# COx2/docker-nvidia-glx-desktop

Measured on AMD Instinct MI355X. Metric: encoded FPS + p50 end-to-end latency at 1080p60 H.264; concurrent sessions/node, higher is better.
Workload: dtype uint8 video (8-bit 4:2:0), H.264 Constrained Baseline

## Files before the change

### csrc/bindings/module.cpp

```cpp
#include <pybind11/numpy.h>
#include <pybind11/pybind11.h>
#include <pybind11/stl.h>

#include <cstring>

#include "../codec/h264_core.h"
#include "../codec/h264_encoder.h"
#include "../codec/vp8_encoder.h"
#include "../codec/hevc_encoder.h"
#include "../common/hip_check.h"
#include "../common/trace.h"
#include "../kernels/pixel.h"
#include "../runtime/session.h"

namespace py = pybind11;
using namespace mx;

void register_net(py::module& m);
void register_audio(py::module& m);
void register_rfb(py::module& m);

namespace {

template <class T>
// ... 6 lines not shown
    return py::bytes(reinterpret_cast<const char*>(v.data()), v.size());
}

struct PyBits {
    std::vector<uint32_t> words;
    h264::BitWriter w;
    PyBits() : words(4096) { w.init(words.data()); }
    py::tuple finish() {
        const uint32_t bits = w.bits;
        w.flush();
        std::vector<uint8_t> out;
        for (uint32_t i = 0; i < (bits + 7) / 8; ++i) out.push_back((uint8_t)(words[i / 4] >> (24 - 8 * (i % 4))));
        return py::make_tuple(to_bytes(out), bits);
    }
};

py::tuple cavlc_block_py(const std::vector<int>& coef, int nc) {
    PyBits b;
    int16_t c[16] = {0};
    const int n = (int)coef.size();
    if (n != 4 && n != 15 && n != 16) throw std::invalid_argument("block must have 4, 15 or 16 coefficients");
    for (int i = 0; i < n; ++i) c[i] = (int16_t)coef[i];
    h264::cavlc_block(b.w, c, n, nc);
    return b.finish();
}

py::array_t<int> fdct_py(py::array_t<int, py::array::c_style | py::array::forcecast> x) {
    if (x.size() != 16) throw std::invalid_argument("need 16 values");
    py::array_t<int> y(16);
    h264::fdct4x4(x.data(), y.mutable_data());
    return y;
}
py::array_t<int> idct_py(py::array_t<int, py::array::c_style | py::array::forcecast> x) {
    if (x.size() != 16) throw std::invalid_argument("need 16 values");
    py::array_t<int> y(16);
    h264::idct4x4(x.data(), y.mutable_data());
    return y;
}

py::array_t<uint8_t> copy_plane(const uint8_t* dev, int pitch, int w, int h) {
    py::array_t<uint8_t> out({h, w});
    HIP_CHECK(hipDeviceSynchronize());
    HIP_CHECK(hipMemcpy2D(out.mutable_data(), w, dev, pitch, w, h, hipMemcpyDeviceToHost));
    return out;
}

}

PYBIND11_MODULE(_native, m) {
    m.doc() = "mxdesk native runtime: HIP kernels (gfx950), H.264 encoder, session pipeline";

    m.def("device_count", []() {
        int n = 0;
        if (hipGetDeviceCount(&n) != hipSuccess) return 0;
        return n;
    });
    m.def("set_device", [](int d) { HIP_CHECK(hipSetDevice(d)); });
    m.def("device_name", [](int d) {
        hipDeviceProp_t p;
        HIP_CHECK(hipGetDeviceProperties(&p, d));
        return std::string(p.gcnArchName) + " / " + p.name;
    });
    m.def("synchronize", []() { HIP_CHECK(hipDeviceSynchronize()); });
    register_net(m);
    register_audio(m);
    register_rfb(m);
    m.def("now_us", &Session::now_us, "CLOCK_MONOTONIC microseconds (same clock as time.monotonic())");

    py::module h = m.def_submodule("h264", "H.264 building blocks (for tests)");
    h.def("hpel_planes", [](py::array_t<uint8_t, py::array::c_style> ref, int coded_w) {
        if (ref.ndim() != 2 || coded_w % 16 || ref.shape(0) % 16 || ref.shape(1) < coded_w)
            throw std::invalid_argument("ref must be (coded_h, pitch) with 16-aligned coded size");
        int hp = 0;
        auto planes = h264::hpel_planes_for_test(ref.data(), coded_w, (int)ref.shape(0), (int)ref.shape(1), &hp);
        const int rows = (int)ref.shape(0) + 2 * h264::kHpelPad;
        py::list out;
        for (auto& p : planes) {
            py::array_t<uint8_t> a({rows, hp});
            std::memcpy(a.mutable_data(), p.data(), p.size());
            out.append(a);
        }
        return out;
    });
    h.def("cavlc_block", &cavlc_block_py, py::arg("coef"), py::arg("nc"));
    h.def("fdct4x4", &fdct_py);
    h.def("idct4x4", &idct_py);
    h.def("ue", [](uint32_t k) {
        PyBits b;
        h264::put_ue(b.w, k);
        return b.finish();
    });
    h.def("se", [](int v) {
        PyBits b;
        h264::put_se(b.w, v);
        return b.finish();
    });
    h.def("luma_qpel", [](py::array_t<uint8_t, py::array::c_style> plane, int x4, int y4) {
        if (plane.ndim() != 2) throw std::invalid_argument("2-D plane");
        const int H = (int)plane.shape(0), W = (int)plane.shape(1);
        return h264::luma_qpel(plane.data(), W, W, H, x4, y4);
    });
    h.def("level_for", &h264::pick_level);

    py::class_<h264::EncoderConfig>(m, "EncoderConfig")
        .def(py::init<>())
        .def_readwrite("width", &h264::EncoderConfig::width)
        .def_readwrite("height", &h264::EncoderConfig::height)
        .def_readwrite("fps", &h264::EncoderConfig::fps)
        .def_readwrite("bitrate_kbps", &h264::EncoderConfig::bitrate_kbps)
        .def_readwrite("qp", &h264::EncoderConfig::qp)
        .def_readwrite("qp_min", &h264::EncoderConfig::qp_min)
        .def_readwrite("qp_max", &h264::EncoderConfig::qp_max)
        .def_readwrite("keyint", &h264::EncoderConfig::keyint)
        .def_readwrite("search_range", &h264::EncoderConfig::search_range)
        .def_readwrite("me_coarse", &h264::EncoderConfig::me_coarse)
        .def_readwrite("intra4x4", &h264::EncoderConfig::intra4x4)
        .def_readwrite("subpel", &h264::EncoderConfig::subpel)
        .def_readwrite("chroma_qp_offset", &h264::EncoderConfig::chroma_qp_offset)
        .def_readwrite("pipeline_depth", &h264::EncoderConfig::pipeline_depth)
        .def_readwrite("aq", &h264::EncoderConfig::aq)
        .def_readwrite("intra_in_p", &h264::EncoderConfig::intra_in_p)
        .def_readwrite("vp8_bpred", &h264::EncoderConfig::vp8_bpred)
        .def_readwrite("vp8_intra", &h264::EncoderConfig::vp8_intra)
        .def_readwrite("mask_x0", &h264::EncoderConfig::mask_x0)
        .def_readwrite("mask_y0", &h264::EncoderConfig::mask_y0)
        .def_readwrite("mask_x1", &h264::EncoderConfig::mask_x1)
        .def_readwrite("mask_y1", &h264::EncoderConfig::mask_y1)
        .def_readwrite("deblock", &h264::EncoderConfig::deblock)
        .def_readwrite("partitions", &h264::EncoderConfig::partitions)
        .def_readwrite("tu_split", &h264::EncoderConfig::tu_split)
        .def_readwrite("hevc_slice_cost", &h264::EncoderConfig::hevc_slice_cost)
        .def_readwrite("hevc_wpp", &h264::EncoderConfig::hevc_wpp)
        .def_readwrite("hevc_wpp_rows", &h264::EncoderConfig::hevc_wpp_rows)
        .def_readwrite("sao", &h264::EncoderConfig::sao)
        .def_readwrite("hevc_chroma_keep", &h264::EncoderConfig::hevc_chroma_keep)
        .def_readwrite("hevc_intra_split", &h264::EncoderConfig::hevc_intra_split);

    py::class_<h264::FrameStats>(m, "FrameStats")
        .def_readonly("frame_index", &h264::FrameStats::frame_index)
        .def_readonly("idr", &h264::FrameStats::idr)
        .def_readonly("qp", &h264::FrameStats::qp)
        .def_readonly("bytes", &h264::FrameStats::bytes)
        .def_readonly("skipped_mbs", &h264::FrameStats::skipped_mbs)
        .def_readonly("encode_ms", &h264::FrameStats::encode_ms)
        .def_property_readonly("sse", [](const h264::FrameStats& s) { return py::make_tuple(s.sse[0], s.sse[1], s.sse[2]); })
        .def_readonly("sse_masked", &h264::FrameStats::sse_masked)
        .def_readonly("masked_pixels", &h264::FrameStats::masked_pixels)
        .def_readonly("deblocked", &h264::FrameStats::deblocked)
        .def_readonly("db_coherent", &h264::FrameStats::db_coherent)
        .def_readonly("db_changed", &h264::FrameStats::db_changed)
        .def_readonly("db_moving", &h264::FrameStats::db_moving);

    py::class_<h264::CpuH264Encoder>(m, "CpuH264Encoder")
        .def(py::init<const h264::EncoderConfig&>())
        .def(
            "encode",
            [](h264::CpuH264Encoder& e, py::array_t<uint8_t, py::array::c_style> y,
               py::array_t<uint8_t, py::array::c_style> uv, bool force_idr) {
                if (y.ndim() != 2 || uv.ndim() != 2 || y.shape(1) != uv.shape(1))
                    throw std::invalid_argument("y (H,P) and uv (H/2,P) planes with equal pitch");
                const int pitch = (int)y.shape(1);
                const int cw = e.coded_pitch();
                const auto& cfg = e.common().config();
                const int ch = e.common().mb_h() * 16;
                if (y.shape(0) < cfg.height || pitch < cfg.width || uv.shape(0) < cfg.height / 2)
                    throw std::invalid_argument("planes smaller than the encoder's configured picture");
// ... 598 lines not shown
```

### csrc/codec/h264_encoder.cpp

```cpp
#include "h264_encoder.h"

#include <hip/hip_ext.h>

#include <algorithm>
#include <cmath>
#include <cstring>
#include <stdexcept>
#include <string>

#include "../common/hip_check.h"
#include "h264_mb.h"

namespace mx {
namespace h264 {

EncoderCommon::EncoderCommon(const EncoderConfig& c) : cfg_(c) {
    if (c.width <= 0 || c.height <= 0 || (c.width & 1) || (c.height & 1))
        throw std::invalid_argument("encoder size must be positive and even");
    mb_w_ = (c.width + 15) / 16;
    mb_h_ = (c.height + 15) / 16;
    cur_qp_ = std::clamp(c.qp, 0, 51);
}

double EncoderCommon::frame_budget_bits() const {
// ... 106 lines not shown
        const uint8_t b = rbsp[i];
        if (zeros >= 2 && b <= 3) {
            out.push_back(3);
            zeros = 0;
        }
        out.push_back(b);
        zeros = (b == 0) ? zeros + 1 : 0;
    }
}

void EncoderCommon::write_parameter_sets(std::vector<uint8_t>& out) const {
    uint32_t words[64];
    SeqParams sp;
    sp.width = cfg_.width;
    sp.height = cfg_.height;
    sp.mb_w = mb_w_;
    sp.mb_h = mb_h_;
    sp.level_idc = pick_level(mb_w_ * mb_h_, cfg_.fps);
    sp.log2_max_frame_num = log2_max_frame_num();
    sp.fps_num = cfg_.fps;
    sp.fps_den = 1;
    BitWriter w;
    w.init(words);
    write_sps(w, sp);
    std::vector<uint8_t> rbsp;
    words_to_bytes(words, w.bits + (w.bits % 8 ? 8 - w.bits % 8 : 0), rbsp);
    static const uint8_t sc[4] = {0, 0, 0, 1};
    out.insert(out.end(), sc, sc + 4);
    out.push_back(0x67);
    emulation_prevent(out, rbsp.data(), rbsp.size());
    w.init(words);
    write_pps(w, pic_init_qp(), cfg_.chroma_qp_offset);
    rbsp.clear();
    words_to_bytes(words, w.bits + (w.bits % 8 ? 8 - w.bits % 8 : 0), rbsp);
    out.insert(out.end(), sc, sc + 4);
    out.push_back(0x68);
    emulation_prevent(out, rbsp.data(), rbsp.size());
}

void EncoderCommon::write_slice_nal(std::vector<uint8_t>& out, const uint8_t* rbsp, size_t n, bool idr) const {
    static const uint8_t sc[4] = {0, 0, 0, 1};
    out.insert(out.end(), sc, sc + 4);
    out.push_back(idr ? 0x65 : 0x41);
    emulation_prevent(out, rbsp, n);
}

std::vector<std::vector<uint8_t>> hpel_planes_for_test(const uint8_t* ref, int coded_w, int coded_h, int pitch,
                                                       int* hp_pitch_out) {
    Geometry g{};
    g.width = coded_w;
    g.height = coded_h;
    g.mb_w = coded_w / 16;
    g.mb_h = coded_h / 16;
    g.coded_w = coded_w;
    g.coded_h = coded_h;
    g.pitch = pitch;
    const int hp_pitch = (coded_w + 2 * kHpelPad + 255) & ~255;
    const size_t hp_bytes = (size_t)hp_pitch * (coded_h + 2 * kHpelPad);
    uint8_t* dref = nullptr;
    uint8_t* planes[4];
    FrameState fs{};
    DeviceBuffers b{};
    HIP_CHECK(hipMalloc(&dref, (size_t)pitch * coded_h));
    HIP_CHECK(hipMemcpy(dref, ref, (size_t)pitch * coded_h, hipMemcpyHostToDevice));
    for (auto& p : planes) {
        HIP_CHECK(hipMalloc(&p, hp_bytes));
        HIP_CHECK(hipMemset(p, 0, hp_bytes));
    }
    fs.ref_y = dref;
    HIP_CHECK(hipMalloc(&b.fs, sizeof(FrameState)));
    HIP_CHECK(hipMemcpy(b.fs, &fs, sizeof(FrameState), hipMemcpyHostToDevice));
    launch_hpel(g, b, planes, hp_pitch, nullptr);
    HIP_CHECK(hipGetLastError());
    HIP_CHECK(hipDeviceSynchronize());
    std::vector<std::vector<uint8_t>> out(4, std::vector<uint8_t>(hp_bytes));
    for (int i = 0; i < 4; ++i) {
        HIP_CHECK(hipMemcpy(out[i].data(), planes[i], hp_bytes, hipMemcpyDeviceToHost));
        (void)hipFree(planes[i]);
    }
    (void)hipFree(dref);
    (void)hipFree(b.fs);
    *hp_pitch_out = hp_pitch;
    return out;
}

constexpr unsigned kDeviceEvent = hipEventDisableTiming | hipEventReleaseToDevice;

void GpuH264Encoder::alloc_slot(FrameSlot& sl) {
    const int nmb = geom_.mb_w * geom_.mb_h;
    DeviceBuffers& b = sl.buf;
    HIP_CHECK(hipMalloc(&b.fs, sizeof(FrameState)));
    HIP_CHECK(hipMalloc(&b.mb, sizeof(MbInfo) * nmb));
    HIP_CHECK(hipMemsetAsync(b.mb, 0, sizeof(MbInfo) * nmb, stream_));
    HIP_CHECK(hipMalloc(&b.coef, sizeof(int16_t) * kCoefStride * nmb));
    HIP_CHECK(hipMalloc(&b.slot, sizeof(uint32_t) * kSlotWords * (size_t)nmb));
    HIP_CHECK(hipMalloc(&b.slot_bits, sizeof(uint32_t) * nmb));
    HIP_CHECK(hipMalloc(&b.row_agg, sizeof(uint4) * (size_t)geom_.mb_h));
    HIP_CHECK(hipMalloc(&b.row_sse, sizeof(unsigned long long) * 4 * 512));
    HIP_CHECK(hipMalloc(&b.coded_info, sizeof(uint4) * nmb));
    HIP_CHECK(hipMalloc(&b.slice_info, sizeof(uint32_t) * kSliceInfo * kMaxSlices));
    HIP_CHECK(hipMemsetAsync(b.slice_info, 0, sizeof(uint32_t) * kSliceInfo * kMaxSlices, stream_));
    b.out_bytes = (size_t)nmb * 768;
    HIP_CHECK(hipMalloc(&b.quad_unit, sizeof(uint32_t) * (b.out_bytes / 16 + 1)));
    HIP_CHECK(hipMalloc(&b.out_hdr, sizeof(OutHeader)));
    HIP_CHECK(hipMalloc(&b.sse_part, 4 * sizeof(unsigned long long) * kSsePartStride));
    HIP_CHECK(hipMalloc(&b.wave_prog, sizeof(int) * 4));
    HIP_CHECK(hipMalloc(&b.mb_sse, sizeof(uint32_t) * 3 * (size_t)nmb));
    HIP_CHECK(hipMalloc(&b.intra_gain, sizeof(int32_t) * (size_t)nmb));
    HIP_CHECK(hipMalloc(&b.intra_cand, sizeof(int) * (size_t)nmb));
    HIP_CHECK(hipMalloc(&b.db_rec, sizeof(uint4) * (size_t)nmb));
    HIP_CHECK(hipMalloc(&b.db_rowq, sizeof(int) * (size_t)geom_.mb_h));
    HIP_CHECK(hipMalloc(&b.db_glb, sizeof(uint64_t) * 2 * 24 * (size_t)nmb));
    HIP_CHECK(hipMemsetAsync(b.db_glb, 0, sizeof(uint64_t) * 2 * 24 * (size_t)nmb, stream_));
    HIP_CHECK(hipMalloc(&b.pack_done, sizeof(uint32_t)));
    HIP_CHECK(hipMemsetAsync(b.pack_done, 0, sizeof(uint32_t), stream_));
    HIP_CHECK(hipMalloc(&b.db_cnt, sizeof(uint32_t) * 4));
    HIP_CHECK(hipMemsetAsync(b.db_cnt, 0, sizeof(uint32_t) * 4, stream_));
    HIP_CHECK(hipHostMalloc(&b.db_err, sizeof(int), hipHostMallocMapped));
    *b.db_err = 0;
    HIP_CHECK(hipHostMalloc(&sl.fs_host, sizeof(FrameState), hipHostMallocDefault));
    HIP_CHECK(hipHostMalloc(&sl.host_out, kOutPayloadOffset + b.out_bytes + 16, hipHostMallocMapped));
    std::memset(sl.host_out, 0, kOutPayloadOffset);
    HIP_CHECK(hipEventCreateWithFlags(&sl.start, hipEventDisableTiming));
    HIP_CHECK(hipEventCreateWithFlags(&sl.analysis_done, kDeviceEvent));
    HIP_CHECK(hipEventCreateWithFlags(&sl.deblock_done, kDeviceEvent));
    HIP_CHECK(hipEventCreateWithFlags(&sl.hpel_done, kDeviceEvent));
    HIP_CHECK(hipEventCreateWithFlags(&sl.me_done, kDeviceEvent));
    HIP_CHECK(hipEventCreateWithFlags(&sl.done, hipEventDisableTiming));
}

void GpuH264Encoder::free_slot(FrameSlot& sl) {
    DeviceBuffers& b = sl.buf;
    for (void* p : {(void*)b.fs, (void*)b.mb, (void*)b.coef, (void*)b.slot, (void*)b.slot_bits, (void*)b.row_agg,
                    (void*)b.row_sse, (void*)b.coded_info, (void*)b.slice_info,
                    (void*)b.out_hdr, (void*)b.sse_part, (void*)b.wave_prog, (void*)b.mb_sse, (void*)b.intra_gain, (void*)b.intra_cand, (void*)b.quad_unit,
                    (void*)b.db_rec, (void*)b.db_rowq, (void*)b.db_glb, (void*)b.pack_done, (void*)b.db_cnt})
        if (p) (void)hipFree(p);
    if (b.db_err) (void)hipHostFree(b.db_err);
    if (sl.fs_host) (void)hipHostFree(sl.fs_host);
    if (sl.host_out) (void)hipHostFree(sl.host_out);
    for (hipEvent_t e : {sl.start, sl.analysis_done, sl.deblock_done, sl.done, sl.hpel_done, sl.me_done})
        if (e) (void)hipEventDestroy(e);
}

GpuH264Encoder::GpuH264Encoder(const EncoderConfig& cfg, hipStream_t stream)
    : cfg_(cfg.with_aq_default(4)), common_(cfg), stream_(stream) {
    if (cfg.pipeline_depth < 1 || cfg.pipeline_depth > kMaxInFlight)
        throw std::invalid_argument("pipeline_depth must be 1 to 4");
    depth_ = cfg.pipeline_depth;
    db_lag_.reset(cfg_.h264_deblock_mode());
    geom_.width = cfg.width;
    geom_.height = cfg.height;
    geom_.mb_w = common_.mb_w();
    geom_.mb_h = common_.mb_h();
    geom_.coded_w = geom_.mb_w * 16;
    geom_.coded_h = geom_.mb_h * 16;
    geom_.pitch = (geom_.coded_w + 255) & ~255;
    if (geom_.mb_h > kMaxSlices) throw std::invalid_argument("picture too tall");
    if (geom_.mb_w > 512) throw std::invalid_argument("picture too wide (k_intra_wave stages <= 512 MBs per row)");
    const int nmb = geom_.mb_w * geom_.mb_h;
    if ((nmb + 3) / 4 + geom_.mb_h > kSsePartStride)
        throw std::invalid_argument("frame too large for the distortion partials");
    const size_t ysz = (size_t)geom_.pitch * geom_.coded_h, uvsz = ysz / 2;
    for (int i = 0; i < 2; ++i) {
        HIP_CHECK(hipMalloc(&rec_y_[i], ysz));
        HIP_CHECK(hipMalloc(&rec_uv_[i], uvsz));
        HIP_CHECK(hipMemsetAsync(rec_y_[i], 16, ysz, stream_));
        HIP_CHECK(hipMemsetAsync(rec_uv_[i], 128, uvsz, stream_));
        HIP_CHECK(hipMalloc(&src_keep_[i], ysz));
        HIP_CHECK(hipMemsetAsync(src_keep_[i], 16, ysz, stream_));
    }
    if (cfg.mask_x1 > cfg.mask_x0 && cfg.mask_y1 > cfg.mask_y0) {
        mask_mb_[0] = std::max(0, cfg.mask_x0) / 16;
        mask_mb_[1] = std::max(0, cfg.mask_y0) / 16;
        mask_mb_[2] = std::min(geom_.mb_w, (cfg.mask_x1 + 15) / 16);
        mask_mb_[3] = std::min(geom_.mb_h, (cfg.mask_y1 + 15) / 16);
    }
    masked_pixels_ = (int64_t)cfg.width * cfg.height;
    for (int my = mask_mb_[1]; my < mask_mb_[3]; ++my)
        for (int mx = mask_mb_[0]; mx < mask_mb_[2]; ++mx)
            masked_pixels_ -= (int64_t)std::max(0, std::min(16, cfg.width - 16 * mx)) *
                              std::max(0, std::min(16, cfg.height - 16 * my));
    hp_pitch_ = (geom_.coded_w + 2 * kHpelPad + 255) & ~255;
    const size_t hp_bytes = (size_t)hp_pitch_ * (geom_.coded_h + 2 * kHpelPad);
    for (int i = 0; i < 4; ++i) HIP_CHECK(hipMalloc(&hp_[i], hp_bytes));
    if (cfg_.h264_deblock())
        for (int i = 0; i < 4; ++i) HIP_CHECK(hipMalloc(&hpu_[i], hp_bytes));
    for (int i = 0; i < depth_; ++i) alloc_slot(slots_[i]);
    clock_khz_ = device_clock_khz();
    if (depth_ > 1) {
        HIP_CHECK(hipStreamCreateWithFlags(&stream_e_, hipStreamNonBlocking));
        HIP_CHECK(hipStreamCreateWithFlags(&stream_a_, hipStreamNonBlocking));
        HIP_CHECK(hipEventCreateWithFlags(&ref_ready_, kDeviceEvent));
        HIP_CHECK(hipEventRecord(ref_ready_, stream_));
        if (cfg_.h264_deblock()) {
            const char* rv = std::getenv("MXDESK_ME_CU_RESERVE");
            const int reserve = rv ? std::atoi(rv) : 0;
            int ncu = 0;
            HIP_CHECK(hipDeviceGetAttribute(&ncu, hipDeviceAttributeMultiprocessorCount, 0));
            if (reserve > 0 && reserve < ncu) {
                std::vector<uint32_t> mask((size_t)(ncu + 31) / 32, 0u);
                for (int c = 0; c < ncu - reserve; ++c) mask[(size_t)c / 32] |= 1u << (c % 32);
                HIP_CHECK(hipExtStreamCreateWithCUMask(&stream_m_, (uint32_t)mask.size(), mask.data()));
            } else {
                HIP_CHECK(hipStreamCreateWithFlags(&stream_m_, hipStreamNonBlocking));
            }
            HIP_CHECK(hipEventCreateWithFlags(&ev_hpu_, kDeviceEvent));
            HIP_CHECK(hipEventRecord(ev_hpu_, stream_));
        }
    }
    HIP_CHECK(hipStreamSynchronize(stream_));
    const char* et = std::getenv("MXDESK_ENTROPY_THREAD");
    if (stream_e_ && !(et && et[0] == '0')) {
        HIP_CHECK(hipGetDevice(&device_));
        launcher_ = std::thread([this]() { launcher_loop(); });
    }
}

void GpuH264Encoder::set_hpel_side_stream(bool on) {
    hpel_side_ = on;
    if (!on && stream_a_) {
        HIP_CHECK(hipStreamSynchronize(stream_a_));
        HIP_CHECK(hipStreamDestroy(stream_a_));
        stream_a_ = nullptr;
    }
}

void GpuH264Encoder::launcher_loop() {
    (void)hipSetDevice(device_);
    for (;;) {
        EntropyJob j;
        {
            std::unique_lock<std::mutex> lk(lmu_);
            lcv_.wait(lk, [&] { return lstop_ || !ljobs_.empty(); });
            if (ljobs_.empty()) return;
            j = ljobs_.front();
            ljobs_.pop_front();
        }
        try {
            FrameSlot& sl = slots_[j.slot];
            HIP_CHECK(hipStreamWaitEvent(stream_e_, sl.analysis_done, 0));
            launch_entropy(geom_, sl.buf, sl.host_out, stream_e_, j.sse_ready);
            HIP_CHECK(hipGetLastError());
            HIP_CHECK(hipEventRecord(sl.done, stream_e_));
        } catch (...) {
            std::lock_guard<std::mutex> lk(lmu_);
            lerr_ = std::current_exception();
        }
        {
            std::lock_guard<std::mutex> lk(lmu_);
            ++l_done_;
        }
        lcv_.notify_all();
    }
}

void GpuH264Encoder::drain_launcher() const {
    if (!launcher_.joinable()) return;
    std::unique_lock<std::mutex> lk(lmu_);
    lcv_.wait(lk, [&] { return l_done_ >= l_pushed_ || lerr_; });
    if (lerr_) std::rethrow_exception(lerr_);
}

void GpuH264Encoder::wait_launched(int slot) const {
    std::unique_lock<std::mutex> lk(lmu_);
    lcv_.wait(lk, [&] { return l_done_ >= slot_job_[slot] || lerr_; });
    if (lerr_) std::rethrow_exception(lerr_);
}

GpuH264Encoder::~GpuH264Encoder() {
    if (launcher_.joinable()) {
        {
            std::lock_guard<std::mutex> lk(lmu_);
            lstop_ = true;
        }
        lcv_.notify_all();
        launcher_.join();
    }
    (void)hipStreamSynchronize(stream_);
    if (stream_e_) {
        (void)hipStreamSynchronize(stream_e_);
        (void)hipStreamDestroy(stream_e_);
    }
    if (stream_a_) {
        (void)hipStreamSynchronize(stream_a_);
        (void)hipStreamDestroy(stream_a_);
    }
    if (ref_ready_) (void)hipEventDestroy(ref_ready_);
    if (stream_m_) {
        (void)hipStreamSynchronize(stream_m_);
        (void)hipStreamDestroy(stream_m_);
    }
    if (ev_hpu_) (void)hipEventDestroy(ev_hpu_);
    for (int i = 0; i < 4; ++i)
        if (hpu_[i]) (void)hipFree(hpu_[i]);
    for (int i = 0; i < 2; ++i) {
        (void)hipFree(rec_y_[i]);
        (void)hipFree(rec_uv_[i]);
        (void)hipFree(src_keep_[i]);
    }
    for (int i = 0; i < 4; ++i) (void)hipFree(hp_[i]);
    for (int i = 0; i < depth_; ++i) free_slot(slots_[i]);
}

void GpuH264Encoder::enqueue_analysis_kernels(bool idr, const uint8_t* src_y, const uint8_t* src_uv, bool publish) {
    FrameSlot& sl = slots_[prep_slot_];
    const FrameState* pub = publish ? sl.fs_host : nullptr;
    auto wait_input = [&]() {
        if (!in_ev_) return;
        HIP_CHECK(hipStreamWaitEvent(stream_, in_ev_, 0));
        in_ev_ = nullptr;
    };
    if (idr) {
        wait_input();
        launch_intra(geom_, sl.buf, src_y, src_uv, stream_, pub);
        if (cfg_.aq >= 3)
            launch_save_src(geom_, sl.buf, src_y, stream_);
    } else {
        static const bool early = [] {
            const char* e = std::getenv("MXDESK_INPUT_WAIT");
            return e && std::string(e) == "early";
        }();
        if (early) wait_input();
        const bool side_me = stream_m_ && pub && sl.me_unf;
        if (side_me) {
            HIP_CHECK(hipStreamWaitEvent(stream_m_, ev_hpu_, 0));
            if (in_ev_) {
                HIP_CHECK(hipStreamWaitEvent(stream_m_, in_ev_, 0));
                in_ev_ = nullptr;
            }
            launch_me(geom_, sl.buf, src_y, stream_m_, pub);
            HIP_CHECK(hipEventRecord(sl.me_done, stream_m_));
        }
        if (stream_a_ && hpel_side_ && pub && ref_seq_ + 1 == seq_) {
            HIP_CHECK(hipStreamWaitEvent(stream_a_, ref_ready_, 0));
            launch_hpel(geom_, sl.buf, hp_, hp_pitch_, stream_a_, pub);
            HIP_CHECK(hipEventRecord(sl.hpel_done, stream_a_));
            HIP_CHECK(hipStreamWaitEvent(stream_, sl.hpel_done, 0));
        } else {
            launch_hpel(geom_, sl.buf, hp_, hp_pitch_, stream_, pub);
        }
        wait_input();
        if (side_me)
            HIP_CHECK(hipStreamWaitEvent(stream_, sl.me_done, 0));
        else
            launch_me(geom_, sl.buf, src_y, stream_);
        launch_inter(geom_, sl.buf, src_y, src_uv, stream_);
        if (cfg_.intra_in_p) launch_intra_in_p(geom_, sl.buf, src_y, src_uv, stream_);
    }
}

void GpuH264Encoder::link_entropy() {
    if (!stream_e_) return;
    drain_launcher();
    FrameSlot& sl = slots_[prep_slot_];
    HIP_CHECK(hipEventRecord(sl.analysis_done, stream_));
    HIP_CHECK(hipStreamWaitEvent(stream_e_, sl.analysis_done, 0));
}

void GpuH264Encoder::enqueue_entropy() {
    drain_launcher();
    FrameSlot& sl = slots_[prep_slot_];
    launch_entropy(geom_, sl.buf, sl.host_out, stream_e_ ? stream_e_ : stream_, nullptr);
}

void GpuH264Encoder::unfiltered_planes(FrameSlot& sl) {
    launch_hpel_of(geom_, sl.fs_host->rec_y, hpu_, hp_pitch_, stream_);
    if (stream_m_) HIP_CHECK(hipEventRecord(ev_hpu_, stream_));
}

void GpuH264Encoder::enqueue_kernels(bool idr, const uint8_t* src_y, const uint8_t* src_uv, bool publish) {
    FrameSlot& sl = slots_[prep_slot_];
    enqueue_analysis_kernels(idr, src_y, src_uv, publish);
    async_frame_ = launcher_.joinable() && publish && !sync_launch_;
    if (async_frame_) {
        HIP_CHECK(hipEventRecord(sl.analysis_done, stream_));
        hipEvent_t sse_ready = nullptr;
        if (sl.deblock) {
            unfiltered_planes(sl);
            launch_deblock(geom_, sl.buf, src_y, src_uv, stream_);
            HIP_CHECK(hipEventRecord(sl.deblock_done, stream_));
            sse_ready = sl.deblock_done;
        }
        if (stream_a_ && hpel_side_ && publish) {
            HIP_CHECK(hipEventRecord(ref_ready_, stream_));
            ref_seq_ = seq_;
        }
        HIP_CHECK(hipGetLastError());
        {
            std::lock_guard<std::mutex> lk(lmu_);
            if (lerr_) std::rethrow_exception(lerr_);
            ljobs_.push_back(EntropyJob{prep_slot_, sse_ready});
            slot_job_[prep_slot_] = ++l_pushed_;
        }
        lcv_.notify_all();
        return;
    }
    link_entropy();
    hipStream_t es = stream_e_ ? stream_e_ : stream_;
    hipEvent_t sse_ready = nullptr;
    if (sl.deblock) {
        unfiltered_planes(sl);
        launch_deblock(geom_, sl.buf, src_y, src_uv, stream_);
        if (stream_e_) {
            HIP_CHECK(hipEventRecord(sl.deblock_done, stream_));
            sse_ready = sl.deblock_done;
        }
    }
    if (stream_a_ && hpel_side_ && publish) {
        HIP_CHECK(hipEventRecord(ref_ready_, stream_));
        ref_seq_ = seq_;
    }
    launch_entropy(geom_, sl.buf, sl.host_out, es, sse_ready);
    HIP_CHECK(hipGetLastError());
}

void GpuH264Encoder::fill_state(FrameSlot& sl, bool idr, int qp, int ref, int cur) {
    FrameState& f = *sl.fs_host;
    f.ref_y = rec_y_[ref];
    f.ref_uv = rec_uv_[ref];
    f.rec_y = rec_y_[cur];
    f.rec_uv = rec_uv_[cur];
    f.idr = idr ? 1 : 0;
    f.frame_num = common_.cur_frame_num();
    f.idr_pic_id = common_.cur_idr_pic_id();
    f.qp = qp;
    f.slice_rows = idr ? idr_slice_rows(geom_.mb_h) : geom_.mb_h;
    f.num_slices = (geom_.mb_h + f.slice_rows - 1) / f.slice_rows;
    f.search_range = me_range(cfg_.search_range);
    f.me_coarse = cfg_.me_coarse;
    f.intra4x4 = cfg_.intra4x4;
    f.subpel = cfg_.subpel;
    f.deblock_off = sl.deblock ? 0 : 1;
    if (++db_epoch_ == 0) db_epoch_ = 1;
    f.db_epoch = (int32_t)db_epoch_;
    f.pic_init_qp = common_.pic_init_qp();
    f.chroma_qp_offset = cfg_.chroma_qp_offset;
    f.log2_max_frame_num = common_.log2_max_frame_num();
    const size_t org = (size_t)kHpelPad * hp_pitch_ + kHpelPad;
    f.hp_pitch = hp_pitch_;
    f.aq = cfg_.aq;
    f.intra_in_p = cfg_.intra_in_p;
    f.partitions = cfg_.partitions ? 1 : 0;
    f.mask_mx0 = mask_mb_[0];
    f.mask_my0 = mask_mb_[1];
    f.mask_mx1 = mask_mb_[2];
    f.mask_my1 = mask_mb_[3];
    f.hp_f = hp_[0] + org;
    f.hp_h = hp_[1] + org;
    f.hp_v = hp_[2] + org;
    f.hp_j = hp_[3] + org;
    f.me_f = sl.me_unf ? hpu_[0] + org : nullptr;
    f.me_h = sl.me_unf ? hpu_[1] + org : nullptr;
    f.me_v = sl.me_unf ? hpu_[2] + org : nullptr;
    f.me_j = sl.me_unf ? hpu_[3] + org : nullptr;
    f.sse_part = sl.buf.sse_part;
    f.prev_src = src_keep_[ref];
    f.save_src = src_keep_[cur];
}

int GpuH264Encoder::probe_bytes(const uint8_t* src_y, const uint8_t* src_uv, int qp) {
    if (!inflight_.empty()) throw std::logic_error("GpuH264Encoder: probe with frames in flight");
    prep_slot_ = 0;
    FrameSlot& sl = slots_[0];
    sl.deblock = cfg_.deblock == 1;
    sl.me_unf = false;
    fill_state(sl, true, qp, cur_ ^ 1, cur_);
    sl.fs_host->frame_num = 0;
    sl.fs_host->idr_pic_id = 0;
    sync_launch_ = true;
    enqueue_kernels(true, src_y, src_uv, true);
    sync_launch_ = false;
    HIP_CHECK(hipStreamSynchronize(stream_));
    if (stream_e_) HIP_CHECK(hipStreamSynchronize(stream_e_));
    const OutHeader hdr = *reinterpret_cast<const OutHeader*>(sl.host_out);
    return hdr.overflow ? (int)sl.buf.out_bytes : (int)(hdr.total_bytes + hdr.num_slices * 6 + 32);
}

bool GpuH264Encoder::prepare(bool force_idr) {
    if ((int)inflight_.size() >= depth_)
        throw std::logic_error("GpuH264Encoder: collect() a frame first (pipeline full)");
    const int s = (depth_ == 1) ? 0 : next_slot_;
    next_slot_ = (next_slot_ + 1) % depth_;
    prep_slot_ = s;
    ++seq_;
    FrameSlot& sl = slots_[s];
    common_.begin_frame(force_idr || !have_ref_);
    have_ref_ = true;
    const bool idr = common_.cur_idr();
    sl.idr = idr;
    sl.qp = common_.cur_qp();
    const int ref = cur_;
    cur_ ^= 1;
    sl.fidx = seq_;
    sl.me_unf = !idr && last_deblock_;
    sl.deblock = db_lag_.decide((long long)seq_, idr);
    last_deblock_ = sl.deblock;
    fill_state(sl, idr, sl.qp, ref, cur_);
    return idr;
}

void GpuH264Encoder::enqueue_body(bool idr, const uint8_t* src_y, const uint8_t* src_uv) {
    drain_launcher();
    FrameSlot& sl = slots_[prep_slot_];
    HIP_CHECK(hipMemcpyAsync(sl.buf.fs, sl.fs_host, sizeof(FrameState), hipMemcpyHostToDevice, stream_));
    enqueue_kernels(idr, src_y, src_uv, false);
}

void GpuH264Encoder::enqueue_analysis(bool idr, const uint8_t* src_y, const uint8_t* src_uv) {
    drain_launcher();
    FrameSlot& sl = slots_[prep_slot_];
    HIP_CHECK(hipMemcpyAsync(sl.buf.fs, sl.fs_host, sizeof(FrameState), hipMemcpyHostToDevice, stream_));
    enqueue_analysis_kernels(idr, src_y, src_uv, false);
}

void GpuH264Encoder::record_start() {}

void GpuH264Encoder::record_done() {
    FrameSlot& sl = slots_[prep_slot_];
    if (async_frame_) {
        async_frame_ = false;
    } else {
        slot_job_[prep_slot_] = 0;
        HIP_CHECK(hipEventRecord(sl.done, stream_e_ ? stream_e_ : stream_));
    }
    inflight_.push_back(prep_slot_);
}

void GpuH264Encoder::submit(const uint8_t* src_y, const uint8_t* src_uv, bool force_idr) {
    while (common_.wants_probe()) {
        const int q = common_.probe_qp();
        common_.add_probe(q, probe_bytes(src_y, src_uv, q));
    }
    const bool idr = prepare(force_idr);
    record_start();
    enqueue_kernels(idr, src_y, src_uv, true);
    record_done();
}
// ... 51 lines not shown
```

### csrc/codec/h264_encoder.h

```cpp
#pragma once
#include <hip/hip_runtime.h>
#include <stdint.h>

#include <cmath>
#include <condition_variable>
#include <cstdlib>
#include <deque>
#include <exception>
#include <mutex>
#include <string>
#include <thread>
#include <vector>

#include "h264_core.h"
#include "h264_deblock.h"
#include "h264_gpu.h"
#include "video_encoder.h"

namespace mx {
namespace h264 {

struct EncoderConfig {
    int width = 1920;
    int height = 1080;
// ... 37 lines not shown
};

struct FrameStats {
    int64_t frame_index = 0;
    int idr = 0;
    int qp = 0;
    int bytes = 0;
    int skipped_mbs = 0;
    double encode_ms = 0;
    uint64_t sse[3] = {0, 0, 0};
    uint64_t sse_masked = 0;
    int64_t masked_pixels = 0;
    int deblocked = 0;
    int db_coherent = 0, db_changed = 0, db_moving = 0;
};

class EncoderCommon {
   public:
    explicit EncoderCommon(const EncoderConfig& c);
    const EncoderConfig& config() const { return cfg_; }
    int mb_w() const { return mb_w_; }
    int mb_h() const { return mb_h_; }
    void begin_frame(bool force_idr);
    bool cur_idr() const { return cur_idr_; }
    int cur_qp() const { return cur_qp_; }
    int cur_frame_num() const { return frame_num_; }
    int cur_idr_pic_id() const { return idr_pic_id_; }
    int log2_max_frame_num() const { return 8; }
    int pic_init_qp() const { return 26; }
    void write_parameter_sets(std::vector<uint8_t>& out) const;
    void write_slice_nal(std::vector<uint8_t>& out, const uint8_t* rbsp, size_t n, bool idr) const;
    void end_frame(int bytes, bool idr);
    void request_idr() { idr_requested_ = true; }
    void set_bitrate(int kbps) { cfg_.bitrate_kbps = kbps; }
    int64_t frames() const { return frame_index_; }

    static double qstep(double qp) { return 0.625 * std::exp2(qp / 6.0); }
    double frame_budget_bits() const;
    bool wants_probe() const { return cfg_.bitrate_kbps > 0 && begun_ == 0 && probes_ < kMaxProbes && !probe_done_; }
    int probe_qp() const;
    void add_probe(int qp, int bytes);
    double vbv_excess_bits() const { return vbv_; }
    static constexpr int kDrainFrames = 4;
    static constexpr double kPPrior = 0.3;
    static constexpr double kIdrBudget = 5.0;
    static constexpr int kMaxProbes = 2;
    static constexpr int kMaxStep = 4;
    static constexpr int kMaxDown = 3;

   private:
    int qp_for(double x, double bits, double alpha) const;
    EncoderConfig cfg_;
    int mb_w_, mb_h_;
    bool cur_idr_ = true;
    bool idr_requested_ = true;
    int cur_qp_;
    int frame_num_ = 0;
    int idr_pic_id_ = -1;
    int64_t frame_index_ = 0;
    int64_t begun_ = 0;
    int64_t since_idr_ = 0;
    double x_i_ = 0, x_p_ = 0;
    double alpha_p_ = 1.0;
    double prev_p_bits_ = 0;
    int prev_p_qp_ = -1;
    int last_i_qp_ = -1, last_p_qp_ = -1;
    bool last_was_idr_ = false;
    double vbv_ = 0;
    struct Pending {
        double budget;
        int qp;
        bool idr;
        int64_t since_idr;
    };
    std::deque<Pending> pending_;
    int probes_ = 0;
    bool probe_done_ = false;
    int probe_q_[kMaxProbes] = {0, 0};
};

void emulation_prevent(std::vector<uint8_t>& out, const uint8_t* rbsp, size_t n);
std::vector<std::vector<uint8_t>> hpel_planes_for_test(const uint8_t* ref, int coded_w, int coded_h, int pitch,
                                                       int* hp_pitch);

class GpuH264Encoder final : public VideoEncoder {
   public:
    const char* codec() const override { return "h264"; }
    EncoderCommon& rc() override { return common_; }
    static constexpr int kMaxInFlight = 4;
    GpuH264Encoder(const EncoderConfig& cfg, hipStream_t stream);
    ~GpuH264Encoder();
    GpuH264Encoder(const GpuH264Encoder&) = delete;
    GpuH264Encoder& operator=(const GpuH264Encoder&) = delete;

    const Geometry& geometry() const override { return geom_; }
    int pitch() const override { return geom_.pitch; }
    hipStream_t stream() const { return stream_; }
    int depth() const override { return depth_; }
    int in_flight() const { return (int)inflight_.size(); }

    void submit(const uint8_t* src_y, const uint8_t* src_uv, bool force_idr = false) override;
    const std::vector<uint8_t>& collect() override;
    const FrameStats& last_stats() const override { return stats_; }
    EncoderCommon& common() { return common_; }
    const uint8_t* recon_y() const override { return rec_y_[cur_]; }
    const uint8_t* recon_uv() const override { return rec_uv_[cur_]; }
    bool prepare(bool force_idr) override;
    void enqueue_body(bool idr, const uint8_t* src_y, const uint8_t* src_uv) override;
    void record_start() override;
    void record_done() override;
    bool supports_split() const override { return !cfg_.h264_deblock(); }
    bool masked_sse_in_encoder() const override { return true; }
    int prep_slot() const override { return prep_slot_; }
    hipStream_t entropy_stream() const override { return stream_e_; }
    void enqueue_analysis(bool idr, const uint8_t* src_y, const uint8_t* src_uv) override;
    void enqueue_entropy() override;
    void link_entropy() override;
    void set_hpel_side_stream(bool on) override;
    void quiesce() override { drain_launcher(); }
    bool set_input_event(hipEvent_t ev) override {
        in_ev_ = ev;
        return true;
    }
    hipEvent_t done_event() const override { return last_done_; }
    bool device_clock() const override { return true; }
    uint64_t last_t_end() const override { return last_t_end_; }
    hipEvent_t pending_done_event() const override {
        if (inflight_.empty()) return last_done_;
        wait_launched(inflight_.front());
        return slots_[inflight_.front()].done;
    }
    void enqueue_kernels(bool idr, const uint8_t* src_y, const uint8_t* src_uv, bool publish);
    void enqueue_analysis_kernels(bool idr, const uint8_t* src_y, const uint8_t* src_uv, bool publish);

   private:
    struct FrameSlot {
        DeviceBuffers buf{};
        FrameState* fs_host = nullptr;
        uint8_t* host_out = nullptr;
        hipEvent_t start = nullptr, analysis_done = nullptr, deblock_done = nullptr, done = nullptr;
        hipEvent_t hpel_done = nullptr;
        bool idr = false;
        bool deblock = false;
        bool me_unf = false;
        int qp = 0;
        uint64_t fidx = 0;
        hipEvent_t me_done = nullptr;
    };
    void alloc_slot(FrameSlot& sl);
    void free_slot(FrameSlot& sl);
    void fill_state(FrameSlot& sl, bool idr, int qp, int ref, int cur);
    void unfiltered_planes(FrameSlot& sl);
    int probe_bytes(const uint8_t* src_y, const uint8_t* src_uv, int qp);
    struct EntropyJob {
        int slot;
        hipEvent_t sse_ready;
    };
    void launcher_loop();
    void wait_launched(int slot) const;
    void drain_launcher() const;
    std::thread launcher_;
    mutable std::mutex lmu_;
    mutable std::condition_variable lcv_;
    std::deque<EntropyJob> ljobs_;
    uint64_t l_pushed_ = 0, l_done_ = 0;
    uint64_t slot_job_[kMaxInFlight] = {};
    bool lstop_ = false;
    std::exception_ptr lerr_;
    bool sync_launch_ = false;
    bool async_frame_ = false;
    int device_ = 0;

    EncoderConfig cfg_;
    EncoderCommon common_;
    hipStream_t stream_;
    hipStream_t stream_e_ = nullptr;
    hipStream_t stream_a_ = nullptr;
    bool hpel_side_ = true;
    hipEvent_t in_ev_ = nullptr;
    hipEvent_t ref_ready_ = nullptr;
    uint64_t seq_ = 0, ref_seq_ = ~0ull;
    int depth_ = 1;
    Geometry geom_;
    FrameSlot slots_[kMaxInFlight];
    int next_slot_ = 0, prep_slot_ = 0;
    std::deque<int> inflight_;
    hipEvent_t last_done_ = nullptr;
    uint64_t last_t_end_ = 0;
    double clock_khz_ = 100000;
    uint8_t* hp_[4] = {nullptr, nullptr, nullptr, nullptr};
    uint8_t* hpu_[4] = {nullptr, nullptr, nullptr, nullptr};
    hipStream_t stream_m_ = nullptr;
    hipEvent_t ev_hpu_ = nullptr;
    bool last_deblock_ = false;
    int hp_pitch_ = 0;
    uint8_t* rec_y_[2] = {nullptr, nullptr};
    uint8_t* rec_uv_[2] = {nullptr, nullptr};
    uint8_t* src_keep_[2] = {nullptr, nullptr};
    int cur_ = 0;
    bool have_ref_ = false;
    uint32_t db_epoch_ = 0;
    DbLagDecision db_lag_;
    int mask_mb_[4] = {0, 0, 0, 0};
    int64_t masked_pixels_ = 0;
    std::vector<uint8_t> au_;
    FrameStats stats_;
};

class CpuH264Encoder {
   public:
    explicit CpuH264Encoder(const EncoderConfig& cfg);
    const std::vector<uint8_t>& encode(const uint8_t* y, const uint8_t* uv, int pitch, bool force_idr = false);
    const FrameStats& last_stats() const { return stats_; }
    EncoderCommon& common() { return common_; }
    const std::vector<uint8_t>& recon_y() const { return rec_y_[cur_]; }
    const std::vector<uint8_t>& recon_uv() const { return rec_uv_[cur_]; }
    int coded_pitch() const { return cw_; }
    const std::vector<uint32_t>& mb_bits() const { return mb_bits_; }
    const std::vector<MbInfo>& mb_info() const { return mb_; }

   private:
    void encode_intra(const uint8_t* y, const uint8_t* uv, int pitch);
    void encode_inter(const uint8_t* y, const uint8_t* uv, int pitch);
    void entropy(std::vector<uint8_t>& payload, std::vector<uint32_t>& slice_off, std::vector<uint32_t>& slice_len);
    int frame_qp_() const { return qp_override_ >= 0 ? qp_override_ : common_.cur_qp(); }
    void decide_deblock();
    void update_deblock_decision();
    bool deblock_now_ = false;
    bool ref_deblocked_ = false;
    std::vector<uint8_t> rec_unf_y_;
    DbLagDecision db_lag_;
    uint64_t enc_seq_ = 0;
    DbAutoCounts db_counts_;
    int qp_override_ = -1;

    EncoderConfig cfg_;
    EncoderCommon common_;
    int cw_, ch_;
    std::vector<uint8_t> rec_y_[2], rec_uv_[2];
    int cur_ = 0;
    bool have_ref_ = false;
    std::vector<MbInfo> mb_;
    std::vector<int16_t> coef_;
    std::vector<uint32_t> mb_bits_;
    std::vector<uint8_t> prev_src_;
    std::vector<uint8_t> au_;
    FrameStats stats_;
};

void me_search_cpu(const uint8_t* sy, int pitch, const uint8_t* ref_y, int cw, int ch, int x0, int y0, int qp,
                   int search_range, int subpel, int* mvx, int* mvy, int coarse);
void me_search_parts_cpu(const uint8_t* sy, int pitch, const uint8_t* ref_y, int cw, int ch, int x0, int y0, int qp,
                         int search_range, int subpel, int coarse, MbInfo& m);

void pad_nv12(const uint8_t* y, const uint8_t* uv, int w, int h, int pitch, int coded_w, int coded_h,
              std::vector<uint8_t>& oy, std::vector<uint8_t>& ouv);

}
}
```

### csrc/codec/h264_gpu.h

```cpp
#pragma once
#include <vector>
#include <hip/hip_runtime.h>
#include <stdint.h>

#define MXHD_GPU __host__ __device__ __forceinline__

namespace mx {
namespace h264 {

constexpr int kSlotWords = 640;
constexpr int kCoefStride = 416;
constexpr int kCoefLuma = 0;
constexpr int kCoefLumaDc = 256;
constexpr int kCoefChromaDc = 272;
constexpr int kCoefChromaAc = 280;

enum MbType : uint8_t { kMbP16x16 = 0, kMbI16x16 = 1, kMbI4x4 = 2 };

struct MbInfo {
    int16_t mvx, mvy;
    uint8_t type;
    uint8_t cbp;
    uint8_t i16_mode;
    uint8_t chroma_mode;
    uint8_t nz_luma[16];
    uint8_t nz_cb[4];
    uint8_t nz_cr[4];
    uint8_t skip;
    uint8_t qp;
    uint8_t cbp_c;
    uint8_t itype;
    uint8_t i4[8];
    uint32_t cost;
    int16_t pmv[4];
    uint8_t part;
    uint8_t pad_[7];
};
static_assert(sizeof(MbInfo) == 64, "MbInfo layout");
enum MbPart : uint8_t { kPart16x16 = 0, kPart16x8 = 1, kPart8x16 = 2 };

MXHD_GPU bool is_intra(const MbInfo& m) { return m.type != kMbP16x16; }
template <class FS>
MXHD_GPU bool mb_unmasked(const FS* fs, int mbx, int mby) {
    return !(mbx >= fs->mask_mx0 && mbx < fs->mask_mx1 && mby >= fs->mask_my0 && mby < fs->mask_my1);
}
MXHD_GPU bool carries_dqp(const MbInfo& m) { return m.type == kMbI16x16 || m.cbp != 0; }

struct FrameState {
    const uint8_t* ref_y;
    const uint8_t* ref_uv;
    uint8_t* rec_y;
    uint8_t* rec_uv;
    int32_t idr;
    int32_t frame_num;
    int32_t idr_pic_id;
    int32_t qp;
    int32_t slice_rows;
    int32_t num_slices;
    int32_t search_range;
    int32_t subpel;
    int32_t me_coarse;
    int32_t intra4x4;
    int32_t deblock_off;
    int32_t db_epoch;
    int32_t pic_init_qp;
    int32_t chroma_qp_offset;
    int32_t log2_max_frame_num;
    int32_t hp_pitch;
    int32_t aq;
    int32_t intra_in_p;
    int32_t partitions;
    int32_t mask_mx0, mask_my0, mask_mx1, mask_my1;
    const uint8_t* prev_src;
    uint8_t* save_src;
    const uint8_t* hp_f;
    const uint8_t* hp_h;
    const uint8_t* hp_v;
    const uint8_t* hp_j;
    const uint8_t* me_f;
    const uint8_t* me_h;
    const uint8_t* me_v;
    const uint8_t* me_j;
    unsigned long long* sse_part;
};
constexpr int kHpelPad = 48;
constexpr int kSsePartStride = 65536;

struct OutHeader {
    uint32_t total_bytes;
    uint32_t num_slices;
    uint32_t overflow;
    uint32_t deblocked;
    uint64_t sse[3];
    uint64_t sse_masked;
    uint64_t t_start;
    uint64_t t_end;
    uint32_t db_coherent, db_changed, db_moving;
    uint32_t pad;
};
static_assert(sizeof(OutHeader) % 16 == 0, "payload must stay 16-byte aligned");
constexpr int kMaxSlices = 1024;
constexpr int kSliceInfo = 8;
constexpr size_t kOutPayloadOffset = sizeof(OutHeader) + 2 * kMaxSlices * sizeof(uint32_t);

struct Geometry {
    int width, height;
    int mb_w, mb_h;
    int pitch;
    int coded_w, coded_h;
};

struct DeviceBuffers {
    FrameState* fs;
    MbInfo* mb;
    int16_t* coef;
    uint32_t* slot;
    uint32_t* slot_bits;
    uint4* row_agg;
    unsigned long long* row_sse;
    uint4* coded_info;
    uint32_t* quad_unit;
    uint32_t* slice_info;
    size_t out_bytes;
    OutHeader* out_hdr;
    unsigned long long* sse_part;
    int* wave_prog;
    int32_t* intra_gain;
    int* intra_cand;
    uint32_t* mb_sse;
    uint4* db_rec;
    int* db_rowq;
    uint64_t* db_glb;
    int* db_err;
    uint32_t* db_cnt;
    uint32_t* pack_done;
};

void launch_me(const Geometry& g, const DeviceBuffers& b, const uint8_t* src_y, hipStream_t stream,
               const FrameState* state = nullptr);
void launch_hpel_of(const Geometry& g, const uint8_t* luma, uint8_t* const planes[4], int hp_pitch, hipStream_t stream);
void launch_inter(const Geometry& g, const DeviceBuffers& b, const uint8_t* src_y, const uint8_t* src_uv,
                  hipStream_t stream);
void launch_intra(const Geometry& g, const DeviceBuffers& b, const uint8_t* src_y, const uint8_t* src_uv,
                  hipStream_t stream, const FrameState* publish = nullptr);
void launch_hpel(const Geometry& g, const DeviceBuffers& b, uint8_t* const planes[4], int hp_pitch,
                 hipStream_t stream, const FrameState* publish = nullptr);
std::vector<unsigned long long> deblock_row_stamps(int mb_h);
void launch_deblock(const Geometry& g, const DeviceBuffers& b, const uint8_t* src_y, const uint8_t* src_uv,
                    hipStream_t stream);
void launch_save_src(const Geometry& g, const DeviceBuffers& b, const uint8_t* src_y, hipStream_t stream);
void launch_entropy(const Geometry& g, const DeviceBuffers& b, uint8_t* host_out, hipStream_t stream,
                    hipEvent_t wait_for_sse = nullptr);
void launch_intra_in_p(const Geometry& g, const DeviceBuffers& b, const uint8_t* src_y, const uint8_t* src_uv,
                       hipStream_t stream);

}
}
```

### csrc/codec/h264_kernels.hip

```cpp
#include <hip/hip_runtime.h>

#include <cstddef>

#include "../common/hip_check.h"
#include "h264_core.h"
#include "h264_deblock.h"
#include "h264_gpu.h"
#include "h264_mb.h"

namespace mx {
namespace h264 {

namespace {

__device__ __forceinline__ uint32_t bswap32(uint32_t v) { return __builtin_bswap32(v); }

template <bool kSwap>
struct OrWriter {
    uint32_t* dst;
    uint32_t pos;
    uint64_t acc;
    int nacc;
    uint32_t bits;

    __device__ __forceinline__ void init(uint32_t* d, uint32_t bitpos) {
        dst = d;
        pos = bitpos;
        acc = 0;
        nacc = 0;
        bits = 0;
    }
    __device__ __forceinline__ void emit(uint32_t w, int n) {
        const uint32_t wi = pos >> 5, sh = pos & 31;
        uint32_t a = w >> sh;
        if (a) atomicOr(dst + wi, kSwap ? bswap32(a) : a);
        if (sh && n > (int)(32 - sh)) {
            uint32_t b2 = w << (32 - sh);
            if (b2) atomicOr(dst + wi + 1, kSwap ? bswap32(b2) : b2);
        }
        pos += n;
    }
    __device__ __forceinline__ void put(uint32_t v, int n) {
        if (n <= 0) return;
        uint64_t m = (n == 32) ? 0xffffffffull : ((1ull << n) - 1);
        acc = (acc << n) | (v & m);
        nacc += n;
        bits += n;
        if (nacc >= 32) {
            emit((uint32_t)(acc >> (nacc - 32)), 32);
            nacc -= 32;
        }
    }
    __device__ __forceinline__ void flush() {
        if (nacc > 0) {
            emit((uint32_t)(acc << (32 - nacc)), nacc);
            nacc = 0;
            acc = 0;
        }
    }
};

__device__ __forceinline__ uint32_t rows_sum(uint32_t v) {
    const auto r16 = __builtin_amdgcn_permlane16_swap(v, v, false, false);
    v = r16[0] + r16[1];
    const auto r32 = __builtin_amdgcn_permlane32_swap(v, v, false, false);
    return r32[0] + r32[1];
}
__device__ __forceinline__ int wave_sum(int v) {
    v += __builtin_amdgcn_mov_dpp(v, 0xB1, 0xF, 0xF, false);
    v += __builtin_amdgcn_mov_dpp(v, 0x4E, 0xF, 0xF, false);
    v += __builtin_amdgcn_mov_dpp(v, 0x124, 0xF, 0xF, false);
    v += __builtin_amdgcn_mov_dpp(v, 0x128, 0xF, 0xF, false);
    return (int)rows_sum((uint32_t)v);
}

struct Planes {
    const uint8_t *f, *h, *v, *j;
    int pitch;
};
__device__ __forceinline__ Planes planes_of(const FrameState* fs) {
    return Planes{fs->hp_f, fs->hp_h, fs->hp_v, fs->hp_j, fs->hp_pitch};
}
__device__ __forceinline__ Planes me_planes_of(const FrameState* fs) {
    return fs->me_f ? Planes{fs->me_f, fs->me_h, fs->me_v, fs->me_j, fs->hp_pitch} : planes_of(fs);
}
__device__ __forceinline__ int qpel_planes(const Planes& P, int x4, int y4) {
    const int xi = x4 >> 2, yi = y4 >> 2, xf = x4 & 3, yf = y4 & 3;
    const int o = yi * P.pitch + xi;
    const int G = P.f[o];
    if ((xf | yf) == 0) return G;
    if (yf == 0) {
        const int b = P.h[o];
        if (xf == 2) return b;
        return ((xf == 1 ? G : (int)P.f[o + 1]) + b + 1) >> 1;
    }
    if (xf == 0) {
        const int hh = P.v[o];
        if (yf == 2) return hh;
        return ((yf == 1 ? G : (int)P.f[o + P.pitch]) + hh + 1) >> 1;
    }
    if (xf == 2 && yf == 2) return P.j[o];
    if (xf == 2) return ((yf == 1 ? (int)P.h[o] : (int)P.h[o + P.pitch]) + P.j[o] + 1) >> 1;
    if (yf == 2) return ((xf == 1 ? (int)P.v[o] : (int)P.v[o + 1]) + P.j[o] + 1) >> 1;
    const int bb = (yf == 1) ? P.h[o] : P.h[o + P.pitch];
    const int hh = (xf == 1) ? P.v[o] : P.v[o + 1];
    return (bb + hh + 1) >> 1;
}

constexpr int kHpTW = 128, kHpTH = 16;
constexpr int kHpSW = kHpTW + 8;
__device__ __forceinline__ int byte_of(uint32_t w, int k) { return (int)((w >> (8 * k)) & 0xff); }
__device__ __forceinline__ uint32_t pack4(int a, int b, int c, int d) {
    const uint32_t lo = __builtin_amdgcn_perm((uint32_t)b, (uint32_t)a, 0x0c0c0400u);
    const uint32_t hi = __builtin_amdgcn_perm((uint32_t)d, (uint32_t)c, 0x0c0c0400u);
    return __builtin_amdgcn_perm(hi, lo, 0x05040100u);
}
struct StateArg {
    FrameState v;
    FrameState* dst;
    int publish;
    uint64_t* t_start;
};
__device__ __forceinline__ void publish_state(const StateArg& a) {
    static_assert(sizeof(FrameState) % 4 == 0, "FrameState is copied as dwords");
    if (a.t_start && blockIdx.x == 0 && blockIdx.y == 0 && threadIdx.x == 0) *a.t_start = wall_clock64();
    if (a.publish && blockIdx.x == 0 && blockIdx.y == 0 && threadIdx.x < sizeof(FrameState) / 4)
        reinterpret_cast<uint32_t*>(a.dst)[threadIdx.x] = reinterpret_cast<const uint32_t*>(&a.v)[threadIdx.x];
}
__device__ __forceinline__ const FrameState& state_of(const StateArg& a) { return a.publish ? a.v : *a.dst; }

__global__ __launch_bounds__(256) void k_hpel(Geometry g, StateArg sa, uint8_t* __restrict__ pf,
                                              uint8_t* __restrict__ ph, uint8_t* __restrict__ pv,
                                              uint8_t* __restrict__ pj, int hp_pitch,
                                              const uint8_t* __restrict__ src) {
    __shared__ uint32_t smp[kHpTH + 5][kHpSW / 4];
    __shared__ int4 b1[kHpTH + 5][kHpTW / 4];
    publish_state(sa);
    const uint8_t* __restrict__ ref = src ? src : state_of(sa).ref_y;
    const int px0 = blockIdx.x * kHpTW, py0 = blockIdx.y * kHpTH;
    const int W = g.coded_w + 2 * kHpelPad, H = g.coded_h + 2 * kHpelPad;
    const int tid = threadIdx.x;
    const int xs = px0 - 4 - kHpelPad, ys = py0 - 2 - kHpelPad;
    const bool interior = xs >= 0 && xs + kHpSW <= g.coded_w && ys >= 0 && ys + kHpTH + 5 <= g.coded_h &&
                          (g.pitch & 3) == 0 && (reinterpret_cast<uintptr_t>(ref) & 3) == 0;
    for (int i = tid; i < (kHpTH + 5) * (kHpSW / 4); i += 256) {
        const int r = i / (kHpSW / 4), k4 = i - r * (kHpSW / 4);
        uint32_t w;
        if (interior) {
            w = *reinterpret_cast<const uint32_t*>(ref + (size_t)(ys + r) * g.pitch + xs + 4 * k4);
        } else {
            w = 0;
            for (int k = 0; k < 4; ++k)
                w |= (uint32_t)ref_px(ref, g.pitch, g.coded_w, g.coded_h, xs + 4 * k4 + k, ys + r) << (8 * k);
        }
        smp[r][k4] = w;
    }
    __syncthreads();
    for (int i = tid; i < (kHpTH + 5) * (kHpTW / 4); i += 256) {
        const int r = i / (kHpTW / 4), q = i - r * (kHpTW / 4);
        const uint32_t w0 = smp[r][q], w1 = smp[r][q + 1], w2 = smp[r][q + 2];
        int s[12];
#pragma unroll
        for (int k = 0; k < 4; ++k) {
            s[k] = byte_of(w0, k);
            s[4 + k] = byte_of(w1, k);
            s[8 + k] = byte_of(w2, k);
        }
        int t[4];
#pragma unroll
        for (int j = 0; j < 4; ++j) t[j] = tap6(s[j + 2], s[j + 3], s[j + 4], s[j + 5], s[j + 6], s[j + 7]);
        b1[r][q] = make_int4(t[0], t[1], t[2], t[3]);
    }
    __syncthreads();
    const int q = tid & (kHpTW / 4 - 1), r0 = (tid / (kHpTW / 4)) * 2;
    const int x = px0 + 4 * q;
    if (x >= W) return;
    int sv[7][4], bv[7][4];
#pragma unroll
    for (int k = 0; k < 7; ++k) {
        const uint32_t w = smp[r0 + k][q + 1];
        const int4 bb = b1[r0 + k][q];
#pragma unroll
        for (int j = 0; j < 4; ++j) sv[k][j] = byte_of(w, j);
        bv[k][0] = bb.x;
        bv[k][1] = bb.y;
        bv[k][2] = bb.z;
        bv[k][3] = bb.w;
    }
#pragma unroll
    for (int rr = 0; rr < 2; ++rr) {
        const int y = py0 + r0 + rr;
        if (y >= H) break;
        int Hs[4], Vs[4], Js[4];
#pragma unroll
        for (int j = 0; j < 4; ++j) {
            Hs[j] = clip255((bv[rr + 2][j] + 16) >> 5);
            const int v1 = tap6(sv[rr][j], sv[rr + 1][j], sv[rr + 2][j], sv[rr + 3][j], sv[rr + 4][j], sv[rr + 5][j]);
            Vs[j] = clip255((v1 + 16) >> 5);
            const int j1 = tap6(bv[rr][j], bv[rr + 1][j], bv[rr + 2][j], bv[rr + 3][j], bv[rr + 4][j], bv[rr + 5][j]);
            Js[j] = clip255((j1 + 512) >> 10);
        }
        const size_t o = (size_t)y * hp_pitch + x;
        *reinterpret_cast<uint32_t*>(pf + o) = smp[r0 + rr + 2][q + 1];
        *reinterpret_cast<uint32_t*>(ph + o) = pack4(Hs[0], Hs[1], Hs[2], Hs[3]);
        *reinterpret_cast<uint32_t*>(pv + o) = pack4(Vs[0], Vs[1], Vs[2], Vs[3]);
        *reinterpret_cast<uint32_t*>(pj + o) = pack4(Js[0], Js[1], Js[2], Js[3]);
    }
}

constexpr int kSpW = 20;
__device__ __forceinline__ int qpel_lds(const uint8_t (*sp)[18][kSpW], int x4, int y4) {
    const int xi = x4 >> 2, yi = y4 >> 2, xf = x4 & 3, yf = y4 & 3;
    const int G = sp[0][yi][xi];
    if ((xf | yf) == 0) return G;
    if (yf == 0) {
        const int b = sp[1][yi][xi];
        if (xf == 2) return b;
        return ((xf == 1 ? G : (int)sp[0][yi][xi + 1]) + b + 1) >> 1;
    }
    if (xf == 0) {
        const int hh = sp[2][yi][xi];
        if (yf == 2) return hh;
        return ((yf == 1 ? G : (int)sp[0][yi + 1][xi]) + hh + 1) >> 1;
    }
    if (xf == 2 && yf == 2) return sp[3][yi][xi];
    if (xf == 2) return ((yf == 1 ? (int)sp[1][yi][xi] : (int)sp[1][yi + 1][xi]) + sp[3][yi][xi] + 1) >> 1;
    if (yf == 2) return ((xf == 1 ? (int)sp[2][yi][xi] : (int)sp[2][yi][xi + 1]) + sp[3][yi][xi] + 1) >> 1;
    const int bb = (yf == 1) ? sp[1][yi][xi] : sp[1][yi + 1][xi];
    const int hh = (xf == 1) ? sp[2][yi][xi] : sp[2][yi][xi + 1];
    return (bb + hh + 1) >> 1;
}

constexpr int kMaxRange = 32;
static_assert(kMaxRange + 2 <= kHpelPad, "search window must stay inside the padded planes");
constexpr int kWinStride = 16 + 2 * kMaxRange + 8;

constexpr int kMeThreads = 256, kMeWaves = kMeThreads / 64;
__device__ __forceinline__ void me_full_body(const Geometry& g, const FrameState* __restrict__ fs,
                                             const uint8_t* __restrict__ src_y, MbInfo* __restrict__ mbs) {
    __shared__ uint32_t win32[(16 + 2 * kMaxRange) * kWinStride / 4];
    __shared__ uint32_t srcw[64];
    __shared__ unsigned long long red[kMeWaves];
    __shared__ uint32_t cand_cost[8];
    __shared__ uint32_t s_sad0[4];

    const int mbi = blockIdx.x;
    const int mbx = mbi % g.mb_w, mby = mbi / g.mb_w;
    const int x0 = mbx * 16, y0 = mby * 16;
    const int tid = threadIdx.x, lane = tid & 63;
    const int R = me_range(fs->search_range);
    const int W = 16 + 2 * R;
    const Planes P = me_planes_of(fs);
    const int lambda = lambda_sad(fs->qp);

    constexpr int kWs4 = kWinStride / 4;
    {
        if (tid < 64) {
            const int r = tid >> 2, c4 = (tid & 3) * 4;
            const uint32_t sw = *reinterpret_cast<const uint32_t*>(src_y + (y0 + r) * g.pitch + x0 + c4);
            const uint32_t rw = *reinterpret_cast<const uint32_t*>(P.f + (y0 + r) * P.pitch + x0 + c4);
            const int d = wave_sum((int)__builtin_amdgcn_sad_u8(sw, rw, 0u));
            if (tid == 0) s_sad0[0] = (uint32_t)d;
        }
        __syncthreads();
        const uint32_t sad0 = s_sad0[0];
        if (sad0 <= static_sad(fs->qp)) {
            if (tid == 0) {
                MbInfo& m = mbs[mbi];
                m.mvx = 0;
                m.mvy = 0;
                m.part = kPart16x16;
                m.pmv[0] = m.pmv[1] = m.pmv[2] = m.pmv[3] = 0;
            }
            return;
        }
    }
    const bool t256 = tid < 256;
    for (int i = tid; i < W * kWs4; i += kMeThreads) {
        const int wy = i / kWs4, wx4 = (i - wy * kWs4) * 4;
        win32[i] = (wx4 < W) ? *reinterpret_cast<const uint32_t*>(P.f + (y0 - R + wy) * P.pitch + (x0 - R + wx4)) : 0u;
    }
    if (tid < 64) {
        const int r = tid >> 2, c = (tid & 3) * 4;
        srcw[tid] = *reinterpret_cast<const uint32_t*>(src_y + (y0 + r) * g.pitch + x0 + c);
    }
    __syncthreads();

    const int side = 2 * R + 1, gw = (side + 3) >> 2, ngroups = side * gw;
    unsigned long long best = ~0ull;
    const bool coarse = fs->me_coarse != 0;
    const bool parts = fs->partitions != 0;
    const int ntask = (coarse && !parts) ? (R + 1) * gw : 0;
    auto mkey = [&](uint32_t sad, int dxr, int dyr) {
        const int dx = dxr - R, dy = dyr - R;
        const uint32_t cost = me_cost(sad, lambda, 4 * dx, 4 * dy);
        const uint32_t dist = (uint32_t)(abs(dx) + abs(dy));
        return ((unsigned long long)cost << 32) | (dist << 16) | (uint32_t)(dyr * side + dxr);
    };
    unsigned long long pb[4] = {~0ull, ~0ull, ~0ull, ~0ull};
    auto kmin = [](unsigned long long a, unsigned long long c) { return c < a ? c : a; };
    auto visit_quads = [&](const uint32_t* qd, int dxr, int dyr) {
        best = kmin(best, mkey(qd[0] + qd[1] + qd[2] + qd[3], dxr, dyr));
        pb[0] = kmin(pb[0], mkey(qd[0] + qd[1], dxr, dyr));
        pb[1] = kmin(pb[1], mkey(qd[2] + qd[3], dxr, dyr));
        pb[2] = kmin(pb[2], mkey(qd[0] + qd[2], dxr, dyr));
        pb[3] = kmin(pb[3], mkey(qd[1] + qd[3], dxr, dyr));
    };
    if (parts) {
        const int nsh = coarse ? 2 : 4, ntp = coarse ? (R + 1) * gw : ngroups;
        for (int q = tid; q < ntp; q += kMeThreads) {
            const int dyr = coarse ? 2 * (q / gw) : q / gw, g = q % gw;
            uint32_t acc[4][4];
#pragma unroll
            for (int i = 0; i < 4; ++i) acc[i][0] = acc[i][1] = acc[i][2] = acc[i][3] = 0;
#pragma unroll 2
            for (int r = 0; r < 16; ++r) {
                const int a = (dyr + r) * kWs4 + g, hq = r < 8 ? 0 : 2;
                const uint32_t w0 = win32[a], w1 = win32[a + 1], w2 = win32[a + 2], w3 = win32[a + 3], w4 = win32[a + 4];
                const uint32_t s0 = srcw[r * 4 + 0], s1 = srcw[r * 4 + 1], s2 = srcw[r * 4 + 2], s3 = srcw[r * 4 + 3];
#pragma unroll
                for (int si = 0; si < 4; ++si) {
                    if (si >= nsh) break;
                    const int sh = coarse ? 2 * si : si;
                    const uint32_t a0 = sh ? __builtin_amdgcn_alignbyte(w1, w0, sh) : w0;
                    const uint32_t a1 = sh ? __builtin_amdgcn_alignbyte(w2, w1, sh) : w1;
                    const uint32_t a2 = sh ? __builtin_amdgcn_alignbyte(w3, w2, sh) : w2;
                    const uint32_t a3 = sh ? __builtin_amdgcn_alignbyte(w4, w3, sh) : w3;
                    uint32_t lft = hq ? acc[si][2] : acc[si][0], rgt = hq ? acc[si][3] : acc[si][1];
                    lft = __builtin_amdgcn_sad_u8(a1, s1, __builtin_amdgcn_sad_u8(a0, s0, lft));
                    rgt = __builtin_amdgcn_sad_u8(a3, s3, __builtin_amdgcn_sad_u8(a2, s2, rgt));
                    if (hq) {
                        acc[si][2] = lft;
                        acc[si][3] = rgt;
                    } else {
                        acc[si][0] = lft;
                        acc[si][1] = rgt;
                    }
                }
            }
#pragma unroll
            for (int si = 0; si < 4; ++si) {
                if (si >= nsh) break;
                const int dxr = 4 * g + (coarse ? 2 * si : si);
                if (dxr >= side) break;
                visit_quads(acc[si], dxr, dyr);
            }
        }
    }
    for (int q = tid; q < ntask; q += kMeThreads) {
        const int dyr = 2 * (q / gw), g = q % gw;
        uint32_t s0a = 0, s2a = 0;
#pragma unroll 4
        for (int r = 0; r < 16; ++r) {
            const int a = (dyr + r) * kWs4 + g;
            const uint32_t w0 = win32[a], w1 = win32[a + 1], w2 = win32[a + 2], w3 = win32[a + 3], w4 = win32[a + 4];
            const uint32_t s0 = srcw[r * 4 + 0], s1 = srcw[r * 4 + 1], s2 = srcw[r * 4 + 2], s3 = srcw[r * 4 + 3];
            s0a = __builtin_amdgcn_sad_u8(w0, s0, s0a);
            s0a = __builtin_amdgcn_sad_u8(w1, s1, s0a);
            s0a = __builtin_amdgcn_sad_u8(w2, s2, s0a);
            s0a = __builtin_amdgcn_sad_u8(w3, s3, s0a);
            s2a = __builtin_amdgcn_sad_u8(__builtin_amdgcn_alignbyte(w1, w0, 2), s0, s2a);
            s2a = __builtin_amdgcn_sad_u8(__builtin_amdgcn_alignbyte(w2, w1, 2), s1, s2a);
            s2a = __builtin_amdgcn_sad_u8(__builtin_amdgcn_alignbyte(w3, w2, 2), s2, s2a);
            s2a = __builtin_amdgcn_sad_u8(__builtin_amdgcn_alignbyte(w4, w3, 2), s3, s2a);
        }
#pragma unroll
        for (int h2 = 0; h2 < 2; ++h2) {
            const int dxr = 4 * g + 2 * h2;
            if (dxr >= side) break;
            const int dx = dxr - R, dy = dyr - R, c = dyr * side + dxr;
            const uint32_t cost = me_cost(h2 ? s2a : s0a, lambda, 4 * dx, 4 * dy);
            const uint32_t dist = (uint32_t)(abs(dx) + abs(dy));
            const unsigned long long key = ((unsigned long long)cost << 32) | (dist << 16) | (uint32_t)c;
            best = key < best ? key : best;
// ... 45 lines not shown
            for (int o = 32; o > 0; o >>= 1) {
                const unsigned long long other = __shfl_xor(v, o, 64);
                v = other < v ? other : v;
            }
            if (lane == 0) pred4[sh][tid >> 6] = v;
        }
    }
    __syncthreads();
    unsigned long long b = red[0];
    for (int i = 1; i < kMeWaves; ++i) b = red[i] < b ? red[i] : b;
    unsigned long long pbest[4] = {~0ull, ~0ull, ~0ull, ~0ull};
    if (parts)
        for (int sh = 0; sh < 4; ++sh)
            for (int i = 0; i < kMeWaves; ++i) pbest[sh] = pred4[sh][i] < pbest[sh] ? pred4[sh][i] : pbest[sh];
    if (parts && coarse) {
        __shared__ unsigned long long pnkey[4][8];
        const int ev = (tid & 255) >> 3, sub = tid & 7, sh = ev >> 3, k = ev & 7;
        const int cb0 = (int)(pbest[sh] & 0xffff), bxr = cb0 % side, byr = cb0 / side;
        int ddx, ddy;
        subpel_offset(k, &ddx, &ddy);
        const int nxr = bxr + ddx, nyr = byr + ddy;
        const bool inside = t256 && nxr >= 0 && nxr < side && nyr >= 0 && nyr < side;
        int d = 0;
        if (inside) {
            const uint8_t* wb = reinterpret_cast<const uint8_t*>(win32);
            const uint8_t* sb = reinterpret_cast<const uint8_t*>(srcw);
            for (int part_row = 0; part_row < 2; ++part_row) {
                const int rr = sh < 2 ? (sh == 0 ? sub : 8 + sub) : 2 * sub + part_row;
                const int c0 = sh < 2 ? 8 * part_row : (sh == 2 ? 0 : 8);
#pragma unroll
                for (int j = 0; j < 8; ++j)
                    d += abs((int)sb[rr * 16 + c0 + j] - (int)wb[(nyr + rr) * kWinStride + nxr + c0 + j]);
            }
        }
        for (int o = 4; o > 0; o >>= 1) d += __shfl_xor(d, o, 64);
        if (t256 && sub == 0) pnkey[sh][k] = inside ? mkey((uint32_t)d, nxr, nyr) : ~0ull;
        __syncthreads();
        for (int s2 = 0; s2 < 4; ++s2)
            for (int i = 0; i < 8; ++i) pbest[s2] = pnkey[s2][i] < pbest[s2] ? pnkey[s2][i] : pbest[s2];
    }
    if (coarse) {
        __shared__ unsigned long long nkey[8];
        const int cb0 = (int)(b & 0xffff), bxr = cb0 % side, byr = cb0 / side;
        const int k = (tid & 255) >> 5, sub = tid & 31, py = sub >> 1, px0 = (sub & 1) * 8;
        int ddx, ddy;
        subpel_offset(k, &ddx, &ddy);
        const int nxr = bxr + ddx, nyr = byr + ddy;
        const bool inside = t256 && nxr >= 0 && nxr < side && nyr >= 0 && nyr < side;
        int d = 0;
        if (inside) {
            const uint8_t* wrow = reinterpret_cast<const uint8_t*>(win32) + (nyr + py) * kWinStride + nxr + px0;
            const uint32_t s0 = srcw[py * 4 + (px0 >> 2)], s1 = srcw[py * 4 + (px0 >> 2) + 1];
#pragma unroll
            for (int j = 0; j < 8; ++j) d += abs((int)(((j < 4 ? s0 : s1) >> (8 * (j & 3))) & 0xff) - (int)wrow[j]);
        }
        for (int o = 16; o > 0; o >>= 1) d += __shfl_xor(d, o, 64);
        if (t256 && sub == 0) {
            const int dx = nxr - R, dy = nyr - R;
            const uint32_t cost = me_cost((uint32_t)d, lambda, 4 * dx, 4 * dy);
            const uint32_t dist = (uint32_t)(abs(dx) + abs(dy));
            nkey[k] = inside ? (((unsigned long long)cost << 32) | (dist << 16) | (uint32_t)(nyr * side + nxr)) : ~0ull;
        }
        __syncthreads();
        for (int i = 0; i < 8; ++i) b = nkey[i] < b ? nkey[i] : b;
    }
    const int cbest = (int)(b & 0xffff);
    int mvx = 4 * ((cbest % side) - R), mvy = 4 * ((cbest / side) - R);

    if (parts) {
        const uint32_t c16 = (uint32_t)(b >> 32);
        const uint32_t chz = (uint32_t)(pbest[0] >> 32) + (uint32_t)(pbest[1] >> 32) + 2u * (uint32_t)lambda;
        const uint32_t cvt = (uint32_t)(pbest[2] >> 32) + (uint32_t)(pbest[3] >> 32) + 2u * (uint32_t)lambda;
        const int part = (c16 <= chz && c16 <= cvt) ? kPart16x16 : (chz <= cvt ? kPart16x8 : kPart8x16);
        if (part != kPart16x16) {
            const int s0 = part == kPart16x8 ? 0 : 2;
            int pvx[2], pvy[2];
            uint32_t pcost[2];
            for (int i = 0; i < 2; ++i) {
                const int cb = (int)(pbest[s0 + i] & 0xffff);
                pvx[i] = 4 * ((cb % side) - R);
                pvy[i] = 4 * ((cb / side) - R);
                pcost[i] = (uint32_t)(pbest[s0 + i] >> 32);
            }
            if (fs->subpel) {
                __shared__ uint8_t psp[2][4][18][kSpW];
                __shared__ uint32_t pcand[2][8];
                for (int i = tid; i < 2 * 4 * 18 * 18; i += kMeThreads) {
                    const int pi = i / (4 * 324), rem0 = i - pi * 4 * 324;
                    const int pl = rem0 / 324, rem = rem0 - pl * 324, r = rem / 18, c = rem - r * 18;
                    const uint8_t* base = pl == 0 ? P.f : pl == 1 ? P.h : pl == 2 ? P.v : P.j;
                    const int ix = x0 + (pvx[pi] >> 2) - 1, iy = y0 + (pvy[pi] >> 2) - 1;
                    psp[pi][pl][r][c] = base[(iy + r) * P.pitch + ix + c];
                }
                __syncthreads();
                const int pi = (tid & 255) >> 7, k = (tid >> 4) & 7, sub = tid & 15;
                const int rx = part == kPart8x16 ? 8 * pi : 0, ry = part == kPart16x8 ? 8 * pi : 0;
                const int prow = part == kPart16x8 ? (sub >> 1) : sub, pcol = part == kPart16x8 ? (sub & 1) * 8 : 0;
                const int yy = ry + prow, xx = rx + pcol;
                const uint32_t s0w = srcw[yy * 4 + (xx >> 2)], s1w = srcw[yy * 4 + (xx >> 2) + 1];
                const int ivx = pvx[pi], ivy = pvy[pi];
                const int base_x4 = xx * 4 + 4 - ivx, base_y4 = yy * 4 + 4 - ivy;
                for (int step = 2; step >= 1; step >>= 1) {
                    int ddx, ddy;
                    subpel_offset(k, &ddx, &ddy);
                    const int cx = pvx[pi] + ddx * step, cy = pvy[pi] + ddy * step;
                    int d = 0;
#pragma unroll
                    for (int j = 0; j < 8; ++j) {
                        const int sv = (int)(((j < 4 ? s0w : s1w) >> (8 * (j & 3))) & 0xff);
                        d += abs(sv - qpel_lds(psp[pi], base_x4 + 4 * j + cx, base_y4 + cy));
                    }
                    for (int o = 8; o > 0; o >>= 1) d += __shfl_xor(d, o, 64);
                    __syncthreads();
                    if (t256 && sub == 0) pcand[pi][k] = me_cost((uint32_t)d, lambda, cx, cy);
                    __syncthreads();
                    for (int q = 0; q < 2; ++q) {
                        int bdx = 0, bdy = 0;
                        uint32_t bcost = pcost[q];
                        for (int kk = 0; kk < 8; ++kk) {
                            const uint32_t cc = pcand[q][kk];
                            if (cc < bcost) {
                                int ex, ey;
                                subpel_offset(kk, &ex, &ey);
                                bcost = cc;
                                bdx = ex * step;
                                bdy = ey * step;
                            }
                        }
                        pvx[q] += bdx;
                        pvy[q] += bdy;
                        pcost[q] = bcost;
                    }
                }
            }
            if (tid == 0) {
                MbInfo& m = mbs[mbi];
                m.mvx = (int16_t)mvx;
                m.mvy = (int16_t)mvy;
                m.part = (uint8_t)part;
                m.pmv[0] = (int16_t)pvx[0];
                m.pmv[1] = (int16_t)pvy[0];
                m.pmv[2] = (int16_t)pvx[1];
                m.pmv[3] = (int16_t)pvy[1];
            }
            return;
        }
    }

    if (fs->subpel) {
        __shared__ uint8_t sp[4][18][kSpW];
        const int ix = x0 + (mvx >> 2) - 1, iy = y0 + (mvy >> 2) - 1;
        for (int i = tid; i < 4 * 18 * 18; i += kMeThreads) {
            const int pl = i / 324, rem = i - pl * 324, r = rem / 18, c = rem - r * 18;
            const uint8_t* base = pl == 0 ? P.f : pl == 1 ? P.h : pl == 2 ? P.v : P.j;
            sp[pl][r][c] = base[(iy + r) * P.pitch + ix + c];
        }
        __syncthreads();
        uint32_t cur_cost = (uint32_t)(b >> 32);
        const int k = (tid & 255) >> 5, sub = tid & 31;
        const int py = sub >> 1, px0 = (sub & 1) * 8;
        const uint32_t s0 = srcw[py * 4 + (px0 >> 2)], s1 = srcw[py * 4 + (px0 >> 2) + 1];
        const int base_x4 = px0 * 4 + 4 - mvx, base_y4 = py * 4 + 4 - mvy;
        for (int step = 2; step >= 1; step >>= 1) {
            int ddx, ddy;
            subpel_offset(k, &ddx, &ddy);
            const int cx = mvx + ddx * step, cy = mvy + ddy * step;
            int d = 0;
#pragma unroll
            for (int j = 0; j < 8; ++j) {
                const int sv = (int)(((j < 4 ? s0 : s1) >> (8 * (j & 3))) & 0xff);
                d += abs(sv - qpel_lds(sp, base_x4 + 4 * j + cx, base_y4 + cy));
            }
            for (int o = 16; o > 0; o >>= 1) d += __shfl_xor(d, o, 64);
            __syncthreads();
            if (t256 && sub == 0) cand_cost[k] = me_cost((uint32_t)d, lambda, cx, cy);
            __syncthreads();
            int bdx = 0, bdy = 0;
            uint32_t bcost = cur_cost;
            for (int kk = 0; kk < 8; ++kk) {
                const uint32_t cc = cand_cost[kk];
                if (cc < bcost) {
                    int ex, ey;
                    subpel_offset(kk, &ex, &ey);
                    bcost = cc;
                    bdx = ex * step;
                    bdy = ey * step;
                }
            }
            mvx += bdx;
            mvy += bdy;
            cur_cost = bcost;
        }
    }
    if (tid == 0) {
        MbInfo& m = mbs[mbi];
        m.mvx = (int16_t)mvx;
        m.mvy = (int16_t)mvy;
        m.part = kPart16x16;
        m.pmv[0] = m.pmv[1] = m.pmv[2] = m.pmv[3] = 0;
    }
}

__global__ __launch_bounds__(kMeThreads) void k_me_full(Geometry g, const FrameState* __restrict__ fs,
                                                  const uint8_t* __restrict__ src_y, MbInfo* __restrict__ mbs) {
    me_full_body(g, fs, src_y, mbs);
}
__global__ __launch_bounds__(kMeThreads) void k_me_full_val(Geometry g, FrameState fs,
                                                      const uint8_t* __restrict__ src_y, MbInfo* __restrict__ mbs) {
    me_full_body(g, &fs, src_y, mbs);
}

template <int K>
__device__ __forceinline__ int qbc(int v) {
    return __builtin_amdgcn_mov_dpp(v, K * 0x55, 0xF, 0xF, false);
}
__device__ __forceinline__ int quad_sum(int v) { return qbc<0>(v) + qbc<1>(v) + qbc<2>(v) + qbc<3>(v); }

__device__ __forceinline__ void fdct_row(const int* x, int r, int* y) {
    const int s03 = x[0] + x[3], d03 = x[0] - x[3], s12 = x[1] + x[2], d12 = x[1] - x[2];
    const int t[4] = {s03 + s12, 2 * d03 + d12, s03 - s12, d03 - 2 * d12};
#pragma unroll
    for (int c = 0; c < 4; ++c) {
        const int a0 = qbc<0>(t[c]), a1 = qbc<1>(t[c]), a2 = qbc<2>(t[c]), a3 = qbc<3>(t[c]);
        const int u03 = a0 + a3, e03 = a0 - a3, u12 = a1 + a2, e12 = a1 - a2;
        y[c] = r == 0 ? u03 + u12 : r == 1 ? 2 * e03 + e12 : r == 2 ? u03 - u12 : e03 - 2 * e12;
    }
}
__device__ __forceinline__ void idct_row(const int* d, int r, int* out) {
    const int e0 = d[0] + d[2], e1 = d[0] - d[2], e2 = (d[1] >> 1) - d[3], e3 = d[1] + (d[3] >> 1);
    const int f[4] = {e0 + e3, e1 + e2, e1 - e2, e0 - e3};
#pragma unroll
    for (int c = 0; c < 4; ++c) {
        const int b0 = qbc<0>(f[c]), b1 = qbc<1>(f[c]), b2 = qbc<2>(f[c]), b3 = qbc<3>(f[c]);
        const int g0 = b0 + b2, g1 = b0 - b2, g2 = (b1 >> 1) - b3, g3 = b1 + (b3 >> 1);
        const int v = r == 0 ? g0 + g3 : r == 1 ? g1 + g2 : r == 2 ? g1 - g2 : g0 - g3;
        out[c] = (v + 32) >> 6;
    }
}
__device__ __forceinline__ int had_row_abs(const int* x, int r) {
    const int t[4] = {x[0] + x[1] + x[2] + x[3], x[0] + x[1] - x[2] - x[3], x[0] - x[1] - x[2] + x[3],
                      x[0] - x[1] + x[2] - x[3]};
    int s = 0;
#pragma unroll
    for (int c = 0; c < 4; ++c) {
        const int a = qbc<0>(t[c]), b = qbc<1>(t[c]), cc = qbc<2>(t[c]), d = qbc<3>(t[c]);
        const int v = r == 0 ? a + b + cc + d : r == 1 ? a + b - cc - d : r == 2 ? a - b - cc + d : a - b + cc - d;
        s += v < 0 ? -v : v;
    }
    return s;
}
__device__ __forceinline__ int quant_row(const int* y, int r, int qp, bool intra, int start, int* z) {
    const int qm = qp % 6, qbits = 15 + qp / 6;
    const int f = intra ? ((1 << qbits) / 3) : ((1 << qbits) / 6);
    int nz = 0;
#pragma unroll
    for (int c = 0; c < 4; ++c) {
        const int i = r * 4 + c;
        if (i < start) {
            z[c] = 0;
            continue;
        }
        const int a = y[c] < 0 ? -y[c] : y[c];
        int q = (int)(((int64_t)a * kQuantMF[qm][kPosClass[i]] + f) >> qbits);
        q = q > kMaxLevel ? kMaxLevel : q;
        z[c] = y[c] < 0 ? -q : q;
        nz += (q != 0);
    }
    return nz;
}
__device__ __forceinline__ void dequant_row(const int* z, int r, int qp, int* d) {
    const int qm = qp % 6, qs = qp / 6;
#pragma unroll
    for (int c = 0; c < 4; ++c) d[c] = z[c] * kDequantV[qm][kPosClass[r * 4 + c]] * (1 << qs);
}

__global__ __launch_bounds__(256) void k_inter_encode(Geometry g, const FrameState* __restrict__ fs,
                                                       const uint8_t* __restrict__ src_y,
                                                       const uint8_t* __restrict__ src_uv, MbInfo* __restrict__ mbs,
                                                       int16_t* __restrict__ coef, uint32_t* __restrict__ mb_sse,
                                                       int* __restrict__ wave_prog) {
    __shared__ uint8_t pred[4][384];
    __shared__ int16_t res[4][384];
    __shared__ int cdc[4][8];
    __shared__ int cdc_nz[4][2];

    const int wave = threadIdx.x >> 6, lane = threadIdx.x & 63;
    const int nmb = g.mb_w * g.mb_h;
    const int bid = blockIdx.x;
    const int mbi = bid * 4 + wave;
    if (bid == 0 && threadIdx.x == 0) wave_prog[1] = 0;
    const bool valid = mbi < nmb;
    const int mbx = valid ? mbi % g.mb_w : 0, mby = valid ? mbi / g.mb_w : 0;
    const int x0 = mbx * 16, y0 = mby * 16;
    const Planes P = planes_of(fs);
    const uint8_t* ref_uv = fs->ref_uv;
    const int cw = g.coded_w / 2, ch = g.coded_h / 2;
    int mvx = 0, mvy = 0;
    int lsad = 0;
    int tsad = 0;
    MbInfo mi;
    mi.part = kPart16x16;
    if (valid) {
        mi = mbs[mbi];
        const int r = lane >> 2, c0 = (lane & 3) * 4;
        const Mv lv = px_mv(mi, c0, r);
        mvx = lv.x;
        mvy = lv.y;
        const uint32_t sw = *reinterpret_cast<const uint32_t*>(src_y + (y0 + r) * g.pitch + x0 + c0);
        if (fs->aq >= 3) {
            const int ix = mvx >> 2, iy = mvy >> 2;
            const int px = x0 + c0 + ix, py = y0 + r + iy;
            if (px >= 0 && px + 4 <= g.coded_w && py >= 0 && py < g.coded_h &&
                ((px & 3) == 0 || (px & ~3) + 8 <= g.pitch)) {
                const uint32_t* qa = reinterpret_cast<const uint32_t*>(fs->prev_src + (size_t)py * g.pitch + (px & ~3));
                const uint32_t sh = (uint32_t)(px & 3);
                const uint32_t pw = sh ? __builtin_amdgcn_alignbyte(qa[1], qa[0], sh) : qa[0];
                tsad = (int)__builtin_amdgcn_sad_u8(sw, pw, 0u);
            } else {
                for (int k = 0; k < 4; ++k)
                    tsad += abs((int)((sw >> (8 * k)) & 0xff) -
                                ref_px(fs->prev_src, g.pitch, g.coded_w, g.coded_h, x0 + c0 + k + ix, y0 + r + iy));
            }
            *reinterpret_cast<uint32_t*>(fs->save_src + (y0 + r) * g.pitch + x0 + c0) = sw;
        }
        if (((mvx | mvy) & 3) == 0) {
            const uint8_t* q = P.f + (size_t)((y0 + r) + (mvy >> 2)) * P.pitch + (x0 + c0 + (mvx >> 2));
            const uint32_t* qa = reinterpret_cast<const uint32_t*>(reinterpret_cast<uintptr_t>(q) & ~(uintptr_t)3);
            const uint32_t sh = (uint32_t)(reinterpret_cast<uintptr_t>(q) & 3);
            const uint32_t pw = sh ? __builtin_amdgcn_alignbyte(qa[1], qa[0], sh) : qa[0];
            for (int k = 0; k < 4; ++k) {
                const int p = (int)((pw >> (8 * k)) & 0xff);
                const int d = (int)((sw >> (8 * k)) & 0xff) - p;
                pred[wave][r * 16 + c0 + k] = (uint8_t)p;
                res[wave][r * 16 + c0 + k] = (int16_t)d;
                lsad += d < 0 ? -d : d;
            }
        } else {
            for (int k = 0; k < 4; ++k) {
                const int p = qpel_planes(P, (x0 + c0 + k) * 4 + mvx, (y0 + r) * 4 + mvy);
                const int d = (int)((sw >> (8 * k)) & 0xff) - p;
                pred[wave][r * 16 + c0 + k] = (uint8_t)p;
                res[wave][r * 16 + c0 + k] = (int16_t)d;
                lsad += d < 0 ? -d : d;
            }
        }
        const int cr_ = lane >> 3, cc = lane & 7;
        const int xc = x0 / 2 + cc, yc = y0 / 2 + cr_;
        const Mv cv = px_mv(mi, 2 * cc, 2 * cr_);
        for (int comp = 0; comp < 2; ++comp) {
            const int p = chroma_pred8(ref_uv, g.pitch, cw, ch, comp, xc * 8 + cv.x, yc * 8 + cv.y);
            const int sv = src_uv[yc * g.pitch + 2 * xc + comp];
            pred[wave][256 + comp * 64 + cr_ * 8 + cc] = (uint8_t)p;
            res[wave][256 + comp * 64 + cr_ * 8 + cc] = (int16_t)(sv - p);
        }
    }
    __syncthreads();
    const uint32_t lsad_mb = (uint32_t)wave_sum(lsad);
    const int tcls = temporal_class((uint32_t)wave_sum(tsad), __ballot((mvx | mvy) != 0) == 0ull);
    const int qp = mb_qp_for(fs->qp, lsad_mb, tcls, fs->aq);
    const int qpc = chroma_qp(qp, fs->chroma_qp_offset);
    int16_t* mc = coef + (size_t)(valid ? mbi : 0) * kCoefStride;

    const int lb = lane >> 2, rr = lane & 3, lbx = kBlkX[lb], lby = kBlkY[lb];
    int x[4], y[4], z[4], rres[4];
    const int ro = (lby * 4 + rr) * 16 + lbx * 4;
#pragma unroll
    for (int c = 0; c < 4; ++c) x[c] = res[wave][ro + c];
    const int hs = quad_sum(had_row_abs(x, rr));
    fdct_row(x, rr, y);
    const int nzb = quad_sum(quant_row(y, rr, qp, false, 0, z));
    {
        int d[4];
        dequant_row(z, rr, qp, d);
        idct_row(d, rr, rres);
    }
    int d_pred = 0, d_coded = 0;
#pragma unroll
    for (int c = 0; c < 4; ++c) {
        const int pv = pred[wave][ro + c];
        const int e = pv + x[c] - clip255(pv + rres[c]);
        d_pred += x[c] * x[c];
        d_coded += e * e;
    }
    const uint32_t bits = rr == 0 ? block_bits_est(nzb) : 0u;
    const bool drop = valid && drop_luma_for(fs->aq, lsad_mb, tcls, qp, wave_sum(d_pred), wave_sum(d_coded),
                                             (uint32_t)wave_sum((int)bits));
    const bool drop_c = drop_chroma_for(fs->aq, tcls, drop);
    const int nz_l = drop ? 0 : nzb;
    int sse_y = 0;
    if (valid) {
        uint32_t packed = 0;
        const bool vis = x0 + lbx * 4 < g.width && (y0 + lby * 4 + rr) < g.height;
#pragma unroll
        for (int c = 0; c < 4; ++c) {
            if (drop) z[c] = rres[c] = 0;
            mc[kCoefLuma + lb * 16 + kZigzagInv4x4[rr * 4 + c]] = (int16_t)z[c];
            const int pv = pred[wave][ro + c];
            const int v = clip255(pv + rres[c]);
            const int e = pv + x[c] - v;
            sse_y += vis ? e * e : 0;
            packed |= (uint32_t)v << (8 * c);
        }
        *reinterpret_cast<uint32_t*>(fs->rec_y + (y0 + lby * 4 + rr) * g.pitch + x0 + lbx * 4) = packed;
        if (rr == 0) mbs[mbi].nz_luma[lby * 4 + lbx] = (uint8_t)nz_l;
    }
    const uint32_t satd_mb = (uint32_t)wave_sum(rr == 0 ? (hs + 1) >> 1 : 0);

    const int cbk = lane >> 2, ccomp = (cbk >> 2) & 1, cblk = cbk & 3, cbx = cblk & 1, cby = cblk >> 1;
    const int co = 256 + ccomp * 64 + (cby * 4 + rr) * 8 + cbx * 4;
    const bool clane = lane < 32;
    int cz[4], nzc = 0;
    if (clane) {
        int cx[4], cy[4];
#pragma unroll
        for (int c = 0; c < 4; ++c) cx[c] = drop_c ? 0 : res[wave][co + c];
        fdct_row(cx, rr, cy);
        if (rr == 0) cdc[wave][ccomp * 4 + cblk] = cy[0];
        nzc = quant_row(cy, rr, qpc, false, 1, cz);
    }
    nzc = quad_sum(nzc);
    if (valid && clane) {
#pragma unroll
        for (int c = 0; c < 4; ++c) {
            const int i = rr * 4 + c;
            if (i > 0) mc[kCoefChromaAc + (ccomp * 4 + cblk) * 16 + kZigzagInv4x4[i]] = (int16_t)cz[c];
        }
        if (rr == 0) (ccomp ? mbs[mbi].nz_cr : mbs[mbi].nz_cb)[cblk] = (uint8_t)nzc;
    }
    __syncthreads();
    if (valid && (lane == 0 || lane == 16)) {
        const int comp = lane >> 4;
        int in[4], zd[4], dq[4];
        for (int i = 0; i < 4; ++i) in[i] = cdc[wave][comp * 4 + i];
        const int n = quant_dc_chroma(in, zd, qpc, false);
        for (int i = 0; i < 4; ++i) mc[kCoefChromaDc + comp * 4 + i] = (int16_t)zd[i];
        dequant_dc_chroma(zd, dq, qpc);
        for (int i = 0; i < 4; ++i) cdc[wave][comp * 4 + i] = dq[i];
        cdc_nz[wave][comp] = n;
    }
    __syncthreads();
    int sse_c = 0;
    if (clane) {
        int d[4], cr[4];
        dequant_row(cz, rr, qpc, d);
        if (rr == 0) d[0] = cdc[wave][ccomp * 4 + cblk];
        idct_row(d, rr, cr);
        if (valid) {
            const int xc = x0 / 2 + cbx * 4, yc = y0 / 2 + cby * 4 + rr;
#pragma unroll
            for (int c = 0; c < 4; ++c) {
                const int v = clip255(pred[wave][co + c] + cr[c]);
                const int e = pred[wave][co + c] + res[wave][co + c] - v;
                sse_c += (2 * (xc + c) < g.width && 2 * yc < g.height) ? e * e : 0;
                fs->rec_uv[yc * g.pitch + 2 * (xc + c) + ccomp] = (uint8_t)v;
            }
        }
    }
    {
        const int sy = wave_sum(sse_y);
        const int su = wave_sum(lane < 16 ? sse_c : 0);
        const int sv = wave_sum((lane >= 16 && lane < 32) ? sse_c : 0);
        if (valid && fs->intra_in_p && lane < 3)
            mb_sse[lane * nmb + mbi] = (uint32_t)(lane == 0 ? sy : (lane == 1 ? su : sv));
        __shared__ uint32_t part[4][4];
        if (lane == 0) {
            part[0][wave] = valid ? (uint32_t)sy : 0u;
            part[1][wave] = valid ? (uint32_t)su : 0u;
            part[2][wave] = valid ? (uint32_t)sv : 0u;
            part[3][wave] = (valid && mb_unmasked(fs, mbx, mby)) ? (uint32_t)sy : 0u;
        }
        __syncthreads();
        if (threadIdx.x < 4) {
            const int c = threadIdx.x;
            fs->sse_part[c * kSsePartStride + bid] =
                (unsigned long long)part[c][0] + part[c][1] + part[c][2] + part[c][3];
        }
    }
    const unsigned long long luma_mask = __ballot(valid && rr == 0 && nz_l > 0);
    const unsigned long long chroma_mask = __ballot(valid && clane && rr == 0 && nzc > 0);
    if (valid && lane == 0) {
        int cbp = 0;
        for (int b8 = 0; b8 < 4; ++b8)
            if ((luma_mask >> (16 * b8)) & 0x1111ull) cbp |= 1 << b8;
        const int cc = (chroma_mask != 0) ? 2 : ((cdc_nz[wave][0] | cdc_nz[wave][1]) ? 1 : 0);
        cbp |= cc << 4;
        MbInfo& m = mbs[mbi];
        m.type = kMbP16x16;
        m.cbp = (uint8_t)cbp;
        m.qp = (uint8_t)qp;
        m.i16_mode = 0;
        m.chroma_mode = 0;
        m.cost = inter_cost_mb(satd_mb, fs->qp, mi);
    }
}

__constant__ uint8_t kRasterToBlk[16] = {0, 1, 4, 5, 2, 3, 6, 7, 8, 9, 12, 13, 10, 11, 14, 15};
__device__ __forceinline__ void wave_sync_lds() {
    __builtin_amdgcn_fence(__ATOMIC_RELEASE, "wavefront");
    __builtin_amdgcn_wave_barrier();
    __builtin_amdgcn_fence(__ATOMIC_ACQUIRE, "wavefront");
}

constexpr int kLT = 24;
constexpr int kCT = 10;
constexpr int kCTI = 20;

__global__ __launch_bounds__(256) void k_intra_analyze(Geometry g, StateArg sa, const uint8_t* __restrict__ src_y,
                                                       const uint8_t* __restrict__ src_uv, MbInfo* __restrict__ mbs,
                                                       int* __restrict__ wave_prog, int32_t* __restrict__ gain,
                                                       int* __restrict__ cand) {
    __shared__ IntraCosts costs[4];
    __shared__ uint8_t ltile[4][17][kLT];
    __shared__ uint8_t ctile[4][9][kCTI];
    publish_state(sa);
    const FrameState* fs = &state_of(sa);
    if (blockIdx.x == 0) {
        if (!fs->idr)
            for (int i = threadIdx.x; i < 4 * g.mb_h; i += 256)
                fs->sse_part[(i / g.mb_h) * kSsePartStride + (g.mb_w * g.mb_h + 3) / 4 + i % g.mb_h] = 0;
    }
    const int wave = threadIdx.x >> 6, lane = threadIdx.x & 63;
    const int mbi = blockIdx.x * 4 + wave;
    if (mbi >= g.mb_w * g.mb_h) return;
    if (!fs->idr && !intra_candidate(mbs[mbi].cost)) {
        if (lane == 0) gain[mbi] = 0;
        return;
    }
    const int mbx = mbi % g.mb_w, mby = mbi / g.mb_w;
    const int x0 = mbx * 16, y0 = mby * 16;
    const Avail av = mb_avail(g, mbx, mby, fs->slice_rows);
    for (int i = lane; i < 17 * 21; i += 64) {
        const int r = i / 21, cx = i - r * 21, x = x0 - 1 + cx, y = y0 - 1 + r;
        ltile[wave][r][cx] = (x >= 0 && y >= 0 && x < g.coded_w) ? src_y[y * g.pitch + x] : 0;
    }
    for (int i = lane; i < 9 * 18; i += 64) {
        const int r = i / 18, bx = i - r * 18, x = x0 - 2 + bx, y = y0 / 2 - 1 + r;
        ctile[wave][r][bx] = (x >= 0 && y >= 0) ? src_uv[y * g.pitch + x] : 0;
    }
    wave_sync_lds();
    const uint8_t* sy = &ltile[wave][1][1];
    const uint8_t* suv = &ctile[wave][1][2];
    IntraCosts& c = costs[wave];
    const int rb = lane >> 2, r = lane & 3, bx = rb & 3, by = rb >> 2;
    auto satd_quad = [&](int d0, int d1, int d2, int d3) -> uint32_t {
        int t[4] = {d0 + d1 + d2 + d3, d0 + d1 - d2 - d3, d0 - d1 - d2 + d3, d0 - d1 + d2 - d3};
        uint32_t sum = 0;
#pragma unroll
        for (int j = 0; j < 4; ++j) {
            int v = t[j];
            int o = __builtin_amdgcn_mov_dpp(v, 0xB1, 0xF, 0xF, false);
            v = (r & 1) ? o - v : v + o;
            o = __builtin_amdgcn_mov_dpp(v, 0x4E, 0xF, 0xF, false);
            v = (r & 2) ? o - v : v + o;
            sum += (uint32_t)(v < 0 ? -v : v);
        }
        sum += (uint32_t)__builtin_amdgcn_mov_dpp((int)sum, 0xB1, 0xF, 0xF, false);
        sum += (uint32_t)__builtin_amdgcn_mov_dpp((int)sum, 0x4E, 0xF, 0xF, false);
        return (sum + 1) >> 1;
    };
    {
        const Nb4 n = nb4_from_plane(sy, kLT, 0, 0, bx, by, av.left, av.top, av.topright, av.topleft);
        int sv[4];
#pragma unroll
        for (int j = 0; j < 4; ++j) sv[j] = sy[(4 * by + r) * kLT + 4 * bx + j];
        for (int m = 0; m < 9; ++m) {
            const bool ok = i4_mode_ok(m, n);
            int d[4];
#pragma unroll
            for (int j = 0; j < 4; ++j) d[j] = ok ? sv[j] - pred4x4_px(m, n, j, r) : 0;
            const uint32_t t = satd_quad(d[0], d[1], d[2], d[3]);
            if (r == 0) c.c4[kRasterToBlk[rb]][m] = ok ? t : kCostInf;
        }
    }
    {
        const NbMb n = nbmb_from_plane(sy, kLT, 0, 0, 16, 1, 0, av.left, av.top, av.topleft);
        for (int m = 0; m < 4; ++m) {
            const bool ok = i16_mode_ok(m, n);
            uint32_t t = 0;
            if (ok) {
                const PredMb p = prep_i16(m, n);
                int d[4];
#pragma unroll
                for (int j = 0; j < 4; ++j)
                    d[j] = (int)sy[(4 * by + r) * kLT + 4 * bx + j] - pred16_px(p, n, 4 * bx + j, 4 * by + r);
// ... 1250 lines not shown
    const bool idr = fs->idr != 0;
    const int ns = (int)h.num_slices;
    const uint32_t nquads = (h.total_bytes + 15) / 16;
    uint4* out = reinterpret_cast<uint4*>(host + kOutPayloadOffset);
    const int sub = threadIdx.x & 3;
    for (size_t qbase = gid >> 2; qbase < ((nquads + 63) / 64) * 64; qbase += stride >> 2) {
        const bool active = qbase < nquads;
        uint32_t acc = 0;
        if (active) {
            const uint32_t W0 = (uint32_t)qbase * 128 + 32 * sub;
            const int qa = (int)quad_unit[qbase];
            int lo = 0, hi = ns - 1;
            while (lo < hi) {
                const int mid = (lo + hi + 1) >> 1;
                if (slice_info[kSliceInfo * mid + 1] * 8 <= W0) lo = mid; else hi = mid - 1;
            }
            for (int s = lo; s < ns; ++s) {
                const uint32_t sbit = slice_info[kSliceInfo * s + 1] * 8;
                if (sbit >= W0 + 32) break;
                const uint32_t hbits = slice_info[kSliceInfo * s + 0];
                const uint32_t dend = slice_info[kSliceInfo * s + 4];
                if (sbit + slice_info[kSliceInfo * s + 2] * 8 <= W0) continue;
                const uint32_t trail = idr ? 0u : slice_info[kSliceInfo * s + 3];
                if (sbit + hbits > W0) {
                    uint32_t hw[4] = {0, 0, 0, 0};
                    BitWriter bw;
                    bw.init(hw);
                    write_slice_header(bw, slice_params(fs, s, g.mb_w));
                    bw.flush();
                    overlap(acc, W0, sbit, hbits, [&](uint32_t x, int n) { return slot_get(hw, x, n); });
                }
                if (dend > W0 && sbit + hbits < W0 + 32) {
                    int a = max((int)slice_info[kSliceInfo * s + 6], qa);
                    const int rend = (int)slice_info[kSliceInfo * s + 7];
                    const int b = rend - 1;
                    while (a < b && coded_info[a + 1].x <= W0) ++a;
                    for (int r = a; r < rend; ++r) {
                        const uint4 ci = coded_info[r];
                        const uint32_t off = ci.x;
                        if (off >= W0 + 32) break;
                        if (off + ci.z <= W0) continue;
                        const int run = (int)ci.w;
                        const int plen = idr ? 0 : ue_len((uint32_t)run);
                        const uint32_t pv = (uint32_t)run + 1;
                        const uint32_t* sp = slot + (size_t)ci.y * kSlotWords;
                        overlap(acc, W0, off, ci.z, [&](uint32_t x, int n) {
                            uint32_t r2 = 0;
                            int rem = n;
                            if ((int)x < plen) {
                                const int kk = min(rem, plen - (int)x);
                                r2 = (pv >> (plen - (int)x - kk)) & mask_bits(kk);
                                rem -= kk;
                                x += kk;
                            }
                            if (rem > 0) r2 = (rem == 32 ? 0u : (r2 << rem)) | slot_get(sp, x - plen, rem);
                            return r2;
                        });
                    }
                }
                const int tl = trail ? ue_len(trail) : 0;
                const uint32_t tv = trail ? (((trail + 1) << 1) | 1u) : 1u;
                overlap(acc, W0, dend, tl + 1, [&](uint32_t x, int n) { return tv >> (tl + 1 - (int)x - n); });
            }
        }
        const uint32_t w = bswap32(acc);
        const int lane = threadIdx.x & 63, q0 = lane & ~3;
        const uint32_t w0 = __shfl(w, q0), w1 = __shfl(w, q0 + 1), w2 = __shfl(w, q0 + 2), w3 = __shfl(w, q0 + 3);
        if (active && sub == 0) out[qbase] = make_uint4(w0, w1, w2, w3);
    }
}

}

void launch_hpel(const Geometry& g, const DeviceBuffers& b, uint8_t* const planes[4], int hp_pitch,
                 hipStream_t stream, const FrameState* publish) {
    const int W = g.coded_w + 2 * kHpelPad, H = g.coded_h + 2 * kHpelPad;
    dim3 grid((W + kHpTW - 1) / kHpTW, (H + kHpTH - 1) / kHpTH);
    StateArg sa{};
    if (publish) sa.v = *publish;
    sa.dst = b.fs;
    sa.publish = publish ? 1 : 0;
    sa.t_start = b.out_hdr ? &b.out_hdr->t_start : nullptr;
    hipLaunchKernelGGL(k_hpel, grid, dim3(256), 0, stream, g, sa, planes[0], planes[1], planes[2], planes[3],
                       hp_pitch, (const uint8_t*)nullptr);
}

void launch_hpel_of(const Geometry& g, const uint8_t* luma, uint8_t* const planes[4], int hp_pitch, hipStream_t stream) {
    const int W = g.coded_w + 2 * kHpelPad, H = g.coded_h + 2 * kHpelPad;
    dim3 grid((W + kHpTW - 1) / kHpTW, (H + kHpTH - 1) / kHpTH);
    StateArg sa{};
    hipLaunchKernelGGL(k_hpel, grid, dim3(256), 0, stream, g, sa, planes[0], planes[1], planes[2], planes[3], hp_pitch,
                       luma);
}

void launch_me(const Geometry& g, const DeviceBuffers& b, const uint8_t* src_y, hipStream_t stream,
               const FrameState* state) {
    const int nmb = g.mb_w * g.mb_h;
    if (state)
        hipLaunchKernelGGL(k_me_full_val, dim3(nmb), dim3(kMeThreads), 0, stream, g, *state, src_y, b.mb);
    else
        hipLaunchKernelGGL(k_me_full, dim3(nmb), dim3(kMeThreads), 0, stream, g, b.fs, src_y, b.mb);
}

void launch_inter(const Geometry& g, const DeviceBuffers& b, const uint8_t* src_y, const uint8_t* src_uv,
                  hipStream_t stream) {
    const int nmb = g.mb_w * g.mb_h;
    hipLaunchKernelGGL(k_inter_encode, dim3((nmb + 3) / 4), dim3(256), 0, stream, g, b.fs, src_y, src_uv, b.mb,
                       b.coef, b.mb_sse, b.wave_prog);
}

static void launch_analyze(const Geometry& g, const DeviceBuffers& b, const uint8_t* src_y, const uint8_t* src_uv,
                           hipStream_t stream, const FrameState* publish, bool first) {
    const int nmb = g.mb_w * g.mb_h;
    StateArg sa{};
    if (publish) sa.v = *publish;
    sa.dst = b.fs;
    sa.publish = publish ? 1 : 0;
    sa.t_start = (b.out_hdr && first) ? &b.out_hdr->t_start : nullptr;
    hipLaunchKernelGGL(k_intra_analyze, dim3((nmb + 3) / 4), dim3(256), 0, stream, g, sa, src_y, src_uv, b.mb,
                       b.wave_prog, b.intra_gain, b.intra_cand);
}

void launch_intra_in_p(const Geometry& g, const DeviceBuffers& b, const uint8_t* src_y, const uint8_t* src_uv,
                       hipStream_t stream) {
    launch_analyze(g, b, src_y, src_uv, stream, nullptr, false);
    hipLaunchKernelGGL(k_intra_p, dim3(256), dim3(128), 0, stream, g, b.fs, src_y, src_uv, b.mb, b.coef,
                       b.intra_gain, b.mb_sse, b.wave_prog, b.intra_cand);
}

void launch_intra(const Geometry& g, const DeviceBuffers& b, const uint8_t* src_y, const uint8_t* src_uv,
                  hipStream_t stream, const FrameState* publish) {
    launch_analyze(g, b, src_y, src_uv, stream, publish, true);
    const int rows = idr_slice_rows(g.mb_h), slices = (g.mb_h + rows - 1) / rows;
    const size_t lds = (size_t)rows * g.coded_w;
    ensure_func_attr(reinterpret_cast<const void*>(&k_intra_wave), hipFuncAttributeMaxDynamicSharedMemorySize,
                     160 * 1024 - (int)(sizeof(IntraWaveTiles) + sizeof(LumaPipeTiles)) * 8 - 32);
    hipLaunchKernelGGL(k_intra_wave, dim3(slices, 2), dim3(64 * rows), lds, stream, g, b.fs, src_y, src_uv, b.mb,
                       b.coef);
    hipLaunchKernelGGL(k_intra_cbp, dim3((g.mb_w * g.mb_h + 255) / 256), dim3(256), 0, stream, g, b.mb);
}

__global__ __launch_bounds__(256) void k_save_src(Geometry g, const FrameState* __restrict__ fs,
                                                   const uint8_t* __restrict__ src_y) {
    const size_t i = (size_t)blockIdx.x * 256 + threadIdx.x;
    const size_t n = (size_t)g.pitch * g.coded_h / 16;
    if (i < n) reinterpret_cast<uint4*>(fs->save_src)[i] = reinterpret_cast<const uint4*>(src_y)[i];
}

void launch_save_src(const Geometry& g, const DeviceBuffers& b, const uint8_t* src_y, hipStream_t stream) {
    const size_t n = (size_t)g.pitch * g.coded_h / 16;
    hipLaunchKernelGGL(k_save_src, dim3((unsigned)((n + 255) / 256)), dim3(256), 0, stream, g, b.fs, src_y);
}

void launch_entropy(const Geometry& g, const DeviceBuffers& b, uint8_t* host_out, hipStream_t stream,
                    hipEvent_t wait_for_sse) {
    const int nmb = g.mb_w * g.mb_h;
    hipLaunchKernelGGL(k_cavlc, dim3((nmb + kCavlcMbPerBlock - 1) / kCavlcMbPerBlock), dim3(256), 0, stream, g, b.fs,
                       b.mb, b.coef, b.slot,
                       b.slot_bits);
    if (wait_for_sse) HIP_CHECK(hipStreamWaitEvent(stream, wait_for_sse, 0));
    if (g.mb_h > kScanMaxRows || g.mb_w > kScanThreads * kScanRowPer)
        throw std::runtime_error("launch_entropy: frame too large for the row scan");
    hipLaunchKernelGGL(k_scan_rows, dim3(g.mb_h), dim3(kScanThreads), 0, stream, g, b.fs, b.slot_bits, b.row_agg,
                       b.row_sse, b.mb, b.db_cnt);
    hipLaunchKernelGGL(k_scan_out, dim3(g.mb_h), dim3(kScanThreads), 0, stream, g, b.fs, b.slot_bits, b.row_agg,
                       b.row_sse, b.coded_info, b.slice_info, b.out_bytes, b.out_hdr, b.quad_unit, b.db_cnt);
    hipLaunchKernelGGL(k_pack, dim3(256), dim3(256), 0, stream, g, b.fs, b.slot, b.coded_info, b.slice_info,
                       b.out_hdr, host_out, b.quad_unit, b.pack_done);
}

}
}
```

### csrc/codec/hevc_encoder.cpp

```cpp
#include <algorithm>
#include <cstdlib>
#include <cstring>
#include <stdexcept>
#include <string>

#include "../common/hip_check.h"
#include "h264_mb.h"
#include "hevc_encoder.h"

namespace mx {
namespace hevc {

void GpuHevcEncoder::alloc_slot(FrameSlot& sl) {
    const int ncu = geom_.mb_w * geom_.mb_h;
    const int nctb = common_.num_ctbs(), npos = 4 * nctb;
    const int ns = cfg_.hevc_wpp ? std::max(common_.max_slices(), common_.c32_h()) : common_.max_slices();
    HevcDeviceBuffers& b = sl.buf;
    HIP_CHECK(hipMalloc(&b.fs, sizeof(HevcFrameState)));
    HIP_CHECK(hipMalloc(&b.me.fs, sizeof(h264::FrameState)));
    HIP_CHECK(hipMalloc(&b.me.mb, sizeof(h264::MbInfo) * ncu));
    HIP_CHECK(hipMemsetAsync(b.me.mb, 0, sizeof(h264::MbInfo) * ncu, stream_));
    HIP_CHECK(hipMalloc(&b.cu, sizeof(CuInfo) * ncu));
    HIP_CHECK(hipMalloc(&b.coef, sizeof(int16_t) * kCoefPerCu * (size_t)ncu));
    const size_t units_per_slot = std::max((size_t)(ncu + ns - 1) / ns + (size_t)2 * common_.slice_rows() * geom_.mb_w,
// ... 102 lines not shown
    for (int i = 0; i < 4; ++i) HIP_CHECK(hipMalloc(&hp_[i], hp_bytes));
    HIP_CHECK(hipMalloc(&db_state_, sizeof(uint32_t) * 4));
    HIP_CHECK(hipMemsetAsync(db_state_, 0, sizeof(uint32_t) * 4, stream_));
    for (int i = 0; i < depth_; ++i) alloc_slot(slots_[i]);
    if (depth_ > 1) {
        const char* ne = std::getenv("MXDESK_HEVC_ESTREAMS");
        const char* hq = std::getenv("GPU_MAX_HW_QUEUES");
        const int queues = hq && std::atoi(hq) > 0 ? std::atoi(hq) : 4;
        n_es_ = std::clamp(ne ? std::atoi(ne) : std::min(depth_, queues - 2), 1, depth_);
        for (int i = 0; i < n_es_; ++i) HIP_CHECK(hipStreamCreateWithFlags(&stream_e_[i], hipStreamNonBlocking));
        for (int i = n_es_; i < depth_; ++i) stream_e_[i] = stream_e_[i % n_es_];
    }
    clock_khz_ = device_clock_khz();
    HIP_CHECK(hipStreamSynchronize(stream_));
}

GpuHevcEncoder::~GpuHevcEncoder() {
    (void)hipStreamSynchronize(stream_);
    for (int i = 0; i < n_es_; ++i) {
        (void)hipStreamSynchronize(stream_e_[i]);
        (void)hipStreamDestroy(stream_e_[i]);
    }
    for (int i = 0; i < 2; ++i) {
        (void)hipFree(rec_y_[i]);
        (void)hipFree(rec_uv_[i]);
        (void)hipFree(src_keep_[i]);
    }
    for (int i = 0; i < 4; ++i) (void)hipFree(hp_[i]);
    if (pre_y_) (void)hipFree(pre_y_);
    if (pre_uv_) (void)hipFree(pre_uv_);
    for (int i = 0; i < depth_; ++i) free_slot(slots_[i]);
    if (db_state_) (void)hipFree(db_state_);
}

void GpuHevcEncoder::fill_state(FrameSlot& sl, bool idr, int qp, int ref, int cur, bool probe) {
    const size_t org = (size_t)h264::kHpelPad * hp_pitch_ + h264::kHpelPad;
    HevcFrameState& f = *sl.fs_host;
    f.ref_y = rec_y_[ref];
    f.ref_uv = rec_uv_[ref];
    f.sao = (cfg_.sao && !probe) ? 1 : 0;
    f.deblock_on = cfg_.hevc_deblock() ? 1 : 0;
    f.deblock_auto = cfg_.hevc_deblock_auto() ? 1 : 0;
    f.chroma_keep = cfg_.hevc_chroma_keep ? 1 : 0;
    f.rec_y = f.sao ? pre_y_ : rec_y_[cur];
    f.rec_uv = f.sao ? pre_uv_ : rec_uv_[cur];
    f.sao_y = rec_y_[cur];
    f.sao_uv = rec_uv_[cur];
    f.hp_f = hp_[0] + org;
    f.hp_pitch = hp_pitch_;
    f.idr = idr ? 1 : 0;
    f.qp = qp;
    f.slice_rows = 2 * common_.slice_rows();
    f.i_seg_w = common_.i_seg_w();
    f.num_slices = common_.num_slices();
    f.bl_safe = bl_safe_;
    f.bl_safe_split = bl_safe_split_;
    f.depth_inter = common_.depth_inter();
    f.depth_intra = common_.depth_intra();
    f.aq = cfg_.aq;
    f.tu_split = cfg_.tu_split;
    f.chroma_qp_offset = cfg_.chroma_qp_offset;
    f.n_sse_parts = f.sao ? common_.num_ctbs()
                          : (cfg_.hevc_deblock() ? geom_.mb_h : (idr ? geom_.mb_h * common_.i_split() : common_.num_ctbs()));
    f.sse_part = sl.buf.sse_part;
    f.sse_tot = sl.buf.sse_tot;
    for (int k = 0; k < 4; ++k) f.mask_c[k] = mask_c_[k];
    f.prev_src = src_keep_[ref];
    f.save_src = src_keep_[cur];
    f.wpp = cfg_.hevc_wpp ? 1 : 0;
    f.wpp_rows = common_.wpp_rows();
    if (++wpp_epoch_ == 0) wpp_epoch_ = 1;
    f.wpp_epoch = wpp_epoch_;
    f.wpp_ctx = sl.buf.wpp_ctx;
    f.wpp_flag = sl.buf.wpp_flag;
    f.wpp_err = sl.buf.wpp_err;
    h264::FrameState& m = *sl.me_fs_host;
    m.ref_y = rec_y_[ref];
    m.ref_uv = rec_uv_[ref];
    m.qp = qp;
    m.search_range = h264::me_range(cfg_.search_range);
    m.me_coarse = cfg_.me_coarse;
    m.subpel = cfg_.subpel;
    m.partitions = 0;
    m.hp_pitch = hp_pitch_;
    m.hp_f = hp_[0] + org;
    m.hp_h = hp_[1] + org;
    m.hp_v = hp_[2] + org;
    m.hp_j = hp_[3] + org;
    m.sse_part = sl.buf.sse_part;
}

int GpuHevcEncoder::probe_bytes(const uint8_t* src_y, const uint8_t* src_uv, int qp) {
    if (!inflight_.empty()) throw std::logic_error("GpuHevcEncoder: probe with frames in flight");
    prep_slot_ = 0;
    FrameSlot& sl = slots_[0];
    fill_state(sl, true, qp, cur_ ^ 1, cur_, true);
    enqueue_body(true, src_y, src_uv);
    HIP_CHECK(hipStreamSynchronize(stream_));
    HIP_CHECK(hipStreamSynchronize(es(0)));
    const HevcOutHeader hdr = *reinterpret_cast<const HevcOutHeader*>(sl.host_out);
    if (hdr.overflow) return (int)sl.buf.out_bytes;
    const uint32_t* len = reinterpret_cast<const uint32_t*>(sl.host_out + sizeof(HevcOutHeader)) + kMaxSlices;
    size_t total = 0;
    for (uint32_t k = 0; k < hdr.num_slices && k < (uint32_t)kMaxSlices; ++k) total += len[k];
    return (int)(total + common_.num_slices() * 12 + 64);
}

bool GpuHevcEncoder::prepare(bool force_idr) {
    if ((int)inflight_.size() >= depth_) throw std::logic_error("GpuHevcEncoder: collect() a frame first (pipeline full)");
    const int s = (depth_ == 1) ? 0 : next_slot_;
    next_slot_ = (next_slot_ + 1) % depth_;
    prep_slot_ = s;
    FrameSlot& sl = slots_[s];
    h264::EncoderCommon& rc = common_.rc();
    rc.begin_frame(force_idr || !have_ref_);
    have_ref_ = true;
    const bool idr = rc.cur_idr();
    sl.idr = idr;
    sl.qp = rc.cur_qp();
    sl.poc = idr ? 0 : common_.poc();
    const int ref = cur_;
    cur_ ^= 1;
    fill_state(sl, idr, sl.qp, ref, cur_);
    return idr;
}

void GpuHevcEncoder::enqueue_analysis(bool idr, const uint8_t* src_y, const uint8_t* src_uv) {
    enqueue_analysis_impl(idr, src_y, src_uv, false);
}

void GpuHevcEncoder::enqueue_analysis_impl(bool idr, const uint8_t* src_y, const uint8_t* src_uv, bool publish) {
    FrameSlot& sl = slots_[prep_slot_];
    HevcOutHeader* hdr = reinterpret_cast<HevcOutHeader*>(sl.host_out);
    if (publish) {
        launch_hevc_publish(sl.buf, *sl.fs_host, idr ? nullptr : sl.me_fs_host, &hdr->t_start, stream_);
    } else {
        hdr->t_start = 0;
        HIP_CHECK(hipMemcpyAsync(sl.buf.fs, sl.fs_host, sizeof(HevcFrameState), hipMemcpyHostToDevice, stream_));
        if (!idr)
            HIP_CHECK(hipMemcpyAsync(sl.buf.me.fs, sl.me_fs_host, sizeof(h264::FrameState), hipMemcpyHostToDevice,
                                     stream_));
    }
    if (idr) {
        if (cfg_.aq >= 3)
            launch_hevc_save_src(geom_, sl.buf, src_y, stream_);
        launch_hevc_intra(geom_, sl.buf, 2 * common_.slice_rows(), common_.num_slices(), src_y, src_uv, stream_);
    } else {
        h264::launch_hpel(geom_, sl.buf.me, hp_, hp_pitch_, stream_);
        h264::launch_me(geom_, sl.buf.me, src_y, stream_);
        launch_hevc_inter(geom_, sl.buf, src_y, src_uv, stream_);
    }
    launch_hevc_layout(geom_, sl.buf, idr, common_.max_slices(), cfg_.hevc_slice_cost, cfg_.hevc_deblock(), sl.fs_host->sao != 0, src_y,
                       src_uv, stream_, cfg_.hevc_deblock_auto());
}

void GpuHevcEncoder::link_entropy() {
    if (!stream_e_[prep_slot_]) return;
    FrameSlot& sl = slots_[prep_slot_];
    HIP_CHECK(hipEventRecord(sl.analysis_done, stream_));
    HIP_CHECK(hipStreamWaitEvent(stream_e_[prep_slot_], sl.analysis_done, 0));
}

void GpuHevcEncoder::enqueue_entropy() {
    FrameSlot& sl = slots_[prep_slot_];
    launch_hevc_entropy(geom_, sl.buf, common_.max_slices(), sl.host_out, es(prep_slot_));
}

void GpuHevcEncoder::enqueue_body(bool idr, const uint8_t* src_y, const uint8_t* src_uv) {
    enqueue_analysis(idr, src_y, src_uv);
    link_entropy();
    enqueue_entropy();
// ... 138 lines not shown
```

### csrc/codec/video_encoder.h

```cpp
#pragma once
#include <hip/hip_runtime.h>
#include <stdint.h>

#include <vector>

#include "h264_gpu.h"

namespace mx {
namespace h264 {
class EncoderCommon;
struct FrameStats;
}

class VideoEncoder {
   public:
    virtual ~VideoEncoder() = default;
    virtual const char* codec() const = 0;
    virtual const h264::Geometry& geometry() const = 0;
    virtual int pitch() const = 0;
    virtual int depth() const = 0;
    virtual void submit(const uint8_t* src_y, const uint8_t* src_uv, bool force_idr) = 0;
    virtual const std::vector<uint8_t>& collect() = 0;
    virtual const h264::FrameStats& last_stats() const = 0;
    virtual h264::EncoderCommon& rc() = 0;
    virtual const uint8_t* recon_y() const = 0;
    virtual const uint8_t* recon_uv() const = 0;
    virtual hipEvent_t done_event() const = 0;
    virtual bool device_clock() const { return false; }
    virtual uint64_t last_t_end() const { return 0; }
    virtual hipEvent_t pending_done_event() const = 0;
    virtual bool prepare(bool force_idr) = 0;
    virtual void enqueue_body(bool idr, const uint8_t* src_y, const uint8_t* src_uv) = 0;
    virtual void record_start() = 0;
    virtual void record_done() = 0;
    virtual bool supports_split() const { return false; }
    virtual bool masked_sse_in_encoder() const { return false; }
    virtual int prep_slot() const { return 0; }
    virtual hipStream_t entropy_stream() const { return nullptr; }
    virtual void enqueue_analysis(bool idr, const uint8_t* src_y, const uint8_t* src_uv) { (void)idr; (void)src_y; (void)src_uv; }
    virtual void enqueue_entropy() {}
    virtual void link_entropy() {}
    virtual void set_hpel_side_stream(bool on) { (void)on; }
    virtual void quiesce() {}
    virtual bool set_input_event(hipEvent_t ev) { (void)ev; return false; }
};

}
```

### csrc/codec/vp8_gpu.cpp

```cpp
#include <algorithm>
#include <chrono>
#include <memory>
#include <mutex>
#include <cstdio>
#include <cstdlib>
#include <cstring>
#include <stdexcept>
#include <string>
#include <thread>

#include "../common/hip_check.h"
#include "h264_core.h"
#include "h264_mb.h"
#include "vp8_encoder.h"

namespace mx {
namespace vp8 {

namespace {
int pool_threads() {
    const unsigned hc = std::thread::hardware_concurrency();
    return (int)std::clamp(hc ? hc / 2 : 1u, 1u, 16u);
}
int log2_parts_for(int mb_h) { return mb_h >= 8 ? 3 : (mb_h >= 4 ? 2 : (mb_h >= 2 ? 1 : 0)); }
// ... 112 lines not shown
                s.ms = 0;
                (void)hipEventElapsedTime(&s.ms, s.start, s.done);
            }
        } catch (...) {
            s.err = std::current_exception();
        }
        {
            std::lock_guard<std::mutex> lk(wmu_);
            s.ready = true;
        }
        wcv_.notify_all();
    }
}

GpuVp8Encoder::~GpuVp8Encoder() {
    {
        std::lock_guard<std::mutex> lk(wmu_);
        wstop_ = true;
    }
    wcv_.notify_all();
    double wt_us = 0;
    long long wt_n = 0;
    for (int i = 0; i < depth_; ++i) {
        if (slots_[i].writer.joinable()) slots_[i].writer.join();
        wt_us += slots_[i].wt_us;
        wt_n += slots_[i].wt_n;
    }
    if (wt_n > 0 && std::getenv("MXDESK_HOST_TIMING"))
        std::fprintf(stderr, "[mxdesk] vp8 bitstream writer: %.1f us/frame over %lld frames\n", wt_us / wt_n, wt_n);
    (void)hipStreamSynchronize(stream_);
    for (int i = 0; i < 2; ++i) {
        (void)hipFree(rec_y_[i]);
        (void)hipFree(rec_uv_[i]);
        if (src_keep_[i]) (void)hipFree(src_keep_[i]);
    }
    (void)hipFree(hp_);
    for (auto p : hp_sub_)
        if (p) (void)hipFree(p);
    for (int i = 0; i < depth_; ++i) free_slot(slots_[i]);
}

void GpuVp8Encoder::fill_state(Slot& s, bool key, int qp, int ref, int cur) {
    const size_t org = (size_t)h264::kHpelPad * hp_pitch_ + h264::kHpelPad;
    Vp8FrameState& f = s.st_host->v;
    f.ref_y = rec_y_[ref];
    f.ref_uv = rec_uv_[ref];
    f.rec_y = rec_y_[cur];
    f.rec_uv = rec_uv_[cur];
    f.hp_f = hp_ + org;
    f.hp_pitch = hp_pitch_;
    f.key = key ? 1 : 0;
    s.qindex = qindex_for_qp(qp);
    f.qindex = s.qindex;
    if (++epoch_ == 0) epoch_ = 1;
    f.epoch = (int32_t)epoch_;
    s.segmented = !key && cfg_.aq >= 3;
    for (int k = 0; k < kNumSegs; ++k) s.seg_qindex[k] = s.qindex;
    if (s.segmented) segment_qindices(qp, cfg_.aq, s.seg_qindex);
    f.segmented = s.segmented ? 1 : 0;
    f.aq = cfg_.aq;
    f.prev_src = src_keep_[ref];
    f.save_src = src_keep_[cur];
    for (int k = 0; k < kNumSegs; ++k) {
        const Quant Q = quant_of(s.seg_qindex[k]);
        const int q[6] = {Q.y1dc, Q.y1ac, Q.y2dc, Q.y2ac, Q.uvdc, Q.uvac};
        for (int i = 0; i < 6; ++i) {
            f.q[k][i] = q[i];
            f.qm[k][i] = 0xffffffffu / (uint32_t)(3 * q[i]) + 1u;
        }
    }
    f.drop_lambda = h264::lambda_sse(qp);
    f.bpred_lambda = cfg_.vp8_bpred ? h264::lambda_sad(qp) : 0;
    f.intra_lambda = h264::lambda_sad(qp);
    for (int k = 0; k < kNumSegs; ++k) f.lf_level[k] = s.lf_level[k] = 0;
    s.lf_on = false;
    h264::FrameState& m = s.st_host->me;
    std::memset(&m, 0, sizeof m);
    m.ref_y = rec_y_[ref];
    m.ref_uv = rec_uv_[ref];
    m.qp = qp;
    m.search_range = h264::me_range(cfg_.search_range);
    m.me_coarse = cfg_.me_coarse;
    m.subpel = cfg_.subpel ? 1 : 0;
    m.hp_pitch = hp_pitch_;
    m.hp_f = hp_ + org;
    m.hp_h = (cfg_.subpel ? hp_sub_[0] : hp_) + org;
    m.hp_v = (cfg_.subpel ? hp_sub_[1] : hp_) + org;
    m.hp_j = (cfg_.subpel ? hp_sub_[2] : hp_) + org;
}

void GpuVp8Encoder::enqueue_body(bool key, const uint8_t* src_y, const uint8_t* src_uv) {
    Slot& s = slots_[prep_slot_];
    HIP_CHECK(hipMemcpyAsync(s.buf.st, s.st_host, sizeof(Vp8States), hipMemcpyHostToDevice, stream_));
    if (key)
        launch_vp8_key(geom_, s.buf, src_y, src_uv, stream_, cfg_.aq >= 3, cfg_.vp8_bpred != 0);
    else
    {
        uint8_t* const planes[4] = {hp_, hp_sub_[0], hp_sub_[1], hp_sub_[2]};
        launch_vp8_inter(geom_, s.buf, planes, hp_pitch_, cfg_.subpel != 0, src_y, src_uv, stream_, cfg_.vp8_intra != 0);
    }
    if (s.lf_on) launch_vp8_lf(geom_, s.buf, src_y, src_uv, stream_);
    launch_vp8_gather(geom_, s.buf, stream_);
    HIP_CHECK(hipGetLastError());
}

void GpuVp8Encoder::check_slot(Slot& s) {
    if (*s.buf.err) {
        *s.buf.err = 0;
        have_ref_ = false;
        throw std::runtime_error("vp8 gpu encoder: key-frame wavefront hand-off timed out");
    }
}

void GpuVp8Encoder::write_slot(const Slot& s, std::vector<uint8_t>& out, bool probe) {
    const Vp8Mb* mbs = s.buf.mb_host;
    const int16_t* lv = s.buf.lv_host;
    FrameDesc fd{s.key, cfg_.width, cfg_.height, geom_.mb_w, geom_.mb_h, s.qindex, log2_parts_};
    fd.segmented = s.segmented;
    for (int k = 0; k < kNumSegs; ++k) {
        fd.seg_qindex[k] = s.seg_qindex[k];
        fd.lf_level[k] = s.lf_level[k];
    }
    auto levels = [&](int i) -> const int16_t* {
        thread_local int16_t full[kCoefPerMb];
        const Vp8Mb& m = mbs[i];
        const int16_t* p = lv + (size_t)m.slot * 16;
        for (int b = 0; b < kBlocks; ++b) {
            if ((m.nz >> b) & 1u) {
                std::memcpy(full + b * 16, p, 16 * sizeof(int16_t));
                p += 16;
            } else {
                std::memset(full + b * 16, 0, 16 * sizeof(int16_t));
            }
        }
        return full;
    };
    write_frame(fd, mbs, levels, out,
                [&](int n, const std::function<void(int)>& fn) { pool_->run(n, fn); },
                probe ? nullptr : &tok_stats_[s.key ? 1 : 0][s.fidx % kStatsLag]);
}

int GpuVp8Encoder::probe_bytes(const uint8_t* src_y, const uint8_t* src_uv, int qp) {
    if (!inflight_.empty()) throw std::logic_error("GpuVp8Encoder: probe with frames in flight");
    prep_slot_ = 0;
    Slot& s = slots_[0];
    s.key = true;
    fill_state(s, true, qp, cur_ ^ 1, cur_);
    enqueue_body(true, src_y, src_uv);
    HIP_CHECK(hipStreamSynchronize(stream_));
    check_slot(s);
    std::vector<uint8_t> tmp;
    write_slot(s, tmp, true);
    return (int)tmp.size();
}

bool GpuVp8Encoder::prepare(bool force_idr) {
    if ((int)inflight_.size() >= depth_) throw std::logic_error("GpuVp8Encoder: collect() a frame first (pipeline full)");
    const int n = (depth_ == 1) ? 0 : next_slot_;
    next_slot_ = (next_slot_ + 1) % depth_;
    prep_slot_ = n;
    Slot& s = slots_[n];
    common_.begin_frame(force_idr || !have_ref_);
    have_ref_ = true;
    s.key = common_.cur_idr();
    s.qp = common_.cur_qp();
    s.fidx = frames_++;
    const int ref = cur_;
    cur_ ^= 1;
    fill_state(s, s.key, s.qp, ref, cur_);
    lf_levels(lf_.decide(s.fidx, s.key), s.segmented, s.qindex, s.seg_qindex, lf_num_, s.lf_level);
    for (int k = 0; k < kNumSegs; ++k) {
// ... 70 lines not shown
```

### csrc/runtime/session.cpp

```cpp
#include "session.h"

#include <functional>
#include <cstdio>
#include <cstdlib>

#include <exception>
#include <thread>

#include <algorithm>
#include <cmath>
#include <cstring>
#include <stdexcept>

#include "../common/hip_check.h"
#include "../common/trace.h"
#include "../codec/hevc_encoder.h"
#include "../codec/vp8_encoder.h"

namespace mx {

FramePool::FramePool(int width, int height, int slots) : w_(width), h_(height) {
    if (slots < 1) throw std::invalid_argument("FramePool needs >= 1 slot");
    pitch_ = ((width * 4) + 255) & ~255;
    buf_.resize(slots, nullptr);
// ... 12 lines not shown
    return s;
}

static double lanczos3(double x) {
    x = std::fabs(x);
    if (x < 1e-9) return 1.0;
    if (x >= 3.0) return 0.0;
    const double px = M_PI * x;
    return 3.0 * std::sin(px) * std::sin(px / 3.0) / (px * px);
}

void make_lanczos_table(int in_size, int out_size, std::vector<int>& start, std::vector<float>& weights, int& taps) {
    const double s = (double)in_size / out_size;
    const double f = std::max(1.0, s);
    const double support = 3.0 * f;
    taps = (int)std::ceil(2.0 * support) + 1;
    start.resize(out_size);
    weights.assign((size_t)out_size * taps, 0.f);
    for (int o = 0; o < out_size; ++o) {
        const double center = (o + 0.5) * s - 0.5;
        const int x0 = (int)std::floor(center - support) + 1;
        start[o] = x0;
        double sum = 0;
        std::vector<double> w(taps);
        for (int k = 0; k < taps; ++k) {
            w[k] = lanczos3((x0 + k - center) / f);
            sum += w[k];
        }
        for (int k = 0; k < taps; ++k) weights[(size_t)o * taps + k] = (float)(w[k] / sum);
    }
}

int64_t Session::now_us() {
    return std::chrono::duration_cast<std::chrono::microseconds>(std::chrono::steady_clock::now().time_since_epoch())
        .count();
}

Session::Session(const SessionConfig& cfg) : cfg_(cfg) {
    if (cfg_.out_width <= 0) cfg_.out_width = cfg_.width;
    if (cfg_.out_height <= 0) cfg_.out_height = cfg_.height;
    cfg_.enc.width = cfg_.out_width;
    cfg_.enc.height = cfg_.out_height;
    cfg_.enc.fps = cfg_.fps;
    cfg_.enc.mask_x0 = cfg_.mask_x0;
    cfg_.enc.mask_y0 = cfg_.mask_y0;
    cfg_.enc.mask_x1 = cfg_.mask_x1;
    cfg_.enc.mask_y1 = cfg_.mask_y1;
    HIP_CHECK(hipStreamCreateWithFlags(&stream_, hipStreamNonBlocking));
    pool_ = std::make_unique<FramePool>(cfg_.width, cfg_.height, cfg_.pool_slots);
    if ((cfg_.codec == "h264" || cfg_.codec == "avc") && cfg_.use_graph && cfg_.enc.deblock != 0 &&
        cfg_.enc.deblock != 1) {
        if (cfg_.enc.deblock > 1)
            throw std::invalid_argument("hipGraph replay needs a fixed H.264 filter (deblock 0 or 1), not adaptive");
        cfg_.enc.deblock = 0;
    }
    if (cfg_.codec == "h264" || cfg_.codec == "avc")
        enc_ = std::make_unique<h264::GpuH264Encoder>(cfg_.enc, stream_);
    else if (cfg_.codec == "hevc" || cfg_.codec == "h265")
        enc_ = std::make_unique<hevc::GpuHevcEncoder>(cfg_.enc, stream_);
    else if (cfg_.codec == "vp8")
        enc_ = std::make_unique<vp8::GpuVp8Encoder>(cfg_.enc, stream_);
    else
        throw std::invalid_argument("Session: unknown codec '" + cfg_.codec + "' (h264 | hevc | vp8)");
    const h264::Geometry& g = enc_->geometry();
    depth_ = enc_->depth();
    if (depth_ > kMaxDepth) throw std::invalid_argument("Session: encoder pipeline depth above kMaxDepth");
    for (int k = 0; k < depth_; ++k) {
        HIP_CHECK(hipMalloc(&nv12_y_[k], (size_t)g.pitch * g.coded_h));
        HIP_CHECK(hipMalloc(&nv12_uv_[k], (size_t)g.pitch * g.coded_h / 2));
    }
    const std::string codec = enc_->codec();
    const bool cap = cfg_.capture_stream > 0 || (cfg_.capture_stream < 0 && (codec == "h264" || codec == "hevc"));
    if (depth_ > 1 && cap && !cfg_.use_graph) {
        const char* cp = std::getenv("MXDESK_CAPTURE_PRIORITY");
        if (cp && std::string(cp) == "low") {
            int least = 0, greatest = 0;
            HIP_CHECK(hipDeviceGetStreamPriorityRange(&least, &greatest));
            HIP_CHECK(hipStreamCreateWithPriority(&cap_stream_, hipStreamNonBlocking, least));
        } else {
            HIP_CHECK(hipStreamCreateWithFlags(&cap_stream_, hipStreamNonBlocking));
        }
        for (int k = 0; k < depth_; ++k)
            HIP_CHECK(hipEventCreateWithFlags(&ev_conv_[k], hipEventDisableTiming | hipEventReleaseToDevice));
        enc_->set_hpel_side_stream(false);
    }
    if (depth_ > 1 && cfg_.use_graph && !enc_->supports_split())
        throw std::invalid_argument("hipGraph replay with pipeline_depth 2 needs an encoder with the split form");
    if (depth_ >= cfg_.pool_slots) throw std::invalid_argument("pool_slots must exceed pipeline_depth");
    for (int k = 0; k < depth_; ++k)
        HIP_CHECK(hipHostMalloc(&staging_[k], (size_t)pool_->pitch() * cfg_.height, hipHostMallocDefault));
    scale_ = cfg_.out_width != cfg_.width || cfg_.out_height != cfg_.height;
    if (scale_) {
        std::vector<int> sx, sy;
        std::vector<float> wx, wy;
        int tx, ty;
        make_lanczos_table(cfg_.width, cfg_.out_width, sx, wx, tx);
        make_lanczos_table(cfg_.height, cfg_.out_height, sy, wy, ty);
        const size_t bytes = (sx.size() + sy.size()) * 4 + (wx.size() + wy.size()) * 4;
        HIP_CHECK(hipMalloc(&lt_mem_, bytes));
        char* p = static_cast<char*>(lt_mem_);
        lt_.out_w = cfg_.out_width;
        lt_.out_h = cfg_.out_height;
        lt_.taps_x = tx;
        lt_.taps_y = ty;
        lt_.x0 = reinterpret_cast<const int*>(p);
        HIP_CHECK(hipMemcpy(p, sx.data(), sx.size() * 4, hipMemcpyHostToDevice));
        p += sx.size() * 4;
        lt_.y0 = reinterpret_cast<const int*>(p);
        HIP_CHECK(hipMemcpy(p, sy.data(), sy.size() * 4, hipMemcpyHostToDevice));
        p += sy.size() * 4;
        lt_.wx = reinterpret_cast<const float*>(p);
        HIP_CHECK(hipMemcpy(p, wx.data(), wx.size() * 4, hipMemcpyHostToDevice));
        p += wx.size() * 4;
        lt_.wy = reinterpret_cast<const float*>(p);
        HIP_CHECK(hipMemcpy(p, wy.data(), wy.size() * 4, hipMemcpyHostToDevice));
        const h264::Geometry& eg = enc_->geometry();
        pix::ScaleFragsHost fr;
        if (!cfg_.scale_valu && pix::build_scale_frags(cfg_.width, cfg_.height, cfg_.out_width, cfg_.out_height,
                                                       eg.coded_w, eg.coded_h, sx, wx, tx, sy, wy, ty, fr))
            pix::upload_scale_frags(fr, &lt_mf_mem_, lt_.mf);
    }
    for (int k = 0; k < kMaxDepth; ++k) HIP_CHECK(hipEventCreate(&ev_start_[k]));
    devclk_ = enc_->device_clock();
    clock_khz_ = device_clock_khz();
    HIP_CHECK(hipHostMalloc(&ts_, sizeof(uint64_t) * cfg_.pool_slots, hipHostMallocMapped));
    std::memset(ts_, 0, sizeof(uint64_t) * cfg_.pool_slots);
    mask_in_encoder_ = enc_->masked_sse_in_encoder();
    if (masked() && !mask_in_encoder_) {
        const h264::Geometry& eg = enc_->geometry();
        const int nb = pix::sse_masked_blocks(eg.width, eg.height);
        HIP_CHECK(hipMalloc(&mask_dev_, kMaxDepth * (size_t)nb * sizeof(unsigned long long)));
        HIP_CHECK(hipMalloc(&mask_counter_, kMaxDepth * sizeof(unsigned int)));
        HIP_CHECK(hipMemset(mask_counter_, 0, kMaxDepth * sizeof(unsigned int)));
        mask_stride_ = nb;
        HIP_CHECK(hipHostMalloc(&mask_host_, kMaxDepth * sizeof(unsigned long long), hipHostMallocMapped));
        for (int k = 0; k < kMaxDepth; ++k) HIP_CHECK(hipEventCreateWithFlags(&ev_mask_[k], hipEventDisableTiming));
    }
    HIP_CHECK(hipHostMalloc(&synth_host_, sizeof(pix::SynthParams) * cfg_.pool_slots, hipHostMallocDefault));
    HIP_CHECK(hipMalloc(&synth_bg_, (size_t)pool_->pitch() * cfg_.height));
    pix::launch_synth_static(synth_bg_, synth_params(), stream_);
    HIP_CHECK(hipGetLastError());
    HIP_CHECK(hipStreamSynchronize(stream_));
    HIP_CHECK(hipMalloc(&synth_dev_, sizeof(pix::SynthParams) * cfg_.pool_slots));
    graphs_.assign((size_t)cfg_.pool_slots * kMaxDepth * 2 * 2, nullptr);
    t0_us_ = now_us();
}

Session::~Session() {
    if (ht_n_ > 0 && std::getenv("MXDESK_HOST_TIMING"))
        std::fprintf(stderr, "[mxdesk] host us/frame over %lld frames: submit %.1f, wait %.1f, collect %.1f\n",
                     (long long)ht_n_, ht_submit_ / ht_n_, ht_wait_ / ht_n_, ht_post_ / ht_n_);
    if (stream_) (void)hipStreamSynchronize(stream_);
    if (cap_stream_) (void)hipStreamSynchronize(cap_stream_);
    if (upload_stream_) (void)hipStreamSynchronize(upload_stream_);
    enc_.reset();
    for (auto g : graphs_)
        if (g) hipGraphExecDestroy(g);
    hipHostFree(synth_host_);
    if (ts_) hipHostFree(ts_);
    if (synth_bg_) hipFree(synth_bg_);
    hipFree(synth_dev_);
    pool_.reset();
    if (cap_stream_) (void)hipStreamDestroy(cap_stream_);
    for (int k = 0; k < kMaxDepth; ++k) {
        if (nv12_y_[k]) (void)hipFree(nv12_y_[k]);
        if (nv12_uv_[k]) (void)hipFree(nv12_uv_[k]);
        if (ev_conv_[k]) (void)hipEventDestroy(ev_conv_[k]);
// ... 438 lines not shown
```

Baseline: 11040.

## Replace precomputed half-pel planes with on-the-fly luma interpolation in ME and inter

Removes the four padded half-pel plane buffers and the k_hpel pass per frame. Motion estimation and inter prediction now interpolate quarter-sample luma directly from the reconstructed reference in a wave-level routine. The unfiltered-reference planes become a plain luma copy. The change also adds an alternating second entropy stream for depth >= 3 and creates the ME side stream lazily. It saves the hpel pass and its memory traffic but adds extra arithmetic inside the ME and inter kernels.

```diff
diff --git a/csrc/bindings/module.cpp b/csrc/bindings/module.cpp
--- a/csrc/bindings/module.cpp
+++ b/csrc/bindings/module.cpp
@@ -112,6 +112,14 @@
         }
         return out;
     });
+    h.def("mc_luma_gpu", [](py::array_t<uint8_t, py::array::c_style> ref, int coded_w, int x4, int y4) {
+        if (ref.ndim() != 2 || coded_w % 16 || ref.shape(0) % 16 || ref.shape(1) < coded_w)
+            throw std::invalid_argument("ref must be (coded_h, pitch) with 16-aligned coded size");
+        py::array_t<uint8_t> out({16, 16});
+        h264::mc_luma_for_test(ref.data(), coded_w, (int)ref.shape(0), (int)ref.shape(1), x4, y4, out.mutable_data());
+        return out;
+    }, py::arg("ref"), py::arg("coded_w"), py::arg("x4"), py::arg("y4"),
+          "16x16 luma prediction at quarter-sample position (x4, y4) by k_inter_encode's interpolation");
     h.def("cavlc_block", &cavlc_block_py, py::arg("coef"), py::arg("nc"));
     h.def("fdct4x4", &fdct_py);
     h.def("idct4x4", &idct_py);
diff --git a/csrc/codec/h264_encoder.cpp b/csrc/codec/h264_encoder.cpp
--- a/csrc/codec/h264_encoder.cpp
+++ b/csrc/codec/h264_encoder.cpp
@@ -212,6 +212,25 @@
     (void)hipFree(b.fs);
     *hp_pitch_out = hp_pitch;
     return out;
+}
+
+void mc_luma_for_test(const uint8_t* ref, int coded_w, int coded_h, int pitch, int x4, int y4, uint8_t* out) {
+    Geometry g{};
+    g.width = g.coded_w = coded_w;
+    g.height = g.coded_h = coded_h;
+    g.mb_w = coded_w / 16;
+    g.mb_h = coded_h / 16;
+    g.pitch = pitch;
+    uint8_t *dref = nullptr, *dout = nullptr;
+    HIP_CHECK(hipMalloc(&dref, (size_t)pitch * coded_h));
+    HIP_CHECK(hipMalloc(&dout, 256));
+    HIP_CHECK(hipMemcpy(dref, ref, (size_t)pitch * coded_h, hipMemcpyHostToDevice));
+    launch_mc_luma_test(g, dref, x4, y4, dout, nullptr);
+    const hipError_t e = hipGetLastError();
+    if (e == hipSuccess) (void)hipMemcpy(out, dout, 256, hipMemcpyDeviceToHost);
+    (void)hipFree(dref);
+    (void)hipFree(dout);
+    HIP_CHECK(e);
 }
 
 constexpr unsigned kDeviceEvent = hipEventDisableTiming | hipEventReleaseToDevice;
@@ -254,7 +273,6 @@
     HIP_CHECK(hipEventCreateWithFlags(&sl.start, hipEventDisableTiming));
     HIP_CHECK(hipEventCreateWithFlags(&sl.analysis_done, kDeviceEvent));
     HIP_CHECK(hipEventCreateWithFlags(&sl.deblock_done, kDeviceEvent));
-    HIP_CHECK(hipEventCreateWithFlags(&sl.hpel_done, kDeviceEvent));
     HIP_CHECK(hipEventCreateWithFlags(&sl.me_done, kDeviceEvent));
     HIP_CHECK(hipEventCreateWithFlags(&sl.done, hipEventDisableTiming));
 }
@@ -269,7 +287,7 @@
     if (b.db_err) (void)hipHostFree(b.db_err);
     if (sl.fs_host) (void)hipHostFree(sl.fs_host);
     if (sl.host_out) (void)hipHostFree(sl.host_out);
-    for (hipEvent_t e : {sl.start, sl.analysis_done, sl.deblock_done, sl.done, sl.hpel_done, sl.me_done})
+    for (hipEvent_t e : {sl.start, sl.analysis_done, sl.deblock_done, sl.done, sl.me_done})
         if (e) (void)hipEventDestroy(e);
 }
 
@@ -311,30 +329,12 @@
         for (int mx = mask_mb_[0]; mx < mask_mb_[2]; ++mx)
             masked_pixels_ -= (int64_t)std::max(0, std::min(16, cfg.width - 16 * mx)) *
                               std::max(0, std::min(16, cfg.height - 16 * my));
-    hp_pitch_ = (geom_.coded_w + 2 * kHpelPad + 255) & ~255;
-    const size_t hp_bytes = (size_t)hp_pitch_ * (geom_.coded_h + 2 * kHpelPad);
-    for (int i = 0; i < 4; ++i) HIP_CHECK(hipMalloc(&hp_[i], hp_bytes));
-    if (cfg_.h264_deblock())
-        for (int i = 0; i < 4; ++i) HIP_CHECK(hipMalloc(&hpu_[i], hp_bytes));
+    if (cfg_.h264_deblock()) HIP_CHECK(hipMalloc(&rec_unf_, ysz));
     for (int i = 0; i < depth_; ++i) alloc_slot(slots_[i]);
     clock_khz_ = device_clock_khz();
     if (depth_ > 1) {
         HIP_CHECK(hipStreamCreateWithFlags(&stream_e_, hipStreamNonBlocking));
-        HIP_CHECK(hipStreamCreateWithFlags(&stream_a_, hipStreamNonBlocking));
-        HIP_CHECK(hipEventCreateWithFlags(&ref_ready_, kDeviceEvent));
-        HIP_CHECK(hipEventRecord(ref_ready_, stream_));
         if (cfg_.h264_deblock()) {
-            const char* rv = std::getenv("MXDESK_ME_CU_RESERVE");
-            const int reserve = rv ? std::atoi(rv) : 0;
-            int ncu = 0;
-            HIP_CHECK(hipDeviceGetAttribute(&ncu, hipDeviceAttributeMultiprocessorCount, 0));
-            if (reserve > 0 && reserve < ncu) {
-                std::vector<uint32_t> mask((size_t)(ncu + 31) / 32, 0u);
-                for (int c = 0; c < ncu - reserve; ++c) mask[(size_t)c / 32] |= 1u << (c % 32);
-                HIP_CHECK(hipExtStreamCreateWithCUMask(&stream_m_, (uint32_t)mask.size(), mask.data()));
-            } else {
-                HIP_CHECK(hipStreamCreateWithFlags(&stream_m_, hipStreamNonBlocking));
-            }
             HIP_CHECK(hipEventCreateWithFlags(&ev_hpu_, kDeviceEvent));
             HIP_CHECK(hipEventRecord(ev_hpu_, stream_));
         }
@@ -347,12 +347,25 @@
     }
 }
 
-void GpuH264Encoder::set_hpel_side_stream(bool on) {
-    hpel_side_ = on;
-    if (!on && stream_a_) {
-        HIP_CHECK(hipStreamSynchronize(stream_a_));
-        HIP_CHECK(hipStreamDestroy(stream_a_));
-        stream_a_ = nullptr;
+void GpuH264Encoder::ensure_me_stream() {
+    if (stream_m_) return;
+    e2_retired_ = true;
+    if (stream_e2_) {
+        drain_launcher();
+        HIP_CHECK(hipStreamSynchronize(stream_e2_));
+        HIP_CHECK(hipStreamDestroy(stream_e2_));
+        stream_e2_ = nullptr;
+    }
+    const char* rv = std::getenv("MXDESK_ME_CU_RESERVE");
+    const int reserve = rv ? std::atoi(rv) : 0;
+    int ncu = 0;
+    HIP_CHECK(hipDeviceGetAttribute(&ncu, hipDeviceAttributeMultiprocessorCount, 0));
+    if (reserve > 0 && reserve < ncu) {
+        std::vector<uint32_t> mask((size_t)(ncu + 31) / 32, 0u);
+        for (int c = 0; c < ncu - reserve; ++c) mask[(size_t)c / 32] |= 1u << (c % 32);
+        HIP_CHECK(hipExtStreamCreateWithCUMask(&stream_m_, (uint32_t)mask.size(), mask.data()));
+    } else {
+        HIP_CHECK(hipStreamCreateWithFlags(&stream_m_, hipStreamNonBlocking));
     }
 }
 
@@ -369,10 +382,10 @@
         }
         try {
             FrameSlot& sl = slots_[j.slot];
-            HIP_CHECK(hipStreamWaitEvent(stream_e_, sl.analysis_done, 0));
-            launch_entropy(geom_, sl.buf, sl.host_out, stream_e_, j.sse_ready);
+            HIP_CHECK(hipStreamWaitEvent(j.stream, sl.analysis_done, 0));
+            launch_entropy(geom_, sl.buf, sl.host_out, j.stream, j.sse_ready);
             HIP_CHECK(hipGetLastError());
-            HIP_CHECK(hipEventRecord(sl.done, stream_e_));
+            HIP_CHECK(hipEventRecord(sl.done, j.stream));
         } catch (...) {
             std::lock_guard<std::mutex> lk(lmu_);
             lerr_ = std::current_exception();
@@ -412,24 +425,21 @@
         (void)hipStreamSynchronize(stream_e_);
         (void)hipStreamDestroy(stream_e_);
     }
-    if (stream_a_) {
-        (void)hipStreamSynchronize(stream_a_);
-        (void)hipStreamDestroy(stream_a_);
-    }
-    if (ref_ready_) (void)hipEventDestroy(ref_ready_);
+    if (stream_e2_) {
+        (void)hipStreamSynchronize(stream_e2_);
+        (void)hipStreamDestroy(stream_e2_);
+    }
     if (stream_m_) {
         (void)hipStreamSynchronize(stream_m_);
         (void)hipStreamDestroy(stream_m_);
     }
     if (ev_hpu_) (void)hipEventDestroy(ev_hpu_);
-    for (int i = 0; i < 4; ++i)
-        if (hpu_[i]) (void)hipFree(hpu_[i]);
+    if (rec_unf_) (void)hipFree(rec_unf_);
     for (int i = 0; i < 2; ++i) {
         (void)hipFree(rec_y_[i]);
         (void)hipFree(rec_uv_[i]);
         (void)hipFree(src_keep_[i]);
     }
-    for (int i = 0; i < 4; ++i) (void)hipFree(hp_[i]);
     for (int i = 0; i < depth_; ++i) free_slot(slots_[i]);
 }
 
@@ -447,11 +457,7 @@
         if (cfg_.aq >= 3)
             launch_save_src(geom_, sl.buf, src_y, stream_);
     } else {
-        static const bool early = [] {
-            const char* e = std::getenv("MXDESK_INPUT_WAIT");
-            return e && std::string(e) == "early";
-        }();
-        if (early) wait_input();
+        if (depth_ > 1 && pub && sl.me_unf) ensure_me_stream();
         const bool side_me = stream_m_ && pub && sl.me_unf;
         if (side_me) {
             HIP_CHECK(hipStreamWaitEvent(stream_m_, ev_hpu_, 0));
@@ -459,22 +465,13 @@
                 HIP_CHECK(hipStreamWaitEvent(stream_m_, in_ev_, 0));
                 in_ev_ = nullptr;
             }
-            launch_me(geom_, sl.buf, src_y, stream_m_, pub);
+            launch_me(geom_, sl.buf, src_y, stream_m_, pub, true);
             HIP_CHECK(hipEventRecord(sl.me_done, stream_m_));
-        }
-        if (stream_a_ && hpel_side_ && pub && ref_seq_ + 1 == seq_) {
-            HIP_CHECK(hipStreamWaitEvent(stream_a_, ref_ready_, 0));
-            launch_hpel(geom_, sl.buf, hp_, hp_pitch_, stream_a_, pub);
-            HIP_CHECK(hipEventRecord(sl.hpel_done, stream_a_));
-            HIP_CHECK(hipStreamWaitEvent(stream_, sl.hpel_done, 0));
+            HIP_CHECK(hipStreamWaitEvent(stream_, sl.me_done, 0));
         } else {
-            launch_hpel(geom_, sl.buf, hp_, hp_pitch_, stream_, pub);
-        }
-        wait_input();
-        if (side_me)
-            HIP_CHECK(hipStreamWaitEvent(stream_, sl.me_done, 0));
-        else
-            launch_me(geom_, sl.buf, src_y, stream_);
+            wait_input();
+            launch_me(geom_, sl.buf, src_y, stream_, pub);
+        }
         launch_inter(geom_, sl.buf, src_y, src_uv, stream_);
         if (cfg_.intra_in_p) launch_intra_in_p(geom_, sl.buf, src_y, src_uv, stream_);
     }
@@ -494,9 +491,9 @@
     launch_entropy(geom_, sl.buf, sl.host_out, stream_e_ ? stream_e_ : stream_, nullptr);
 }
 
-void GpuH264Encoder::unfiltered_planes(FrameSlot& sl) {
-    launch_hpel_of(geom_, sl.fs_host->rec_y, hpu_, hp_pitch_, stream_);
-    if (stream_m_) HIP_CHECK(hipEventRecord(ev_hpu_, stream_));
+void GpuH264Encoder::unfiltered_copy(FrameSlot& sl) {
+    launch_copy_luma(geom_, sl.fs_host->rec_y, rec_unf_, stream_);
+    if (ev_hpu_) HIP_CHECK(hipEventRecord(ev_hpu_, stream_));
 }
 
 void GpuH264Encoder::enqueue_kernels(bool idr, const uint8_t* src_y, const uint8_t* src_uv, bool publish) {
@@ -507,20 +504,19 @@
         HIP_CHECK(hipEventRecord(sl.analysis_done, stream_));
         hipEvent_t sse_ready = nullptr;
         if (sl.deblock) {
-            unfiltered_planes(sl);
+            unfiltered_copy(sl);
             launch_deblock(geom_, sl.buf, src_y, src_uv, stream_);
             HIP_CHECK(hipEventRecord(sl.deblock_done, stream_));
             sse_ready = sl.deblock_done;
         }
-        if (stream_a_ && hpel_side_ && publish) {
-            HIP_CHECK(hipEventRecord(ref_ready_, stream_));
-            ref_seq_ = seq_;
-        }
+        if (depth_ >= 3 && !stream_e2_ && !e2_retired_ && !stream_m_)
+            HIP_CHECK(hipStreamCreateWithFlags(&stream_e2_, hipStreamNonBlocking));
+        hipStream_t es = (stream_e2_ && (seq_ & 1)) ? stream_e2_ : stream_e_;
         HIP_CHECK(hipGetLastError());
         {
             std::lock_guard<std::mutex> lk(lmu_);
             if (lerr_) std::rethrow_exception(lerr_);
-            ljobs_.push_back(EntropyJob{prep_slot_, sse_ready});
+            ljobs_.push_back(EntropyJob{prep_slot_, sse_ready, es});
             slot_job_[prep_slot_] = ++l_pushed_;
         }
         lcv_.notify_all();
@@ -530,16 +526,12 @@
     hipStream_t es = stream_e_ ? stream_e_ : stream_;
     hipEvent_t sse_ready = nullptr;
     if (sl.deblock) {
-        unfiltered_planes(sl);
+        unfiltered_copy(sl);
         launch_deblock(geom_, sl.buf, src_y, src_uv, stream_);
         if (stream_e_) {
             HIP_CHECK(hipEventRecord(sl.deblock_done, stream_));
             sse_ready = sl.deblock_done;
         }
-    }
-    if (stream_a_ && hpel_side_ && publish) {
-        HIP_CHECK(hipEventRecord(ref_ready_, stream_));
-        ref_seq_ = seq_;
     }
     launch_entropy(geom_, sl.buf, sl.host_out, es, sse_ready);
     HIP_CHECK(hipGetLastError());
@@ -567,8 +559,6 @@
     f.pic_init_qp = common_.pic_init_qp();
     f.chroma_qp_offset = cfg_.chroma_qp_offset;
     f.log2_max_frame_num = common_.log2_max_frame_num();
-    const size_t org = (size_t)kHpelPad * hp_pitch_ + kHpelPad;
-    f.hp_pitch = hp_pitch_;
     f.aq = cfg_.aq;
     f.intra_in_p = cfg_.intra_in_p;
     f.partitions = cfg_.partitions ? 1 : 0;
@@ -576,14 +566,7 @@
     f.mask_my0 = mask_mb_[1];
     f.mask_mx1 = mask_mb_[2];
     f.mask_my1 = mask_mb_[3];
-    f.hp_f = hp_[0] + org;
-    f.hp_h = hp_[1] + org;
-    f.hp_v = hp_[2] + org;
-    f.hp_j = hp_[3] + org;
-    f.me_f = sl.me_unf ? hpu_[0] + org : nullptr;
-    f.me_h = sl.me_unf ? hpu_[1] + org : nullptr;
-    f.me_v = sl.me_unf ? hpu_[2] + org : nullptr;
-    f.me_j = sl.me_unf ? hpu_[3] + org : nullptr;
+    f.me_ref = sl.me_unf ? rec_unf_ : nullptr;
     f.sse_part = sl.buf.sse_part;
     f.prev_src = src_keep_[ref];
     f.save_src = src_keep_[cur];
diff --git a/csrc/codec/h264_encoder.h b/csrc/codec/h264_encoder.h
--- a/csrc/codec/h264_encoder.h
+++ b/csrc/codec/h264_encoder.h
@@ -143,6 +143,7 @@
 void emulation_prevent(std::vector<uint8_t>& out, const uint8_t* rbsp, size_t n);
 std::vector<std::vector<uint8_t>> hpel_planes_for_test(const uint8_t* ref, int coded_w, int coded_h, int pitch,
                                                        int* hp_pitch);
+void mc_luma_for_test(const uint8_t* ref, int coded_w, int coded_h, int pitch, int x4, int y4, uint8_t* out);
 
 class GpuH264Encoder final : public VideoEncoder {
    public:
@@ -177,7 +178,6 @@
     void enqueue_analysis(bool idr, const uint8_t* src_y, const uint8_t* src_uv) override;
     void enqueue_entropy() override;
     void link_entropy() override;
-    void set_hpel_side_stream(bool on) override;
     void quiesce() override { drain_launcher(); }
     bool set_input_event(hipEvent_t ev) override {
         in_ev_ = ev;
@@ -200,7 +200,6 @@
         FrameState* fs_host = nullptr;
         uint8_t* host_out = nullptr;
         hipEvent_t start = nullptr, analysis_done = nullptr, deblock_done = nullptr, done = nullptr;
-        hipEvent_t hpel_done = nullptr;
         bool idr = false;
         bool deblock = false;
         bool me_unf = false;
@@ -211,11 +210,13 @@
     void alloc_slot(FrameSlot& sl);
     void free_slot(FrameSlot& sl);
     void fill_state(FrameSlot& sl, bool idr, int qp, int ref, int cur);
-    void unfiltered_planes(FrameSlot& sl);
+    void unfiltered_copy(FrameSlot& sl);
+    void ensure_me_stream();
     int probe_bytes(const uint8_t* src_y, const uint8_t* src_uv, int qp);
     struct EntropyJob {
         int slot;
         hipEvent_t sse_ready;
+        hipStream_t stream;
     };
     void launcher_loop();
     void wait_launched(int slot) const;
@@ -236,11 +237,10 @@
     EncoderCommon common_;
     hipStream_t stream_;
     hipStream_t stream_e_ = nullptr;
-    hipStream_t stream_a_ = nullptr;
-    bool hpel_side_ = true;
+    hipStream_t stream_e2_ = nullptr;
+    bool e2_retired_ = false;
     hipEvent_t in_ev_ = nullptr;
-    hipEvent_t ref_ready_ = nullptr;
-    uint64_t seq_ = 0, ref_seq_ = ~0ull;
+    uint64_t seq_ = 0;
     int depth_ = 1;
     Geometry geom_;
     FrameSlot slots_[kMaxInFlight];
@@ -249,12 +249,10 @@
     hipEvent_t last_done_ = nullptr;
     uint64_t last_t_end_ = 0;
     double clock_khz_ = 100000;
-    uint8_t* hp_[4] = {nullptr, nullptr, nullptr, nullptr};
-    uint8_t* hpu_[4] = {nullptr, nullptr, nullptr, nullptr};
+    uint8_t* rec_unf_ = nullptr;
     hipStream_t stream_m_ = nullptr;
     hipEvent_t ev_hpu_ = nullptr;
     bool last_deblock_ = false;
-    int hp_pitch_ = 0;
     uint8_t* rec_y_[2] = {nullptr, nullptr};
     uint8_t* rec_uv_[2] = {nullptr, nullptr};
     uint8_t* src_keep_[2] = {nullptr, nullptr};
diff --git a/csrc/codec/h264_gpu.h b/csrc/codec/h264_gpu.h
--- a/csrc/codec/h264_gpu.h
+++ b/csrc/codec/h264_gpu.h
@@ -66,21 +66,13 @@
     int32_t pic_init_qp;
     int32_t chroma_qp_offset;
     int32_t log2_max_frame_num;
-    int32_t hp_pitch;
     int32_t aq;
     int32_t intra_in_p;
     int32_t partitions;
     int32_t mask_mx0, mask_my0, mask_mx1, mask_my1;
     const uint8_t* prev_src;
     uint8_t* save_src;
-    const uint8_t* hp_f;
-    const uint8_t* hp_h;
-    const uint8_t* hp_v;
-    const uint8_t* hp_j;
-    const uint8_t* me_f;
-    const uint8_t* me_h;
-    const uint8_t* me_v;
-    const uint8_t* me_j;
+    const uint8_t* me_ref;
     unsigned long long* sse_part;
 };
 constexpr int kHpelPad = 48;
@@ -137,8 +129,9 @@
 };
 
 void launch_me(const Geometry& g, const DeviceBuffers& b, const uint8_t* src_y, hipStream_t stream,
-               const FrameState* state = nullptr);
-void launch_hpel_of(const Geometry& g, const uint8_t* luma, uint8_t* const planes[4], int hp_pitch, hipStream_t stream);
+               const FrameState* publish = nullptr, bool side = false);
+void launch_copy_luma(const Geometry& g, const uint8_t* luma, uint8_t* dst, hipStream_t stream);
+void launch_mc_luma_test(const Geometry& g, const uint8_t* ref, int x4, int y4, uint8_t* out, hipStream_t stream);
 void launch_inter(const Geometry& g, const DeviceBuffers& b, const uint8_t* src_y, const uint8_t* src_uv,
                   hipStream_t stream);
 void launch_intra(const Geometry& g, const DeviceBuffers& b, const uint8_t* src_y, const uint8_t* src_uv,
diff --git a/csrc/codec/h264_kernels.hip b/csrc/codec/h264_kernels.hip
--- a/csrc/codec/h264_kernels.hip
+++ b/csrc/codec/h264_kernels.hip
@@ -72,39 +72,6 @@
     v += __builtin_amdgcn_mov_dpp(v, 0x124, 0xF, 0xF, false);
     v += __builtin_amdgcn_mov_dpp(v, 0x128, 0xF, 0xF, false);
     return (int)rows_sum((uint32_t)v);
-}
-
-struct Planes {
-    const uint8_t *f, *h, *v, *j;
-    int pitch;
-};
-__device__ __forceinline__ Planes planes_of(const FrameState* fs) {
-    return Planes{fs->hp_f, fs->hp_h, fs->hp_v, fs->hp_j, fs->hp_pitch};
-}
-__device__ __forceinline__ Planes me_planes_of(const FrameState* fs) {
-    return fs->me_f ? Planes{fs->me_f, fs->me_h, fs->me_v, fs->me_j, fs->hp_pitch} : planes_of(fs);
-}
-__device__ __forceinline__ int qpel_planes(const Planes& P, int x4, int y4) {
-    const int xi = x4 >> 2, yi = y4 >> 2, xf = x4 & 3, yf = y4 & 3;
-    const int o = yi * P.pitch + xi;
-    const int G = P.f[o];
-    if ((xf | yf) == 0) return G;
-    if (yf == 0) {
-        const int b = P.h[o];
-        if (xf == 2) return b;
-        return ((xf == 1 ? G : (int)P.f[o + 1]) + b + 1) >> 1;
-    }
-    if (xf == 0) {
-        const int hh = P.v[o];
-        if (yf == 2) return hh;
-        return ((yf == 1 ? G : (int)P.f[o + P.pitch]) + hh + 1) >> 1;
-    }
-    if (xf == 2 && yf == 2) return P.j[o];
-    if (xf == 2) return ((yf == 1 ? (int)P.h[o] : (int)P.h[o + P.pitch]) + P.j[o] + 1) >> 1;
-    if (yf == 2) return ((xf == 1 ? (int)P.v[o] : (int)P.v[o + 1]) + P.j[o] + 1) >> 1;
-    const int bb = (yf == 1) ? P.h[o] : P.h[o + P.pitch];
-    const int hh = (xf == 1) ? P.v[o] : P.v[o + 1];
-    return (bb + hh + 1) >> 1;
 }
 
 constexpr int kHpTW = 128, kHpTH = 16;
@@ -131,12 +98,11 @@
 
 __global__ __launch_bounds__(256) void k_hpel(Geometry g, StateArg sa, uint8_t* __restrict__ pf,
                                               uint8_t* __restrict__ ph, uint8_t* __restrict__ pv,
-                                              uint8_t* __restrict__ pj, int hp_pitch,
-                                              const uint8_t* __restrict__ src) {
+                                              uint8_t* __restrict__ pj, int hp_pitch) {
     __shared__ uint32_t smp[kHpTH + 5][kHpSW / 4];
     __shared__ int4 b1[kHpTH + 5][kHpTW / 4];
     publish_state(sa);
-    const uint8_t* __restrict__ ref = src ? src : state_of(sa).ref_y;
+    const uint8_t* __restrict__ ref = state_of(sa).ref_y;
     const int px0 = blockIdx.x * kHpTW, py0 = blockIdx.y * kHpTH;
     const int W = g.coded_w + 2 * kHpelPad, H = g.coded_h + 2 * kHpelPad;
     const int tid = threadIdx.x;
@@ -232,13 +198,45 @@
 }
 
 constexpr int kMaxRange = 32;
-static_assert(kMaxRange + 2 <= kHpelPad, "search window must stay inside the padded planes");
+constexpr int kWinPadX = 4, kWinPadY = 3;
 constexpr int kWinStride = 16 + 2 * kMaxRange + 8;
+constexpr int kWinRows = 16 + 2 * kMaxRange + 7;
 
 constexpr int kMeThreads = 256, kMeWaves = kMeThreads / 64;
-__device__ __forceinline__ void me_full_body(const Geometry& g, const FrameState* __restrict__ fs,
-                                             const uint8_t* __restrict__ src_y, MbInfo* __restrict__ mbs) {
-    __shared__ uint32_t win32[(16 + 2 * kMaxRange) * kWinStride / 4];
+constexpr int kFpRows = 18 + 5;
+__device__ __forceinline__ void build_footprints(const uint8_t* win, int org0, int org1, int n,
+                                                 uint8_t (*sp)[4][18][kSpW], int16_t (*b1)[kFpRows][kSpW], int tid) {
+    for (int i = tid; i < n * kFpRows * 18; i += kMeThreads) {
+        const int pi = i / (kFpRows * 18), rem = i - pi * (kFpRows * 18), r = rem / 18, c = rem - r * 18;
+        const uint8_t* p = win + (pi ? org1 : org0) + (r - 2) * kWinStride + c;
+        b1[pi][r][c] = (int16_t)tap6(p[-2], p[-1], p[0], p[1], p[2], p[3]);
+    }
+    __syncthreads();
+    for (int i = tid; i < n * 324; i += kMeThreads) {
+        const int pi = i / 324, rem = i - pi * 324, r = rem / 18, c = rem - r * 18;
+        const uint8_t* p = win + (pi ? org1 : org0) + r * kWinStride + c;
+        const int16_t(*b)[kSpW] = b1[pi];
+        const int v1 = tap6(p[-2 * kWinStride], p[-kWinStride], p[0], p[kWinStride], p[2 * kWinStride], p[3 * kWinStride]);
+        const int j1 = tap6(b[r][c], b[r + 1][c], b[r + 2][c], b[r + 3][c], b[r + 4][c], b[r + 5][c]);
+        sp[pi][0][r][c] = p[0];
+        sp[pi][1][r][c] = (uint8_t)clip255((b[r + 2][c] + 16) >> 5);
+        sp[pi][2][r][c] = (uint8_t)clip255((v1 + 16) >> 5);
+        sp[pi][3][r][c] = (uint8_t)clip255((j1 + 512) >> 10);
+    }
+}
+
+struct MeState {
+    const uint8_t* ref;
+    int qp, search_range, subpel, me_coarse, partitions;
+};
+__device__ __forceinline__ MeState me_state(const FrameState& f) {
+    return MeState{f.me_ref ? f.me_ref : f.ref_y, f.qp, f.search_range, f.subpel, f.me_coarse, f.partitions};
+}
+__device__ __forceinline__ void me_full_body(const Geometry& g, const MeState& st, const uint8_t* __restrict__ src_y,
+                                             MbInfo* __restrict__ mbs) {
+    __shared__ uint32_t win_lds[kWinRows * kWinStride / 4];
+    __shared__ uint8_t sp2[2][4][18][kSpW];
+    __shared__ int16_t fp_b1[2][kFpRows][kSpW];
     __shared__ uint32_t srcw[64];
     __shared__ unsigned long long red[kMeWaves];
     __shared__ uint32_t cand_cost[8];
@@ -248,23 +246,23 @@
     const int mbx = mbi % g.mb_w, mby = mbi / g.mb_w;
     const int x0 = mbx * 16, y0 = mby * 16;
     const int tid = threadIdx.x, lane = tid & 63;
-    const int R = me_range(fs->search_range);
+    const int R = me_range(st.search_range);
     const int W = 16 + 2 * R;
-    const Planes P = me_planes_of(fs);
-    const int lambda = lambda_sad(fs->qp);
+    const uint8_t* __restrict__ ref = st.ref;
+    const int lambda = lambda_sad(st.qp);
 
     constexpr int kWs4 = kWinStride / 4;
     {
         if (tid < 64) {
             const int r = tid >> 2, c4 = (tid & 3) * 4;
             const uint32_t sw = *reinterpret_cast<const uint32_t*>(src_y + (y0 + r) * g.pitch + x0 + c4);
-            const uint32_t rw = *reinterpret_cast<const uint32_t*>(P.f + (y0 + r) * P.pitch + x0 + c4);
+            const uint32_t rw = *reinterpret_cast<const uint32_t*>(ref + (y0 + r) * g.pitch + x0 + c4);
             const int d = wave_sum((int)__builtin_amdgcn_sad_u8(sw, rw, 0u));
             if (tid == 0) s_sad0[0] = (uint32_t)d;
         }
         __syncthreads();
         const uint32_t sad0 = s_sad0[0];
-        if (sad0 <= static_sad(fs->qp)) {
+        if (sad0 <= static_sad(st.qp)) {
             if (tid == 0) {
                 MbInfo& m = mbs[mbi];
                 m.mvx = 0;
@@ -276,10 +274,29 @@
         }
     }
     const bool t256 = tid < 256;
-    for (int i = tid; i < W * kWs4; i += kMeThreads) {
+    const int wrows = W + 2 * kWinPadY + 1, wx0 = x0 - R - kWinPadX, wy0 = y0 - R - kWinPadY;
+    const bool dwords = (g.pitch & 3) == 0 && (reinterpret_cast<uintptr_t>(ref) & 3) == 0;
+    for (int i = tid; i < wrows * kWs4; i += kMeThreads) {
         const int wy = i / kWs4, wx4 = (i - wy * kWs4) * 4;
-        win32[i] = (wx4 < W) ? *reinterpret_cast<const uint32_t*>(P.f + (y0 - R + wy) * P.pitch + (x0 - R + wx4)) : 0u;
-    }
+        uint32_t w = 0u;
+        if (wx4 < W + 2 * kWinPadX) {
+            const int py = min(max(wy0 + wy, 0), g.coded_h - 1), px = wx0 + wx4;
+            const uint8_t* row = ref + (size_t)py * g.pitch;
+            if (px < 0)
+                w = row[0] * 0x01010101u;
+            else if (px >= g.coded_w)
+                w = row[g.coded_w - 1] * 0x01010101u;
+            else if (dwords)
+                w = *reinterpret_cast<const uint32_t*>(row + px);
+            else
+                w = row[px] | ((uint32_t)row[px + 1] << 8) | ((uint32_t)row[px + 2] << 16) | ((uint32_t)row[px + 3] << 24);
+        }
+        win_lds[i] = w;
+    }
+    const uint32_t* win32 = win_lds + kWinPadY * kWs4 + kWinPadX / 4;
+    auto fp_org = [&](int vx, int vy) {
+        return ((vy >> 2) + R + kWinPadY - 1) * kWinStride + (vx >> 2) + R + kWinPadX - 1;
+    };
     if (tid < 64) {
         const int r = tid >> 2, c = (tid & 3) * 4;
         srcw[tid] = *reinterpret_cast<const uint32_t*>(src_y + (y0 + r) * g.pitch + x0 + c);
@@ -288,8 +305,8 @@
 
     const int side = 2 * R + 1, gw = (side + 3) >> 2, ngroups = side * gw;
     unsigned long long best = ~0ull;
-    const bool coarse = fs->me_coarse != 0;
-    const bool parts = fs->partitions != 0;
+    const bool coarse = st.me_coarse != 0;
+    const bool parts = st.partitions != 0;
     const int ntask = (coarse && !parts) ? (R + 1) * gw : 0;
     auto mkey = [&](uint32_t sad, int dxr, int dyr) {
         const int dx = dxr - R, dy = dyr - R;
@@ -501,16 +518,11 @@
                 pvy[i] = 4 * ((cb / side) - R);
                 pcost[i] = (uint32_t)(pbest[s0 + i] >> 32);
             }
-            if (fs->subpel) {
-                __shared__ uint8_t psp[2][4][18][kSpW];
+            if (st.subpel) {
+                uint8_t(*psp)[4][18][kSpW] = sp2;
                 __shared__ uint32_t pcand[2][8];
-                for (int i = tid; i < 2 * 4 * 18 * 18; i += kMeThreads) {
-                    const int pi = i / (4 * 324), rem0 = i - pi * 4 * 324;
-                    const int pl = rem0 / 324, rem = rem0 - pl * 324, r = rem / 18, c = rem - r * 18;
-                    const uint8_t* base = pl == 0 ? P.f : pl == 1 ? P.h : pl == 2 ? P.v : P.j;
-                    const int ix = x0 + (pvx[pi] >> 2) - 1, iy = y0 + (pvy[pi] >> 2) - 1;
-                    psp[pi][pl][r][c] = base[(iy + r) * P.pitch + ix + c];
-                }
+                build_footprints(reinterpret_cast<const uint8_t*>(win_lds), fp_org(pvx[0], pvy[0]),
+                                 fp_org(pvx[1], pvy[1]), 2, sp2, fp_b1, tid);
                 __syncthreads();
                 const int pi = (tid & 255) >> 7, k = (tid >> 4) & 7, sub = tid & 15;
                 const int rx = part == kPart8x16 ? 8 * pi : 0, ry = part == kPart16x8 ? 8 * pi : 0;
@@ -566,14 +578,9 @@
         }
     }
 
-    if (fs->subpel) {
-        __shared__ uint8_t sp[4][18][kSpW];
-        const int ix = x0 + (mvx >> 2) - 1, iy = y0 + (mvy >> 2) - 1;
-        for (int i = tid; i < 4 * 18 * 18; i += kMeThreads) {
-            const int pl = i / 324, rem = i - pl * 324, r = rem / 18, c = rem - r * 18;
-            const uint8_t* base = pl == 0 ? P.f : pl == 1 ? P.h : pl == 2 ? P.v : P.j;
-            sp[pl][r][c] = base[(iy + r) * P.pitch + ix + c];
-        }
+    if (st.subpel) {
+        uint8_t(*sp)[18][kSpW] = sp2[0];
+        build_footprints(reinterpret_cast<const uint8_t*>(win_lds), fp_org(mvx, mvy), 0, 1, sp2, fp_b1, tid);
         __syncthreads();
         uint32_t cur_cost = (uint32_t)(b >> 32);
         const int k = (tid & 255) >> 5, sub = tid & 31;
@@ -620,13 +627,15 @@
     }
 }
 
-__global__ __launch_bounds__(kMeThreads) void k_me_full(Geometry g, const FrameState* __restrict__ fs,
-                                                  const uint8_t* __restrict__ src_y, MbInfo* __restrict__ mbs) {
-    me_full_body(g, fs, src_y, mbs);
-}
-__global__ __launch_bounds__(kMeThreads) void k_me_full_val(Geometry g, FrameState fs,
-                                                      const uint8_t* __restrict__ src_y, MbInfo* __restrict__ mbs) {
-    me_full_body(g, &fs, src_y, mbs);
+__global__ __launch_bounds__(kMeThreads) void k_me_full(Geometry g, StateArg sa, const uint8_t* __restrict__ src_y,
+                                                        MbInfo* __restrict__ mbs) {
+    publish_state(sa);
+    me_full_body(g, sa.publish ? me_state(sa.v) : me_state(*sa.dst), src_y, mbs);
+}
+__global__ __launch_bounds__(kMeThreads) void k_me_full_val(Geometry g, StateArg sa, const uint8_t* __restrict__ src_y,
+                                                            MbInfo* __restrict__ mbs) {
+    publish_state(sa);
+    me_full_body(g, me_state(sa.v), src_y, mbs);
 }
 
 template <int K>
@@ -691,6 +700,92 @@
     const int qm = qp % 6, qs = qp / 6;
 #pragma unroll
     for (int c = 0; c < 4; ++c) d[c] = z[c] * kDequantV[qm][kPosClass[r * 4 + c]] * (1 << qs);
+}
+
+__device__ __forceinline__ void wave_sync_lds() {
+    __builtin_amdgcn_fence(__ATOMIC_RELEASE, "wavefront");
+    __builtin_amdgcn_wave_barrier();
+    __builtin_amdgcn_fence(__ATOMIC_ACQUIRE, "wavefront");
+}
+
+constexpr int kMcStride = 24, kMcRows = 16 + 5, kMcWords = kMcRows * kMcStride / 4;
+__device__ __forceinline__ void mc_luma_wave(uint32_t* __restrict__ w, const uint8_t* __restrict__ ref, int pitch,
+                                             int cw, int ch, int n, int xa, int ya, int xb, int yb, int lane, int lpi,
+                                             uint32_t* out) {
+    const bool aligned = (pitch & 3) == 0 && (reinterpret_cast<uintptr_t>(ref) & 3) == 0;
+    for (int i = lane; i < n * kMcWords; i += 64) {
+        const int pi = i >= kMcWords ? 1 : 0, j = i - pi * kMcWords;
+        const int wr = j / (kMcStride / 4), q = j - wr * (kMcStride / 4);
+        const int xs = ((pi ? xb : xa) >> 2) - 2, ys = ((pi ? yb : ya) >> 2) - 2;
+        uint32_t v;
+        if (aligned && xs >= 0 && (xs & ~3) + kMcStride + 4 <= cw) {
+            const int py = min(max(ys + wr, 0), ch - 1), px = xs + 4 * q;
+            const uint32_t* qa = reinterpret_cast<const uint32_t*>(ref + (size_t)py * pitch + (px & ~3));
+            const uint32_t sh = (uint32_t)(px & 3);
+            v = sh ? __builtin_amdgcn_alignbyte(qa[1], qa[0], sh) : qa[0];
+        } else {
+            v = 0;
+            for (int k = 0; k < 4; ++k) v |= (uint32_t)ref_px(ref, pitch, cw, ch, xs + 4 * q + k, ys + wr) << (8 * k);
+        }
+        w[i] = v;
+    }
+    wave_sync_lds();
+    {
+        const int xf = (lpi ? xb : xa) & 3, yf = (lpi ? yb : ya) & 3;
+        w += lpi * kMcWords;
+        const int r = lane >> 2, q0 = lane & 3;
+        uint32_t wd[6][3];
+#pragma unroll
+        for (int rr = 0; rr < 6; ++rr) {
+            const uint32_t* row = w + (r + rr) * (kMcStride / 4) + q0;
+            wd[rr][0] = row[0];
+            wd[rr][1] = row[1];
+            wd[rr][2] = row[2];
+        }
+        auto s = [&](int rr, int c) { return byte_of(wd[rr][c >> 2], c & 3); };
+        auto b1 = [&](int rr) { return tap6(s(rr, 0), s(rr, 1), s(rr, 2), s(rr, 3), s(rr, 4), s(rr, 5)); };
+        auto v1 = [&](int c) { return tap6(s(0, c), s(1, c), s(2, c), s(3, c), s(4, c), s(5, c)); };
+        auto b_at = [&](int rr) { return clip255((b1(rr) + 16) >> 5); };
+        auto h_at = [&](int c) { return clip255((v1(c) + 16) >> 5); };
+        auto j_val = [&]() { return clip255((tap6(b1(0), b1(1), b1(2), b1(3), b1(4), b1(5)) + 512) >> 10); };
+        uint32_t packed = 0;
+#pragma unroll 1
+        for (int k = 0; k < 4; ++k) {
+            const int G = s(2, 2);
+            int p;
+            if ((xf | yf) == 0)
+                p = G;
+            else if (yf == 0)
+                p = xf == 2 ? b_at(2) : ((xf == 1 ? G : s(2, 3)) + b_at(2) + 1) >> 1;
+            else if (xf == 0)
+                p = yf == 2 ? h_at(2) : ((yf == 1 ? G : s(3, 2)) + h_at(2) + 1) >> 1;
+            else if (xf == 2 && yf == 2)
+                p = j_val();
+            else if (xf == 2)
+                p = ((yf == 1 ? b_at(2) : b_at(3)) + j_val() + 1) >> 1;
+            else if (yf == 2)
+                p = ((xf == 1 ? h_at(2) : h_at(3)) + j_val() + 1) >> 1;
+            else
+                p = ((yf == 1 ? b_at(2) : b_at(3)) + (xf == 1 ? h_at(2) : h_at(3)) + 1) >> 1;
+            packed |= (uint32_t)p << (8 * k);
+#pragma unroll
+            for (int rr = 0; rr < 6; ++rr) {
+                wd[rr][0] = __builtin_amdgcn_alignbyte(wd[rr][1], wd[rr][0], 1);
+                wd[rr][1] = __builtin_amdgcn_alignbyte(wd[rr][2], wd[rr][1], 1);
+                wd[rr][2] >>= 8;
+            }
+        }
+        *out = packed;
+    }
+}
+
+__global__ __launch_bounds__(64) void k_mc_luma_test(Geometry g, const uint8_t* __restrict__ ref, int x4, int y4,
+                                                     uint8_t* __restrict__ out) {
+    __shared__ uint32_t w[kMcWords];
+    const int lane = threadIdx.x;
+    uint32_t p = 0;
+    mc_luma_wave(w, ref, g.pitch, g.coded_w, g.coded_h, 1, x4, y4, x4, y4, lane, 0, &p);
+    reinterpret_cast<uint32_t*>(out)[lane] = p;
 }
 
 __global__ __launch_bounds__(256) void k_inter_encode(Geometry g, const FrameState* __restrict__ fs,
@@ -700,6 +795,7 @@
                                                        int* __restrict__ wave_prog) {
     __shared__ uint8_t pred[4][384];
     __shared__ int16_t res[4][384];
+    __shared__ uint32_t mcw[4][2 * kMcWords];
     __shared__ int cdc[4][8];
     __shared__ int cdc_nz[4][2];
 
@@ -711,7 +807,8 @@
     const bool valid = mbi < nmb;
     const int mbx = valid ? mbi % g.mb_w : 0, mby = valid ? mbi / g.mb_w : 0;
     const int x0 = mbx * 16, y0 = mby * 16;
-    const Planes P = planes_of(fs);
+    const uint8_t* __restrict__ ref_y = fs->ref_y;
+    const bool ref_dwords = (g.pitch & 3) == 0 && (reinterpret_cast<uintptr_t>(ref_y) & 3) == 0;
     const uint8_t* ref_uv = fs->ref_uv;
     const int cw = g.coded_w / 2, ch = g.coded_h / 2;
     int mvx = 0, mvy = 0;
@@ -742,26 +839,32 @@
             }
             *reinterpret_cast<uint32_t*>(fs->save_src + (y0 + r) * g.pitch + x0 + c0) = sw;
         }
-        if (((mvx | mvy) & 3) == 0) {
-            const uint8_t* q = P.f + (size_t)((y0 + r) + (mvy >> 2)) * P.pitch + (x0 + c0 + (mvx >> 2));
-            const uint32_t* qa = reinterpret_cast<const uint32_t*>(reinterpret_cast<uintptr_t>(q) & ~(uintptr_t)3);
-            const uint32_t sh = (uint32_t)(reinterpret_cast<uintptr_t>(q) & 3);
-            const uint32_t pw = sh ? __builtin_amdgcn_alignbyte(qa[1], qa[0], sh) : qa[0];
-            for (int k = 0; k < 4; ++k) {
-                const int p = (int)((pw >> (8 * k)) & 0xff);
-                const int d = (int)((sw >> (8 * k)) & 0xff) - p;
-                pred[wave][r * 16 + c0 + k] = (uint8_t)p;
-                res[wave][r * 16 + c0 + k] = (int16_t)d;
-                lsad += d < 0 ? -d : d;
-            }
+        const int part = __builtin_amdgcn_readfirstlane((int)mi.part);
+        const Mv va = blk_mv(mi, 0, 0), vb = blk_mv(mi, part == kPart8x16 ? 2 : 0, part == kPart16x8 ? 2 : 0);
+        const int vax = __builtin_amdgcn_readfirstlane(va.x), vay = __builtin_amdgcn_readfirstlane(va.y);
+        const int vbx = __builtin_amdgcn_readfirstlane(vb.x), vby = __builtin_amdgcn_readfirstlane(vb.y);
+        uint32_t pw = 0;
+        if ((vax | vay | vbx | vby) & 3) {
+            const int lpi = part == kPart16x8 ? (r >> 3) : (part == kPart8x16 ? (c0 >> 3) : 0);
+            mc_luma_wave(mcw[wave], ref_y, g.pitch, g.coded_w, g.coded_h, part == kPart16x16 ? 1 : 2, x0 * 4 + vax,
+                         y0 * 4 + vay, x0 * 4 + vbx, y0 * 4 + vby, lane, lpi, &pw);
         } else {
-            for (int k = 0; k < 4; ++k) {
-                const int p = qpel_planes(P, (x0 + c0 + k) * 4 + mvx, (y0 + r) * 4 + mvy);
-                const int d = (int)((sw >> (8 * k)) & 0xff) - p;
-                pred[wave][r * 16 + c0 + k] = (uint8_t)p;
-                res[wave][r * 16 + c0 + k] = (int16_t)d;
-                lsad += d < 0 ? -d : d;
-            }
+            const int px = x0 + c0 + (mvx >> 2), py = min(max(y0 + r + (mvy >> 2), 0), g.coded_h - 1);
+            if (px >= 0 && px + 4 <= g.coded_w && ((px & 3) == 0 || (px & ~3) + 8 <= g.pitch) && ref_dwords) {
+                const uint32_t* qa = reinterpret_cast<const uint32_t*>(ref_y + (size_t)py * g.pitch + (px & ~3));
+                const uint32_t sh = (uint32_t)(px & 3);
+                pw = sh ? __builtin_amdgcn_alignbyte(qa[1], qa[0], sh) : qa[0];
+            } else {
+                for (int k = 0; k < 4; ++k)
+                    pw |= (uint32_t)ref_px(ref_y, g.pitch, g.coded_w, g.coded_h, px + k, py) << (8 * k);
+            }
+        }
+        for (int k = 0; k < 4; ++k) {
+            const int p = (int)((pw >> (8 * k)) & 0xff);
+            const int d = (int)((sw >> (8 * k)) & 0xff) - p;
+            pred[wave][r * 16 + c0 + k] = (uint8_t)p;
+            res[wave][r * 16 + c0 + k] = (int16_t)d;
+            lsad += d < 0 ? -d : d;
         }
         const int cr_ = lane >> 3, cc = lane & 7;
         const int xc = x0 / 2 + cc, yc = y0 / 2 + cr_;
@@ -914,11 +1017,6 @@
 }
 
 __constant__ uint8_t kRasterToBlk[16] = {0, 1, 4, 5, 2, 3, 6, 7, 8, 9, 12, 13, 10, 11, 14, 15};
-__device__ __forceinline__ void wave_sync_lds() {
-    __builtin_amdgcn_fence(__ATOMIC_RELEASE, "wavefront");
-    __builtin_amdgcn_wave_barrier();
-    __builtin_amdgcn_fence(__ATOMIC_ACQUIRE, "wavefront");
-}
 
 constexpr int kLT = 24;
 constexpr int kCT = 10;
@@ -2335,24 +2433,36 @@
     sa.publish = publish ? 1 : 0;
     sa.t_start = b.out_hdr ? &b.out_hdr->t_start : nullptr;
     hipLaunchKernelGGL(k_hpel, grid, dim3(256), 0, stream, g, sa, planes[0], planes[1], planes[2], planes[3],
-                       hp_pitch, (const uint8_t*)nullptr);
-}
-
-void launch_hpel_of(const Geometry& g, const uint8_t* luma, uint8_t* const planes[4], int hp_pitch, hipStream_t stream) {
-    const int W = g.coded_w + 2 * kHpelPad, H = g.coded_h + 2 * kHpelPad;
-    dim3 grid((W + kHpTW - 1) / kHpTW, (H + kHpTH - 1) / kHpTH);
+                       hp_pitch);
+}
+
+__global__ __launch_bounds__(256) void k_copy_luma(const uint4* __restrict__ src, uint4* __restrict__ dst, size_t n) {
+    const size_t i = (size_t)blockIdx.x * 256 + threadIdx.x;
+    if (i < n) dst[i] = src[i];
+}
+
+void launch_copy_luma(const Geometry& g, const uint8_t* luma, uint8_t* dst, hipStream_t stream) {
+    const size_t n = (size_t)g.pitch * g.coded_h / 16;
+    hipLaunchKernelGGL(k_copy_luma, dim3((unsigned)((n + 255) / 256)), dim3(256), 0, stream,
+                       reinterpret_cast<const uint4*>(luma), reinterpret_cast<uint4*>(dst), n);
+}
+
+void launch_mc_luma_test(const Geometry& g, const uint8_t* ref, int x4, int y4, uint8_t* out, hipStream_t stream) {
+    hipLaunchKernelGGL(k_mc_luma_test, dim3(1), dim3(64), 0, stream, g, ref, x4, y4, out);
+}
+
+void launch_me(const Geometry& g, const DeviceBuffers& b, const uint8_t* src_y, hipStream_t stream,
+               const FrameState* publish, bool side) {
+    const int nmb = g.mb_w * g.mb_h;
     StateArg sa{};
-    hipLaunchKernelGGL(k_hpel, grid, dim3(256), 0, stream, g, sa, planes[0], planes[1], planes[2], planes[3], hp_pitch,
-                       luma);
-}
-
-void launch_me(const Geometry& g, const DeviceBuffers& b, const uint8_t* src_y, hipStream_t stream,
-               const FrameState* state) {
-    const int nmb = g.mb_w * g.mb_h;
-    if (state)
-        hipLaunchKernelGGL(k_me_full_val, dim3(nmb), dim3(kMeThreads), 0, stream, g, *state, src_y, b.mb);
+    if (publish) sa.v = *publish;
+    sa.dst = b.fs;
+    sa.publish = publish ? 1 : 0;
+    sa.t_start = b.out_hdr ? &b.out_hdr->t_start : nullptr;
+    if (side && publish)
+        hipLaunchKernelGGL(k_me_full_val, dim3(nmb), dim3(kMeThreads), 0, stream, g, sa, src_y, b.mb);
     else
-        hipLaunchKernelGGL(k_me_full, dim3(nmb), dim3(kMeThreads), 0, stream, g, b.fs, src_y, b.mb);
+        hipLaunchKernelGGL(k_me_full, dim3(nmb), dim3(kMeThreads), 0, stream, g, sa, src_y, b.mb);
 }
 
 void launch_inter(const Geometry& g, const DeviceBuffers& b, const uint8_t* src_y, const uint8_t* src_uv,
diff --git a/csrc/codec/hevc_encoder.cpp b/csrc/codec/hevc_encoder.cpp
--- a/csrc/codec/hevc_encoder.cpp
+++ b/csrc/codec/hevc_encoder.cpp
@@ -208,11 +208,6 @@
     m.me_coarse = cfg_.me_coarse;
     m.subpel = cfg_.subpel;
     m.partitions = 0;
-    m.hp_pitch = hp_pitch_;
-    m.hp_f = hp_[0] + org;
-    m.hp_h = hp_[1] + org;
-    m.hp_v = hp_[2] + org;
-    m.hp_j = hp_[3] + org;
     m.sse_part = sl.buf.sse_part;
 }
 
diff --git a/csrc/codec/video_encoder.h b/csrc/codec/video_encoder.h
--- a/csrc/codec/video_encoder.h
+++ b/csrc/codec/video_encoder.h
@@ -40,7 +40,6 @@
     virtual void enqueue_analysis(bool idr, const uint8_t* src_y, const uint8_t* src_uv) { (void)idr; (void)src_y; (void)src_uv; }
     virtual void enqueue_entropy() {}
     virtual void link_entropy() {}
-    virtual void set_hpel_side_stream(bool on) { (void)on; }
     virtual void quiesce() {}
     virtual bool set_input_event(hipEvent_t ev) { (void)ev; return false; }
 };
diff --git a/csrc/codec/vp8_gpu.cpp b/csrc/codec/vp8_gpu.cpp
--- a/csrc/codec/vp8_gpu.cpp
+++ b/csrc/codec/vp8_gpu.cpp
@@ -218,11 +218,6 @@
     m.search_range = h264::me_range(cfg_.search_range);
     m.me_coarse = cfg_.me_coarse;
     m.subpel = cfg_.subpel ? 1 : 0;
-    m.hp_pitch = hp_pitch_;
-    m.hp_f = hp_ + org;
-    m.hp_h = (cfg_.subpel ? hp_sub_[0] : hp_) + org;
-    m.hp_v = (cfg_.subpel ? hp_sub_[1] : hp_) + org;
-    m.hp_j = (cfg_.subpel ? hp_sub_[2] : hp_) + org;
 }
 
 void GpuVp8Encoder::enqueue_body(bool key, const uint8_t* src_y, const uint8_t* src_uv) {
diff --git a/csrc/runtime/session.cpp b/csrc/runtime/session.cpp
--- a/csrc/runtime/session.cpp
+++ b/csrc/runtime/session.cpp
@@ -118,7 +118,6 @@
         }
         for (int k = 0; k < depth_; ++k)
             HIP_CHECK(hipEventCreateWithFlags(&ev_conv_[k], hipEventDisableTiming | hipEventReleaseToDevice));
-        enc_->set_hpel_side_stream(false);
     }
     if (depth_ > 1 && cfg_.use_graph && !enc_->supports_split())
         throw std::invalid_argument("hipGraph replay with pipeline_depth 2 needs an encoder with the split form");
```

Result: faster. 11250 (median of 6 runs) (+2.0%).
